# xipengwang/AprilSAM

Measured on AMD Instinct MI355X. Metric: Gauss-Newton iterations/sec + factorise ms on M3500 (chi2 match <=1e-6), higher is better.
Workload: dtype f64; 1 GPU; M3500 batch april_graph_cholesky, 1 replica per GPU (3500 poses, 5454 factors, n=10500); parallelism=single GPU, fronts=680, levels=9, nnz_L=422121

## Files before the change

### aprilsam_amd/csrc/capi.cpp

```cpp
#include <algorithm>
#include <cstdio>
#include <cstdlib>
#include <cstring>
#include <string>
#include <vector>

#include "../../include/aprilsam_amd.h"
#include "plan.h"
#include "errors.h"
#include "refmodel.h"
#include "solver.h"

extern "C" {

void APRILSAM_VERSION(void) {
    printf("================\n");
    printf("| APRILSAM 0.0 |   solver: aprilsam_amd (MI355X / gfx950)\n");
    printf("================\n");
    printf("\n");
}

void april_graph_cholesky_param_init(april_graph_cholesky_param_t *param) {
    asam::drop_context(param);
    asam::unbind_param(param);
// ... 39 lines not shown
int aprilsam_amd_resident_steps(april_graph_t *graph, april_graph_cholesky_param_t *param, int n, int mode) { return asam::resident_steps(graph, param, n, mode); }
int aprilsam_amd_resident_sync(april_graph_t *graph, april_graph_cholesky_param_t *param) { return asam::resident_sync(graph, param); }
double aprilsam_amd_resident_chi2(april_graph_t *graph) { return asam::resident_chi2(graph); }
int aprilsam_amd_resident_end(april_graph_t *graph, april_graph_cholesky_param_t *param) { return asam::resident_end(graph, param); }
int aprilsam_amd_level_profile(const april_graph_cholesky_param_t *param, double *out6, int cap_levels) { return asam::level_profile(param, out6, cap_levels); }
int aprilsam_amd_kernel_profile(const april_graph_cholesky_param_t *param, double *ms, long long *calls, double *flops, double *bytes, const char **names) {
    return asam::kernel_profile(param, ms, calls, flops, bytes, names);
}
int aprilsam_amd_debug_stage(april_graph_t *graph, april_graph_cholesky_param_t *param, int what, double *out) { return asam::debug_stage(graph, param, what, out); }
int aprilsam_amd_debug_front_times(const april_graph_cholesky_param_t *param, long long *out, int n_fronts) { return asam::debug_front_times(param, out, n_fronts); }
int aprilsam_amd_reference_order(int n_nodes, int n_factors, const int *fa, const int *fb, int *out_order, int *out_parent) {
    asam::RefModel m;
    m.batch(n_nodes, n_factors, fa, fb);
    memcpy(out_order, m.ord.data(), sizeof(int) * (size_t)n_nodes);
    if (out_parent) memcpy(out_parent, m.parent.data(), sizeof(int) * (size_t)n_nodes);
    return 0;
}
int aprilsam_amd_shard_begin(april_graph_t *graph, april_graph_cholesky_param_t *param, int rank, int world) { return asam::shard_begin(graph, param, rank, world); }
long long aprilsam_amd_shard_info(const april_graph_cholesky_param_t *param, int what, long long *out, long long cap) { return asam::shard_info(param, what, out, cap); }
int aprilsam_amd_shard_comm_unique_id(char *out128) { return asam::shard_comm_unique_id(out128); }
int aprilsam_amd_shard_comm_init_rccl(april_graph_cholesky_param_t *param, const char *id128) { return asam::shard_comm_init_rccl(param, id128); }
int aprilsam_amd_shard_comm_init_host(april_graph_cholesky_param_t *param, const aprilsam_amd_host_comm_t *cb) { return asam::shard_comm_init_host(param, cb); }
int aprilsam_amd_shard_comm_info(const april_graph_cholesky_param_t *param, long long *out5, char *rccl_path, int cap) { return asam::shard_comm_info(param, out5, rccl_path, cap); }
int aprilsam_amd_shard_iterate(april_graph_t *graph, april_graph_cholesky_param_t *param, int n) { return asam::shard_iterate(graph, param, n); }
int aprilsam_amd_shard_gather_states(april_graph_t *graph, april_graph_cholesky_param_t *param) { return asam::shard_gather_states(graph, param); }
double aprilsam_amd_shard_chi2(april_graph_t *graph, april_graph_cholesky_param_t *param) { return asam::shard_chi2(graph, param); }
void aprilsam_amd_shard_end(april_graph_cholesky_param_t *param) { asam::shard_end(param); }

void *aprilsam_amd_refmodel_create(void) { return new asam::RefModel(); }
void aprilsam_amd_refmodel_destroy(void *m) { delete (asam::RefModel *)m; }
void aprilsam_amd_refmodel_batch(void *m, int n_nodes, int n_factors, const int *fa, const int *fb) { ((asam::RefModel *)m)->batch(n_nodes, n_factors, fa, fb); }
int aprilsam_amd_refmodel_inc_begin(void *m, int n_nodes, int n_factors, const int *fa, const int *fb) {
    asam::RefModel *M = (asam::RefModel *)m;
    M->inc_begin(n_nodes, n_factors, fa, fb);
    return M->naffected;
}
int aprilsam_amd_refmodel_solve_visit(void *m, const double *x, double dxy, double dth, int *visited) {
    asam::RefModel *M = (asam::RefModel *)m;
    for (int i = 0; i < M->N; i++) visited[i] = 0;
    M->solve_visit(x, dxy, dth, [&](int n, bool upd) { visited[n] = upd ? 2 : 1; });
    return M->start_over;
}
void aprilsam_amd_refmodel_get(void *m, int *parent, int *changed, int *relin) {
    asam::RefModel *M = (asam::RefModel *)m;
    for (int i = 0; i < M->N; i++) { if (parent) parent[i] = M->parent[i]; if (changed) changed[i] = M->changed[i]; if (relin) relin[i] = M->relin[i]; }
}
int aprilsam_amd_refmodel_check(void *m) { return ((asam::RefModel *)m)->check_tree(); }
int aprilsam_amd_last_error(char *msg, int cap) { return asam::get_last_error(msg, cap); }
void aprilsam_amd_clear_error(void) { asam::clear_last_error(); }
int aprilsam_amd_selftest(void) { return asam::selftest(); }
const char *aprilsam_amd_version(void) { return "aprilsam_amd 0.1 (gfx950, multifrontal FP64)"; }
void aprilsam_amd_free(void *p) { free(p); }

struct aprilsam_amd_plan { asam::Plan P; };

aprilsam_amd_plan_t *aprilsam_amd_plan_create(int n_nodes, int n_factors, const int *factor_nodes, const double *xy, int leaf_nodes) {
    aprilsam_amd_plan *pl = new aprilsam_amd_plan();
    try {
        asam::build_plan(pl->P, n_nodes, n_factors, factor_nodes, xy, leaf_nodes > 0 ? leaf_nodes : asam::g_opt.leaf_nodes);
    } catch (const asam::SolverError &e) {
        asam::set_last_error(e.code, e.msg);
        fprintf(stderr, "aprilsam_amd: ERROR %d: %s\n", e.code, e.msg.c_str());
        delete pl;
        return nullptr;
    } catch (const std::exception &e) {
        asam::set_last_error(asam::ERR_INTERNAL, e.what());
        fprintf(stderr, "aprilsam_amd: ERROR %d: %s\n", (int)asam::ERR_INTERNAL, e.what());
        delete pl;
        return nullptr;
    }
    return pl;
}
void aprilsam_amd_plan_destroy(aprilsam_amd_plan_t *plan) { delete plan; }

long long aprilsam_amd_shard_plan(const aprilsam_amd_plan_t *plan, int world, int what, long long *out, long long cap) {
    if (!plan || world < 1) return -1;
    std::vector<int> owner; std::vector<char> top; std::vector<long long> xfer, bcast, v;
    asam::shard_map(plan->P, world, owner, top, xfer, bcast);
    if (what == 1) v = xfer; else if (what == 2) v = bcast; else if (what == 3) v.assign(owner.begin(), owner.end());
    else if (what == 4) v = asam::shard_critical_path(plan->P, world, owner, top); else return -1;
    if (out) for (long long i = 0; i < (long long)v.size() && i < cap; i++) out[i] = v[i];
    return (long long)v.size();
}

int aprilsam_amd_xcd_place(int nF, const int *parent, const int *level, const int *nsb, int l0, int cap, int cap_leaf, int which, int *out, int out_cap) {
    if (nF < 0 || !parent || !level || !nsb || which < 0 || which > 3) return -100;
    std::vector<int> up, leaves;
    int top = 0;
    for (int t = 0; t < nF; t++) top = std::max(top, level[t]);
    for (int l = l0; l <= top; l++) for (int t = 0; t < nF; t++) if (level[t] == l) up.push_back(t);
    if (l0 == 1) for (int t = 0; t < nF; t++) if (level[t] == 0) leaves.push_back(t);
    const asam::XcdLists x = asam::xcd_place(up, leaves, parent, nsb, nF, cap, cap_leaf);
    if (which == 3) return asam::xcd_check(x, up, leaves, parent, nF, cap, cap_leaf);
    const std::vector<int> &v = which == 0 ? x.up : which == 1 ? x.dn : x.leaf;
    if (out) for (int i = 0; i < (int)v.size() && i < out_cap; i++) out[i] = v[i];
    return (int)v.size();
}

long long aprilsam_amd_plan_query(const aprilsam_amd_plan_t *plan, const char *what, long long **out) {
    std::string k(what);
    if (k.compare(0, 3, "bd_") == 0 || k.compare(0, 3, "rd_") == 0) asam::build_gather_lists(const_cast<asam::Plan &>(plan->P));
    const asam::Plan &P = plan->P;
    std::vector<long long> v;
    auto from = [&](const auto &a) { v.assign(a.begin(), a.end()); };
    if (k == "perm") from(P.perm);
    else if (k == "pos") from(P.pos);
    else if (k == "front_first") from(P.f_first);
// ... 34 lines not shown
```

### aprilsam_amd/csrc/kernels.hip.h

```cpp
#pragma once
#include <hip/hip_runtime.h>
#include <stdint.h>

#include <type_traits>
namespace asam {

constexpr int PROF_SLOTS = 16;
constexpr int PROF_XCD_UP = 12, PROF_XCD_DN = 13;
constexpr int PROF_X_STORED = 14, PROF_X_DRAINED = 11, PROF_X_FLAG = 15;
__device__ __forceinline__ int xcc_id() { return __builtin_amdgcn_s_getreg(20 | (0 << 6) | ((4 - 1) << 11)) & 7; }
constexpr int TPB = 256;
constexpr int NB = 32;
constexpr int TILE = 64;
constexpr int ASM_CB = 4;
constexpr int OBP = 4;

struct FrontDesc {
    long long off;
    int nsb, nub, first;
    int dest_begin, dest_end;
    int ch_begin, ch_end;
    int rows_begin;
    int parent;
    int dinv0;
// ... 418 lines not shown
        asm volatile("buffer_wbl2 sc1\n\ts_waitcnt vmcnt(0) lgkmcnt(0)" ::: "memory");
        __hip_atomic_store(flag, ev ? ev : 1, __ATOMIC_RELAXED, __HIP_MEMORY_SCOPE_AGENT);
        if (pf) { pf[PROF_X_DRAINED] = t_drained; pf[PROF_X_FLAG] = wall_clock64(); }
    }
}
__device__ __forceinline__ void st_agent(double *p, double v) { __hip_atomic_store(p, v, __ATOMIC_RELAXED, __HIP_MEMORY_SCOPE_AGENT); }
__device__ __forceinline__ void publish_flag_wt(int *flag, int ev, long long *pf = nullptr) {
    asm volatile("s_waitcnt vmcnt(0)" ::: "memory");
    __syncthreads();
    if (threadIdx.x == 0) {
        const long long t_drained = pf ? wall_clock64() : 0;
        __hip_atomic_store(flag, ev, __ATOMIC_RELAXED, __HIP_MEMORY_SCOPE_AGENT);
        if (pf) { pf[PROF_X_DRAINED] = t_drained; pf[PROF_X_FLAG] = wall_clock64(); }
    }
}
__device__ __forceinline__ int x_handover_mode(const DevPlan &P, const int *xflags, int ev, bool in_launch) { return (xflags && ev != 0 && in_launch) ? P.xmode : X_FLUSH; }
constexpr size_t HANDOVER_LDS_MIN = 80 * 1024 + 256;
__device__ __forceinline__ __amdgpu_buffer_rsrc_t xg_rsrc(const DevPlan &P) { return __builtin_amdgcn_make_buffer_rsrc((void *)P.xg, 0, (int)P.xg_bytes, 0x00020000); }
typedef unsigned xg_u4 __attribute__((ext_vector_type(4)));
__device__ __forceinline__ void st_granule(__amdgpu_buffer_rsrc_t r, size_t i, double v, int tag) {
    const xg_u4 g = { (unsigned)__double2loint(v), (unsigned)tag, (unsigned)__double2hiint(v), (unsigned)tag };
    __builtin_amdgcn_raw_buffer_store_b128(g, r, (int)(i * 16), 0, 16);
}
__device__ __forceinline__ void gather_x(const DevPlan &P, const FrontDesc &D_, const int *rows, double *dst, int n, int ev, int *bad, long long *pf) {
    const int tid = threadIdx.x;
    const __amdgpu_buffer_rsrc_t r = xg_rsrc(P);
    auto tagged = [&](const xg_u4 &g) { return ((int)g.y == ev && (int)g.w == ev) || ((int)g.y == XG_CONST && (int)g.w == XG_CONST); };
    auto give_up = [&]() { if (atomicCAS(bad, 0, 9) == 0) { bad[2] = 9; bad[3] = 0; } };
    if (tid == 0) {
        const int g1 = P.fd[D_.parent].parent;
        if (g1 >= 0 && P.fd[g1].nsb > 0) {
            const unsigned gi = 3u * (unsigned)P.fd[g1].first * 16u;
            for (int spins = 0; !tagged(__builtin_amdgcn_raw_buffer_load_b128(r, (int)gi, 0, 16)); ) {
                __builtin_amdgcn_s_sleep(8); asm volatile("" ::: "memory");
                if (++spins > (1 << 21)) { give_up(); break; }
            }
        }
    }
    __syncthreads();
    if (pf && tid == 0) pf[4] = wall_clock64();
    if (tid < n) {
        const int e = tid;
        const unsigned gi = (3u * (unsigned)rows[e / 3] + (unsigned)(e % 3)) * 16u;
        xg_u4 g = __builtin_amdgcn_raw_buffer_load_b128(r, (int)gi, 0, 16);
        for (int spins = 0; !tagged(g); g = __builtin_amdgcn_raw_buffer_load_b128(r, (int)gi, 0, 16)) {
            __builtin_amdgcn_s_sleep(1); asm volatile("" ::: "memory");
            if (++spins > (1 << 23)) { give_up(); break; }
        }
        dst[e] = __hiloint2double((int)g.z, (int)g.x);
    }
}
__device__ __forceinline__ void reset_flag(int *flag, int v) { __hip_atomic_store(flag, v, __ATOMIC_RELAXED, __HIP_MEMORY_SCOPE_AGENT); }

enum { ASM_LDS = 0, ASM_GLOBAL = 1, ASM_SPLIT = 2 };
template <int NT, int MODE, bool ZERO = true>
__device__ __forceinline__ void assemble_front(const DevPlan &P, const FrontDesc &D, const double *__restrict__ pool,
                                               const double *__restrict__ Hc, int bc0, int bc1, bool full,
                                               double *__restrict__ dstL, int ldL, double *__restrict__ dstG, int ldG, int2 *__restrict__ wl,
                                               long long *pf = nullptr, const int *wait_flags = nullptr, int *bad = nullptr, int ev = 0, int skip_child = -1, int skip_child2 = -1) {
    const int tid = threadIdx.x;
    const int nsb = D.nsb, nbc = D.nsb + D.nub;
    const int R = 3 * (nbc + 1);
    const int rhs_row = 3 * nbc;
    const int csplit = MODE == ASM_LDS ? (1 << 30) : (MODE == ASM_GLOBAL ? 0 : 3 * nsb);
    auto put = [&](int col, int row, double v) { if (col < csplit) dstL[(size_t)col * ldL + row] = v; else dstG[(size_t)col * ldG + row] = v; };
    auto add_plain = [&](int col, int row, double v) { if (col < csplit) dstL[(size_t)col * ldL + row] += v; else dstG[(size_t)col * ldG + row] += v; };
    auto add_child = [&](int col, int row, double v) {
        if (col < csplit) front_add<false>(dstL + (size_t)col * ldL + row, v); else front_add<true>(dstG + (size_t)col * ldG + row, v);
    };
    constexpr int NW = NT / 64;
    const int wv = __builtin_amdgcn_readfirstlane(tid >> 6), lane = tid & 63;
    const int nch = D.ch_end - D.ch_begin;
    ChildRec *__restrict__ crs = (ChildRec *)wl;
    if (tid < min(nch, CAPQ)) crs[tid] = P.child[D.ch_begin + tid];
    if constexpr (ZERO) {
        for (int col = 3 * bc0 + wv; col < 3 * bc1; col += NW) {
            const double lam = col < 3 * nsb ? P.lambda[D.first + col / 3] : 0.0;
            for (int row = 3 * (col / 3) + lane; row < R; row += 64) put(col, row, row == col ? lam : 0.0);
        }
    }
    __syncthreads();
    if (pf && tid == 0) pf[4] = wall_clock64();
    {
        int d0 = D.dest_begin, d1 = D.dest_end;
        if (!full) {
            int a = d0, b = d1;
            while (a < b) { int m = (a + b) >> 1; if (P.dest[m].bcol < bc0) a = m + 1; else b = m; }
            d0 = a; b = d1;
            while (a < b) { int m = (a + b) >> 1; if (P.dest[m].bcol < bc1) a = m + 1; else b = m; }
            d1 = a;
        }
        for (int e = tid; e < (d1 - d0) * 9; e += NT) {
            const int d = d0 + e / 9, k = e % 9;
            const int i = k / 3, j = k - 3 * i;
            const DestRec rec = P.dest[d];
            const bool rhs = rec.brow < 0;
            if (rhs ? (i > 0) : (rec.brow == rec.bcol && i < j)) continue;
            double acc = 0;
            if (rec.src_end >= 0) {
                for (int q = rec.src_begin; q < rec.src_end; q += 4) {
                    double a[4];
#pragma unroll
                    for (int j = 0; j < 4; j++) a[j] = Hc[(size_t)min(q + j, rec.src_end - 1) * 9 + k];
#pragma unroll
                    for (int j = 0; j < 4; j++) acc = (q + j < rec.src_end) ? acc + a[j] : acc;
                }
            }
            else { for (int q = rec.src_begin; q < -rec.src_end; q++) acc += Hc[(size_t)P.src_idx[q] * 9 + k]; }
            add_plain(3 * rec.bcol + j, rhs ? rhs_row : 3 * rec.brow + i, acc);
        }
    }
    __syncthreads();
    if (pf && tid == 0) pf[5] = wall_clock64();
    int2 *__restrict__ mywl = wl + CAPQ * 3 + wv * WCAP;
    int g0 = 0;
    auto rec_of = [&](int q) -> ChildRec {
        ChildRec c = crs[q - g0];
        const unsigned lo = __builtin_amdgcn_readfirstlane((unsigned)(c.uoff & 0xffffffffll)), hi = __builtin_amdgcn_readfirstlane((unsigned)(c.uoff >> 32));
        c.uoff = (long long)(((unsigned long long)hi << 32) | lo);
        c.cR = __builtin_amdgcn_readfirstlane(c.cR); c.cnu = __builtin_amdgcn_readfirstlane(c.cnu);
        c.rel_begin = __builtin_amdgcn_readfirstlane(c.rel_begin);
        return c;
    };
    constexpr int TE = 4;
    struct Trip { double v[3 * TE]; int d[TE], rc[TE], col[TE], cc[TE], nrow[TE], r0[TE]; };
    auto load_trip = [&](int i, int n, Trip &T) {
        int2 e[TE]; ChildRec cr[TE];
#pragma unroll
        for (int u = 0; u < TE; u++) e[u] = mywl[i + u < n ? i + u : i];
#pragma unroll
        for (int u = 0; u < TE; u++) cr[u] = crs[(__builtin_amdgcn_readfirstlane(e[u].x) & 0x3fffffff) - g0];
#pragma unroll
        for (int u = 0; u < TE; u++) {
            const bool has = i + u < n;
            const int x = __builtin_amdgcn_readfirstlane(e[u].x), y = __builtin_amdgcn_readfirstlane(e[u].y);
            ChildRec c = cr[u];
            const unsigned lo = __builtin_amdgcn_readfirstlane((unsigned)(c.uoff & 0xffffffffll)), hi = __builtin_amdgcn_readfirstlane((unsigned)(c.uoff >> 32));
            c.uoff = (long long)(((unsigned long long)hi << 32) | lo);
            c.cR = __builtin_amdgcn_readfirstlane(c.cR); c.cnu = __builtin_amdgcn_readfirstlane(c.cnu);
            c.rel_begin = __builtin_amdgcn_readfirstlane(c.rel_begin);
            const int cc = 3 * (y & 0xffff), nrow = has ? 3 * c.cnu + 1 : 0, r = cc + 64 * (x >> 30) + lane;
            T.cc[u] = cc; T.col[u] = 3 * (y >> 16); T.nrow[u] = nrow; T.r0[u] = cc + 64 * (x >> 30);
            const double *__restrict__ sp = pool + c.uoff + (size_t)cc * c.cR;
            const int rc = has ? min(r, nrow - 1) : cc;
#pragma unroll
            for (int c3 = 0; c3 < 3; c3++) T.v[3 * u + c3] = ld_agent(sp + (size_t)c3 * c.cR + rc);
            T.d[u] = P.f_rel[c.rel_begin + min(rc, nrow - 2) / 3];
            T.rc[u] = rc;
        }
    };
    double *dummy = (double *)(wl + CAPQ * 3 + NW * WCAP) + wv * 64 + lane;
    const int dummy_off = MODE == ASM_GLOBAL ? 0 : (int)(dummy - dstL);
    auto apply_trip = [&](const Trip &T) {
#pragma unroll
        for (int u = 0; u < TE; u++) {
            const int r = T.r0[u] + lane;
            const bool inr = r < T.nrow[u];
            const int du = (T.rc[u] < T.nrow[u] - 1) ? 3 * T.d[u] + T.rc[u] % 3 : rhs_row;
            if (T.col[u] < csplit) {
#pragma unroll
                for (int c3 = 0; c3 < 3; c3++) {
                    const int o = (inr && r >= T.cc[u] + c3) ? (T.col[u] + c3) * ldL + du : dummy_off;
                    dstL[o] += T.v[3 * u + c3];
                }
            } else {
#pragma unroll
                for (int c3 = 0; c3 < 3; c3++)
                    if (inr && r >= T.cc[u] + c3) unsafeAtomicAdd(dstG + (size_t)(T.col[u] + c3) * ldG + du, T.v[3 * u + c3]);
            }
        }
    };
    auto rest = [&](int i, int n) {
        for (int u = 0; u < TE && i + u < n; u++) {
            const int2 e = mywl[i + u];
            const int x = __builtin_amdgcn_readfirstlane(e.x), y = __builtin_amdgcn_readfirstlane(e.y);
            if (x >> 30) continue;
            const ChildRec c = rec_of(x & 0x3fffffff);
            const int cc = 3 * (y & 0xffff), col = 3 * (y >> 16), nrow = __builtin_amdgcn_readfirstlane(3 * c.cnu + 1);
            if (cc + 128 >= nrow) continue;
            const double *__restrict__ sp = pool + c.uoff + (size_t)cc * c.cR;
            for (int r0 = cc + 128; r0 < nrow; r0 += 256) {
                double v[12]; int d[4];
#pragma unroll
                for (int k = 0; k < 4; k++) {
                    const int r = r0 + 64 * k + lane;
#pragma unroll
                    for (int c3 = 0; c3 < 3; c3++) v[3 * k + c3] = ld_agent(sp + (size_t)c3 * c.cR + min(r, nrow - 1));
                    d[k] = P.f_rel[c.rel_begin + min(r, nrow - 2) / 3];
                }
#pragma unroll
                for (int k = 0; k < 4; k++) { const int r = r0 + 64 * k + lane; d[k] = (r < nrow - 1) ? 3 * d[k] + r % 3 : rhs_row; }
#pragma unroll
                for (int k = 0; k < 4; k++)
#pragma unroll
                    for (int c3 = 0; c3 < 3; c3++) if (r0 + 64 * k + lane < nrow) add_child(col + c3, d[k], v[3 * k + c3]);
            }
        }
    };
    auto process = [&](int n) {
        for (int i = 0; i < n; i += TE) {
            Trip T;
            load_trip(i, n, T);
            apply_trip(T);
            rest(i, n);
        }
    };
    int qn = 0, c0n = 0;
    auto slice_rel = [&](int q, int c0, int *cnu_out) -> int {
        if (q >= min(nch, g0 + CAPQ)) { *cnu_out = 0; return -1; }
        const ChildRec c = rec_of(q);
        if (q == skip_child || q == skip_child2) { *cnu_out = 0; return -1; }
        *cnu_out = c.cnu;
        const int jb = c0 + lane;
        return (lane < 32 && jb < c.cnu) ? P.f_rel[c.rel_begin + jb] : -1;
    };
// ... 65 lines not shown
#pragma unroll
            for (int b = 0; b < 2; b++) acc[a][b] = (d4_t){ 0, 0, 0, 0 };
        for (int ks = 0; ks < nk; ks++) {
            const int kk = 4 * ks + l4;
            const bool kok = kk < kw;
            const double *col = S + (size_t)(k_lo + (kok ? kk : 0)) * ld;
            double pj[2], pi[2];
#pragma unroll
            for (int q = 0; q < 2; q++) { double x = col[rj[q]], y = col[ri[q]]; pj[q] = kok ? x : 0.0; pi[q] = kok ? y : 0.0; }
#pragma unroll
            for (int a = 0; a < 2; a++)
#pragma unroll
                for (int b = 0; b < 2; b++) acc[a][b] = __builtin_amdgcn_mfma_f64_16x16x4f64(pj[a], pi[b], acc[a][b], 0, 0, 0);
        }
        if (TO_GLOBAL) {
#pragma unroll
            for (int a = 0; a < 2; a++)
#pragma unroll
                for (int b = 0; b < 2; b++)
#pragma unroll
                    for (int reg = 0; reg < 4; reg++) {
                        const int i = i0 + 16 * b + l15, j = j0 + 16 * a + l4 + 4 * reg;
                        if (i < Rv && j < col_hi && i >= j) {
                            if constexpr (TO_GLOBAL == 2) Cg[(size_t)j * ldg + i] = -acc[a][b][reg];
                            else unsafeAtomicAdd(Cg + (size_t)j * ldg + i, -acc[a][b][reg]);
                        }
                    }
        } else {
            double cv[16]; int off[16]; bool ok[16];
#pragma unroll
            for (int a = 0; a < 2; a++)
#pragma unroll
                for (int b = 0; b < 2; b++)
#pragma unroll
                    for (int reg = 0; reg < 4; reg++) {
                        const int i = i0 + 16 * b + l15, j = j0 + 16 * a + l4 + 4 * reg, e = (a * 2 + b) * 4 + reg;
                        ok[e] = i < Rv && j < col_hi && i >= j;
                        off[e] = ok[e] ? j * ld + i : -1;
                    }
#pragma unroll
            for (int e = 0; e < 16; e++) cv[e] = off[e] >= 0 ? S[off[e]] : 0.0;
#pragma unroll
            for (int a = 0; a < 2; a++)
#pragma unroll
                for (int b = 0; b < 2; b++)
#pragma unroll
                    for (int reg = 0; reg < 4; reg++) cv[(a * 2 + b) * 4 + reg] -= acc[a][b][reg];
#pragma unroll
            for (int e = 0; e < 16; e++) if (off[e] >= 0) S[off[e]] = cv[e];
        }
    }
}

template <int NT>
__device__ __forceinline__ void lds_syrk16(double *__restrict__ S, int ld, int k_lo, int k_hi, int col_lo, int col_hi, int Rv,
                                           int w0 = 0, int nw = NT / 64) {
    const int wave = __builtin_amdgcn_readfirstlane((int)(threadIdx.x >> 6)) - w0;
    const int lane = threadIdx.x & 63, l15 = lane & 15, l4 = lane >> 4;
    if (wave < 0 || wave >= nw) return;
    const int ntr = (Rv - col_lo + 15) >> 4, ntc = (col_hi - col_lo + 15) >> 4;
    const int ntiles = ntc * ntr - ntc * (ntc - 1) / 2;
    const int kw = k_hi - k_lo, nk = (kw + 3) >> 2;
    for (int l = wave; l < ntiles; l += nw) {
        int ti = l, tj = 0;
        while (ti >= ntr - tj) { ti -= ntr - tj; tj++; }
        ti += tj;
        const int i0 = col_lo + 16 * ti, j0 = col_lo + 16 * tj;
        const int rj = min(j0 + l15, Rv - 1), ri = min(i0 + l15, Rv - 1);
        const int i = i0 + l15, jb = j0 + l4;
        const int cbase = jb * ld + i;
        bool ok[4];
#pragma unroll
        for (int reg = 0; reg < 4; reg++) { const int j = jb + 4 * reg; ok[reg] = i < Rv && j < col_hi && i >= j; }
        double cv[4], x[4], y[4];
#pragma unroll
        for (int reg = 0; reg < 4; reg++) cv[reg] = S[ok[reg] ? cbase + 4 * reg * ld : 0];
#pragma unroll
        for (int ks = 0; ks < 4; ks++) {
            const int kk = 4 * ks + l4;
            const double *col = S + (k_lo + (kk < kw ? kk : 0)) * ld;
            x[ks] = col[rj]; y[ks] = col[ri];
        }
        d4_t acc = (d4_t){ 0, 0, 0, 0 };
#pragma unroll
        for (int ks = 0; ks < 4; ks++) {
            if (ks < nk) {
                const bool kok = 4 * ks + l4 < kw;
                acc = __builtin_amdgcn_mfma_f64_16x16x4f64(kok ? x[ks] : 0.0, kok ? y[ks] : 0.0, acc, 0, 0, 0);
            }
        }
#pragma unroll
        for (int reg = 0; reg < 4; reg++) if (ok[reg]) S[cbase + 4 * reg * ld] = cv[reg] - acc[reg];
    }
}

constexpr int GB = 4;

constexpr int BW = 16;
template <int NT, int BWT>
__device__ __forceinline__ void chain_block(double *S, int ld, int k0, int wdt, int Rv, int *bad, double (&Dd)[BWT], int nwc) {
    constexpr int BROWS = 64 - BWT;
    constexpr int PER = BWT <= 8 ? 1 : (BWT - 2 + 7) / 8;
    const int wave = __builtin_amdgcn_readfirstlane(threadIdx.x >> 6), lane = threadIdx.x & 63;
    const bool isdiag = lane < BWT;
    const int below0 = k0 + wdt;
    const int nchunk = max(1, (Rv - below0 + BROWS - 1) / BROWS);
    if (wave >= nchunk) return;
    for (int ch = wave + ((nchunk - 1 - wave) / nwc) * nwc; ch >= wave; ch -= nwc) {
        const int row = isdiag ? k0 + lane : below0 + BROWS * ch + (lane - BWT);
        const bool valid = isdiag ? lane < wdt : row < Rv;
        const int rowc = valid ? row : k0;
        double D[BWT];
#pragma unroll
        for (int c = 0; c < BWT; c++) D[c] = S[(size_t)(k0 + (c < wdt ? c : 0)) * ld + rowc];
        int isbad = 0;
        double dn = readlane_d(D[0], 0);
        if (!(dn > 0)) isbad = 1;
        double inv = fast_rsqrt(dn);
#pragma unroll
        for (int j = 0; j < BWT; j++) {
            D[j] *= inv;
            double lc[BWT];
            if (j + 1 < BWT) {
                lc[j + 1] = readlane_d(D[j], j + 1);
                D[j + 1] = fma(-D[j], lc[j + 1], D[j + 1]);
                dn = readlane_d(D[j + 1], j + 1);
                if (j + 1 < wdt && !(dn > 0)) isbad = 1;
            }
#pragma unroll
            for (int c = j + 2; c < BWT; c++) lc[c] = readlane_d(D[j], c);
            __builtin_amdgcn_sched_barrier(0);
            double y = 0, h = 0, e = 0;
#pragma unroll
            for (int st = 0; st < 8; st++) {
                if (j + 1 < BWT) {
                    if (st == 0) { y = __builtin_amdgcn_rsq(dn); h = 0.5 * dn; }
                    else if (st == 1 || st == 4) e = -h * y;
                    else if (st == 2 || st == 5) e = fma(e, y, 0.5);
                    else if (st == 3 || st == 6) y = fma(y, e, y);
                }
#pragma unroll
                for (int q = 0; q < PER; q++) {
                    const int c = j + 2 + PER * st + q;
                    if (c < BWT) D[c] = fma(-D[j], lc[c], D[c]);
                }
                __builtin_amdgcn_sched_barrier(0);
            }
            inv = y;
        }
        if (valid && !isdiag) {
#pragma unroll
            for (int c = BWT - 1; c >= 0; c--) S[(size_t)(k0 + (c < wdt ? c : 0)) * ld + row] = (c < wdt) ? D[c] : D[0];
        }
        if (ch == 0) {
#pragma unroll
            for (int c = 0; c < BWT; c++) Dd[c] = D[c];
            if (isbad && lane == 0) { if (atomicCAS(bad, 0, 1) == 0) { bad[2] = 1; bad[3] = k0 / 3; } }
        }
    }
}
template <int BWT>
__device__ __forceinline__ void chain_store_diag(double *S, int ld, int k0, int wdt, const double (&Dd)[BWT]) {
    const int r = threadIdx.x & 63;
    if (r < wdt) {
#pragma unroll
        for (int c = 0; c < BWT; c++) if (c < wdt) S[(k0 + c) * ld + k0 + r] = (c <= r) ? Dd[c] : 0.0;
    }
}
template <int NT>
__device__ __forceinline__ void factor_dense_blk(double *S, int ld, int ns, int Rv, int hi, int *bad, double * , long long *pf = nullptr) {
    constexpr int NW = NT / 64;
    long long t_chain = 0, t_syrk = 0, t0 = 0;
    const int wave = __builtin_amdgcn_readfirstlane(threadIdx.x >> 6);
    auto chain_sync_store = [&](int k0, int nwc) {
        const int wdt = min(BW, ns - k0);
        if (wdt <= 8) {
            double D8[8];
            chain_block<NT, 8>(S, ld, k0, wdt, Rv, bad, D8, nwc);
            __syncthreads();
            if (wave == 0) chain_store_diag<8>(S, ld, k0, wdt, D8);
        } else {
            double D16[16];
            chain_block<NT, 16>(S, ld, k0, wdt, Rv, bad, D16, nwc);
            __syncthreads();
            if (wave == 0) chain_store_diag<16>(S, ld, k0, wdt, D16);
        }
    };
    auto chain_waves = [&](int k0) {
        const int wdt = min(BW, ns - k0), brows = 64 - (wdt <= 8 ? 8 : 16);
        const int nchunk = max(1, (Rv - (k0 + wdt) + brows - 1) / brows);
        return min(nchunk, NW / 2);
    };
    if (pf) t0 = wall_clock64();
    chain_sync_store(0, NW);
    if (pf) { const long long t1 = wall_clock64(); t_chain += t1 - t0; t0 = t1; }
    for (int k0 = 0; k0 < ns; k0 += BW) {
        const int wdt = min(BW, ns - k0), below0 = k0 + wdt;
        if (below0 < ns) {
            const int next_hi = min(below0 + BW, ns), cw = chain_waves(below0);
            if (NW >= 8) lds_syrk16<NT>(S, ld, k0, below0, below0, next_hi, Rv, 1, NW - 1);
            else lds_syrk16<NT>(S, ld, k0, below0, below0, next_hi, Rv);
            __syncthreads();
            if (pf) { const long long t1 = wall_clock64(); t_syrk += t1 - t0; t0 = t1; }
            if (wave < cw) {
                long long w0_ = 0, c0_ = 0;
                if (pf) { w0_ = wall_clock64(); c0_ = clock64(); }
                chain_sync_store(below0, cw);
                if (pf && threadIdx.x == 0) { pf[10] += clock64() - c0_; pf[15] += wall_clock64() - w0_; }
            } else {
                if (next_hi < hi) lds_syrk16<NT>(S, ld, k0, below0, next_hi, hi, Rv, cw, NW - cw);
                __syncthreads();
            }
            if (pf) { const long long t1 = wall_clock64(); t_chain += t1 - t0; t0 = t1; }
        } else {
            __syncthreads();
            if (below0 < hi) lds_syrk16<NT>(S, ld, k0, below0, below0, hi, Rv);
            __syncthreads();
            if (pf) { const long long t1 = wall_clock64(); t_syrk += t1 - t0; t0 = t1; }
        }
    }
    if (pf && threadIdx.x == 0) { pf[8] = t_chain; pf[9] = t_syrk; }
}
template <int NT>
__device__ __forceinline__ void factor_front_blk(double *S, int ld, int nsb, int nbc, int *bad, double *stage, int nbc_upd = -1, long long *pf = nullptr) {
    if (nbc_upd < 0) nbc_upd = nbc;
    factor_dense_blk<NT>(S, ld, 3 * nsb, 3 * (nbc + 1) - 2, 3 * nbc_upd, bad, stage, pf);
}

__host__ __device__ inline size_t small_front_lds(int R, int C, int nw) { return (size_t)(R | 1) * C * 8 + wl_bytes(nw); }
__host__ __device__ inline size_t panel_front_lds(int R, int ns, int nw) { return (size_t)(R | 1) * ns * 8 + wl_bytes(nw); }

template <int NT>
__device__ __forceinline__ void front_small_body(const DevPlan &P, const int t, double *__restrict__ pool, const double *__restrict__ Hc, int *bad,
                                                 long long full_lds_limit, int *flags, int wait, double *S) {
    const int *wflags = wait ? flags : nullptr;
    const int ev = flags ? flag_value(P) : 0;
    const FrontDesc D = P.fd[t];
    const int nsb = D.nsb, nbc = D.nsb + D.nub;
    const int R = 3 * (nbc + 1), C = 3 * nbc, ld = R | 1;
    double *Fg = pool + D.off;
    if (P.prof && threadIdx.x == 0) P.prof[(size_t)t * PROF_SLOTS + PROF_XCD_UP] = 1 + xcc_id();
    if ((long long)small_front_lds(R, C, NT / 64) <= full_lds_limit) {
        int2 *wl = (int2 *)(S + (size_t)ld * C);
        if (P.prof && threadIdx.x == 0) P.prof[(size_t)t * PROF_SLOTS + 0] = wall_clock64();
        assemble_front<NT, ASM_LDS>(P, D, pool, Hc, 0, nbc, true, S, ld, nullptr, 0, wl, P.prof ? P.prof + (size_t)t * PROF_SLOTS : nullptr, wflags, bad, ev);
        if (P.prof && threadIdx.x == 0) P.prof[(size_t)t * PROF_SLOTS + 1] = wall_clock64();
        factor_front_blk<NT>(S, ld, nsb, nbc, bad, (double *)wl, -1, P.prof ? P.prof + (size_t)t * PROF_SLOTS : nullptr);
        if (P.prof && threadIdx.x == 0) P.prof[(size_t)t * PROF_SLOTS + 2] = wall_clock64();
        for (int c = 3 * nsb + (threadIdx.x >> 6); c < C; c += NT / 64) {
            int r0 = 3 * (c / 3);
            for (int r = r0 + (threadIdx.x & 63); r < R; r += 64) Fg[(size_t)c * R + r] = S[(size_t)c * ld + r];
        }
        if (flags) publish_flag(flags + t, ev);
        for (int c = threadIdx.x >> 6; c < 3 * nsb; c += NT / 64) {
            int r0 = 3 * (c / 3);
            for (int r = r0 + (threadIdx.x & 63); r < R; r += 64) Fg[(size_t)c * R + r] = S[(size_t)c * ld + r];
        }
    } else {
        const int ns = 3 * nsb;
        int2 *wl = (int2 *)(S + (size_t)ld * ns);
        const bool schur_first = P.schur_first_nub > 0 && D.nub >= P.schur_first_nub;
        if (P.prof && threadIdx.x == 0) P.prof[(size_t)t * PROF_SLOTS + 0] = wall_clock64();
        if (schur_first) assemble_front<NT, ASM_SPLIT>(P, D, pool, Hc, 0, nsb, false, S, ld, Fg, R, wl, P.prof ? P.prof + (size_t)t * PROF_SLOTS : nullptr, wflags, bad, ev);
        else assemble_front<NT, ASM_SPLIT>(P, D, pool, Hc, 0, nbc, true, S, ld, Fg, R, wl, P.prof ? P.prof + (size_t)t * PROF_SLOTS : nullptr, wflags, bad, ev);
        if (P.prof && threadIdx.x == 0) P.prof[(size_t)t * PROF_SLOTS + 1] = wall_clock64();
        factor_front_blk<NT>(S, ld, nsb, nbc, bad, (double *)wl, nsb, P.prof ? P.prof + (size_t)t * PROF_SLOTS : nullptr);
        if (P.prof && threadIdx.x == 0) P.prof[(size_t)t * PROF_SLOTS + 2] = wall_clock64();
        if (schur_first) {
            lds_panel_syrk<NT, 2>(S, ld, 0, ns, ns, C, R - 2, Fg, R);
            __syncthreads();
            assemble_front<NT, ASM_GLOBAL, false>(P, D, pool, Hc, nsb, nbc, false, nullptr, 0, Fg, R, wl, nullptr, nullptr, bad);
        }
        else if (nbc > nsb) lds_panel_syrk<NT, 1>(S, ld, 0, ns, ns, C, R - 2, Fg, R);
        if (flags) publish_flag(flags + t, ev);
        for (int c = threadIdx.x >> 6; c < ns; c += NT / 64) {
            int r0 = 3 * (c / 3);
            for (int r = r0 + (threadIdx.x & 63); r < R; r += 64) Fg[(size_t)c * R + r] = S[(size_t)c * ld + r];
        }
    }
    if (P.prof) { __syncthreads(); if (threadIdx.x == 0) P.prof[(size_t)t * PROF_SLOTS + 3] = wall_clock64(); }
}
constexpr int UPD_MAXF = 4;
constexpr int UPD_MAXC = 4;
struct UpdRec {
    long long old_off;
    int mode;
    int old_nub;
    int wout;
    int mask;
    int n_own, own_f[UPD_MAXF], own_la[UPD_MAXF], own_lb[UPD_MAXF], own_slot[UPD_MAXF];
    int n_ch, ch_t[UPD_MAXC], ch_wout[UPD_MAXC], ch_rel[UPD_MAXC], ch_cnu[UPD_MAXC], ch_mask[UPD_MAXC];
    int pad[3];
};
static_assert(sizeof(UpdRec) == 192, "UpdRec layout");
struct UpdCtx {
// ... 226 lines not shown
                    }
#pragma unroll
                    for (int u = 0; u < 4; u++) {
                        r0 = fma(-L[u], kk[7 * u], r0); r1 = fma(-L[u], kk[7 * u + 1], r1); r2 = fma(-L[u], kk[7 * u + 2], r2);
                        L[u] = fma(kk[7 * u + 6], L[u], fma(r0, kk[7 * u + 3], fma(r1, kk[7 * u + 4], r2 * kk[7 * u + 5])));
                    }
#pragma unroll
                    for (int u = 0; u < 4; u++) Li[(size_t)(j + u) * ld] = L[u];
                }
                for (; j < jn; j++) {
                    const double *k8 = K8 + 8 * j;
                    const double L = Li[(size_t)j * ld];
                    r0 = fma(-L, k8[0], r0); r1 = fma(-L, k8[1], r1); r2 = fma(-L, k8[2], r2);
                    Li[(size_t)j * ld] = fma(k8[6], L, fma(r0, k8[3], fma(r1, k8[4], r2 * k8[5])));
                }
                if (i >= ns) {
                    const double w0 = r0 * Cm[0], w1 = (r1 - Cm[1] * w0) * Cm[2], w2 = (r2 - Cm[3] * w0 - Cm[4] * w1) * Cm[5];
                    W0[i] = w0; W0[(size_t)ld + i] = w1; W0[(size_t)2 * ld + i] = w2;
                }
            }
        }
        __syncthreads();
    }
    for (int cu0 = 4 * wave; cu0 < nu; cu0 += 4 * NW) {
        for (int pass = 0; pass * 64 < nu + 1; pass++) {
            double old[4];
#pragma unroll
            for (int u = 0; u < 4; u++) {
                const int cu = min(cu0 + u, nu - 1), ru = pass * 64 + lane;
                const bool has = cu < nu_o && (ru < nu_o || ru == nu);
                old[u] = has ? Fo[(size_t)(ns + cu) * R_o + ns + (ru == nu ? nu_o : ru)] : 0.0;
            }
#pragma unroll
            for (int u = 0; u < 4; u++) {
                const int cu = cu0 + u, ru = pass * 64 + lane;
                if (cu < nu && ru <= nu && ru >= 3 * (cu / 3)) {
                    double acc = old[u];
                    for (int v = 0; v < 3 * nact; v++) acc = fma(Wv[(size_t)v * ld + ns + ru], Wv[(size_t)v * ld + ns + cu], acc);
                    Fg[(size_t)(ns + cu) * R + ns + ru] = acc;
                }
            }
        }
    }
    for (int c = wave; c < ns; c += NW) {
        const int r0 = 3 * (c / 3);
        for (int r = r0 + lane; r < R; r += 64) Fg[(size_t)c * R + r] = Ls[(size_t)c * ld + r];
    }
    if (flags) publish_flag(flags + t, ev);
    if (pf) { __syncthreads(); if (tid == 0) pf[3] = wall_clock64(); }
}

template <int NT>
__global__ void __launch_bounds__(NT) k_front_small(DevPlan P, const int *__restrict__ fronts, double *__restrict__ pool,
                                                    const double *__restrict__ Hc, int *bad, long long full_lds_limit,
                                                    int *flags = nullptr, int wait = 0, UpdCtx uc = UpdCtx{}) {
    extern __shared__ __attribute__((aligned(16))) double S[];
    const int t = fronts[blockIdx.x];
    if (t < 0) return;
    if (uc.recs) {
        const UpdRec *rec = uc.recs + blockIdx.x;
        if (rec->mode) { front_update_body<NT>(P, t, *rec, uc, pool, flags, bad, S); return; }
    }
    front_small_body<NT>(P, t, pool, Hc, bad, full_lds_limit, flags, wait, S);
}

constexpr int ASM_INV_CAP = 4096;
__global__ void __launch_bounds__(TPB) k_assemble_big(DevPlan P, const int *__restrict__ list, const int *__restrict__ pre, int n,
                                                      double *__restrict__ pool, const double *__restrict__ Hc) {
    const int a = find_seg(pre, n, blockIdx.x);
    const int t = list[a], bc0 = (blockIdx.x - pre[a]) * ASM_CB;
    const FrontDesc D = P.fd[t];
    const int nbc = D.nsb + D.nub;
    const int bc1 = min(bc0 + ASM_CB, nbc);
    __shared__ int2 wl[wl_bytes(TPB / 64) / 8];
    __shared__ short inv[2][ASM_INV_CAP];
    const int prim = D.prim1 - 1, sec = D.prim2 - 1;
    if (prim < 0 || nbc + 1 > ASM_INV_CAP) {
        assemble_front<TPB, ASM_GLOBAL>(P, D, pool, Hc, bc0, bc1, false, nullptr, 0, pool + D.off, 3 * (nbc + 1), wl);
        return;
    }
    const int tid = threadIdx.x, wv = __builtin_amdgcn_readfirstlane(tid >> 6), lane = tid & 63;
    const int nst = sec >= 0 ? 2 : 1;
    const ChildRec cr0 = P.child[D.ch_begin + prim], cr1 = P.child[D.ch_begin + max(sec, 0)];
    const int R = 3 * (nbc + 1);
    for (int e = tid; e <= nbc; e += TPB) { inv[0][e] = -1; inv[1][e] = -1; }
    __syncthreads();
    for (int j = tid; j < cr0.cnu; j += TPB) inv[0][P.f_rel[cr0.rel_begin + j]] = (short)j;
    if (nst > 1) for (int j = tid; j < cr1.cnu; j += TPB) inv[1][P.f_rel[cr1.rel_begin + j]] = (short)j;
    if (tid == 0) { inv[0][nbc] = (short)cr0.cnu; if (nst > 1) inv[1][nbc] = (short)cr1.cnu; }
    __syncthreads();
    double *__restrict__ dst = pool + D.off;
    for (int col = 3 * bc0 + wv; col < 3 * bc1; col += TPB / 64) {
        const int bcol = col / 3, c3 = col - 3 * bcol;
        const double lam = col < 3 * D.nsb ? P.lambda[D.first + bcol] : 0.0;
        const int jc0 = __builtin_amdgcn_readfirstlane((int)inv[0][bcol]), jc1 = nst > 1 ? __builtin_amdgcn_readfirstlane((int)inv[1][bcol]) : -1;
        if (jc0 < 0 && jc1 < 0) {
            for (int row = 3 * bcol + lane; row < R; row += 64) dst[(size_t)col * R + row] = row == col ? lam : 0.0;
            continue;
        }
        const int cc0 = 3 * max(jc0, 0) + c3, cc1 = 3 * max(jc1, 0) + c3;
        const double *__restrict__ s0 = pool + cr0.uoff + (size_t)cc0 * cr0.cR, *__restrict__ s1 = pool + cr1.uoff + (size_t)cc1 * cr1.cR;
        for (int r0 = 3 * bcol; r0 < R; r0 += 128) {
            double v0[2], v1[2]; bool ok0[2], ok1[2];
#pragma unroll
            for (int u = 0; u < 2; u++) {
                const int row = r0 + 64 * u + lane, rc = min(row, R - 1), brow = rc / 3, i3 = rc - 3 * brow;
                const int jr0 = inv[0][brow], cr_0 = 3 * jr0 + i3, jr1 = inv[1][brow], cr_1 = 3 * jr1 + i3;
                ok0[u] = row < R && jc0 >= 0 && jr0 >= 0 && (brow < nbc ? cr_0 >= cc0 : i3 == 0);
                ok1[u] = row < R && jc1 >= 0 && jr1 >= 0 && (brow < nbc ? cr_1 >= cc1 : i3 == 0);
                v0[u] = ld_agent(s0 + (ok0[u] ? cr_0 : cc0));
                v1[u] = ld_agent(s1 + (ok1[u] ? cr_1 : cc1));
            }
#pragma unroll
            for (int u = 0; u < 2; u++) {
                const int row = r0 + 64 * u + lane;
                if (row < R) dst[(size_t)col * R + row] = ((row == col ? lam : 0.0) + (ok0[u] ? v0[u] : 0.0)) + (ok1[u] ? v1[u] : 0.0);
// ... 1103 lines not shown
        if (tid < 64) chain_store_diag<W>(M, TAIL_LD, 0, q, Dd);
        __syncthreads();
    };
    if (q <= 8) chain(std::integral_constant<int, 8>{}); else if (q <= 16) chain(std::integral_constant<int, 16>{}); else chain(std::integral_constant<int, TAILQ>{});
    if (ts.solve && tid < 64) {
        const int c = tid, off = 3 * (ts.a_idx - ts.s_idx), qs = off + q;
        const bool on = c < qs, fresh = c >= off;
        const double *Mc = M + (size_t)((on && fresh) ? c - off : 0) * TAIL_LD;
        double l[TAILQ];
#pragma unroll
        for (int i = 1; i < TAILQ; i++) l[i] = fresh ? ((on && i > c && i < qs) ? Mc[i - off] : 0.0) : so[i];
        const double rinv = on ? 1.0 / (fresh ? Mc[c - off] : so[0]) : 0.0;
        double w = on ? (fresh ? Mc[q] : so[TAILQ]) * rinv : 0.0;
#pragma unroll
        for (int i = 1; i < TAILQ; i++) l[i] *= rinv;
#pragma unroll
        for (int i = TAILQ - 1; i > 0; i--) {
            const double xi = readlane_d(w, i);
            w = fma(-l[i], xi, w);
        }
        const int k = c / 3, comp = c - 3 * k;
        const double x0 = __shfl(w, 3 * k, 64), x1 = __shfl(w, 3 * k + 1, 64), x2 = __shfl(w, 3 * k + 2, 64);
        if (on) {
            const int node = ts.first + ts.s_idx + k;
            xg[(size_t)3 * node + comp] = w;
            const size_t o = (size_t)3 * node + comp;
            if (isnan(x0) || isnan(x1) || isnan(x2)) {
                const double qnan = __longlong_as_double(0x7ff8000000000000ll);
                upd.dX[o] = qnan;
                if (upd.dx_out) upd.dx_out[o] = qnan;
            } else {
                double sv = upd.lp[o] + w;
                if (comp == 2) sv = mod2pi_dev(sv);
                upd.dX[o] = w;
                if (upd.st) upd.st[o] = sv;
                if (upd.st_out) { upd.st_out[o] = sv; upd.dx_out[o] = w; }
            }
        }
        if (upd.bad_out && tid == 0 && __hip_atomic_load(a.bad, __ATOMIC_RELAXED, __HIP_MEMORY_SCOPE_AGENT) != 0) {
#pragma unroll
            for (int kk = 0; kk < 4; kk++) upd.bad_out[kk] = __hip_atomic_load(a.bad + kk, __ATOMIC_RELAXED, __HIP_MEMORY_SCOPE_AGENT);
        }
    }
    for (int c = tid >> 6; c < q; c += NT / 64) {
        const int cg = c0 + c;
        for (int r = 3 * (cg / 3) + (tid & 63); r <= m; r += 64)
            Fg[(size_t)cg * R + r] = r < c0 + q ? M[c * TAIL_LD + r - c0] : (r == m ? M[c * TAIL_LD + q] : 0.0);
    }
}

template <int NT>
__global__ void __launch_bounds__(NT) k_inc_one(IncPrologue a, IncFlags fl, InlinePatches, DevPlan P, TailStep ts, const int *__restrict__ up_list, int n_up,
                                                const int *__restrict__ dn_list, int n_dn,
                                                double *__restrict__ pool, long long full_lds_limit, double *__restrict__ x, UpdArgs upd, UpdCtx uc = UpdCtx{}) {
    extern __shared__ __attribute__((aligned(16))) double S[];
    long long *stamps = a.stamps;
    if (stamps && threadIdx.x == 0) stamps[0] = wall_clock64();
    double pre[TAIL_PRE], so[TAILQ + 1];
    if (ts.t >= 0) {
        tail_prefetch<NT>(ts, pool, pre);
        if constexpr (NT < 1024) tail_prefetch_solve(ts, pool, so);
        else { for (int i = 0; i <= TAILQ; i++) so[i] = 0.0; }
    }
    inc_prologue_body(a, fl, ts.t >= 0 ? tail_mirror(S) : nullptr);
    __syncthreads();
    __builtin_amdgcn_s_dcache_inv();
    if (stamps && threadIdx.x == 0) stamps[2] = wall_clock64();
    if (ts.t >= 0) { tail_refactor<NT>(ts, pool, a, S, pre, x, upd, so); __syncthreads(); }
    for (int i = 0; i < n_up; i++) {
        const int t = up_list[i];
        if (uc.recs && uc.recs[i].mode) {
            UpdCtx ul = uc; ul.wflags = nullptr;
            front_update_body<NT>(P, t, uc.recs[i], ul, pool, nullptr, a.bad, S);
            __syncthreads();
            continue;
        }
        if (stamps && i == n_up - 1) {
            DevPlan Pp = P; Pp.prof = stamps + 8 - (size_t)t * PROF_SLOTS; Pp.prof_mode = 1;
            front_small_body<NT>(Pp, t, pool, a.Hc, a.bad, full_lds_limit, nullptr, 0, S);
            if (threadIdx.x == 0) { const FrontDesc D = P.fd[t]; stamps[5] = D.nsb; stamps[6] = D.nub; stamps[7] = D.ch_end - D.ch_begin; }
        } else
            front_small_body<NT>(P, t, pool, a.Hc, a.bad, full_lds_limit, nullptr, 0, S);
        __syncthreads();
    }
    if (stamps && threadIdx.x == 0) stamps[3] = wall_clock64();
    if (threadIdx.x >= TPB) return;
    for (int i = 0; i < n_dn; i++) {
        backsolve_w_body<(NT >= 1024 ? 32 : BSW)>(P, dn_list[i], pool, x, nullptr, a.bad, upd, S);
        __syncthreads();
    }
    if (stamps && threadIdx.x == 0) stamps[4] = wall_clock64();
    if (a.done) {
        __threadfence_system();
        __syncthreads();
        if (threadIdx.x == 0) {
            asm volatile("buffer_wbl2 sc0 sc1\n\ts_waitcnt vmcnt(0) lgkmcnt(0)" ::: "memory");
            __hip_atomic_store(a.done, a.seq, __ATOMIC_RELAXED, __HIP_MEMORY_SCOPE_SYSTEM);
        }
    }
}
__global__ void __launch_bounds__(TPB) k_load_states_lp(int n3, const double *__restrict__ host_st, const double *__restrict__ host_lp,
                                                        double *__restrict__ st, double *__restrict__ lp, int *__restrict__ bad) {
    const int i = blockIdx.x * blockDim.x + threadIdx.x;
    if (bad && i < 4) bad[i] = 0;
    if (i < n3) { st[i] = host_st[i]; lp[i] = host_lp[i]; }
}

__global__ void __launch_bounds__(TPB) k_mask_owned(int n3, const int *__restrict__ nown, int rank, const double *__restrict__ st,
                                                    const double *__restrict__ lp, const double *__restrict__ dx, double *__restrict__ out) {
    const int i = blockIdx.x * blockDim.x + threadIdx.x;
    if (i >= n3) return;
    const bool mine = nown[i / 3] == rank;
    out[i] = mine ? st[i] : 0.0; out[n3 + i] = mine ? lp[i] : 0.0; out[2 * (size_t)n3 + i] = mine ? dx[i] : 0.0;
}

__global__ void __launch_bounds__(TPB) k_load_states(int n3, const double *__restrict__ host_st, double *__restrict__ st, double *__restrict__ lp) {
    const int i = blockIdx.x * blockDim.x + threadIdx.x;
    if (i < n3) { const double v = host_st[i]; st[i] = v; lp[i] = v; }
}

__global__ void __launch_bounds__(TPB) k_update_states(int N, const int *__restrict__ pos, const double *__restrict__ x,
                                                       const double *__restrict__ lp, double *__restrict__ st,
                                                       double *__restrict__ dX, double *__restrict__ st_out = nullptr,
                                                       double *__restrict__ dx_out = nullptr, const int *__restrict__ bad = nullptr,
                                                       int *__restrict__ bad_out = nullptr) {
    int i = blockIdx.x * blockDim.x + threadIdx.x;
    if (bad_out && i < 4) bad_out[i] = bad[i];
    if (i >= N) return;
    const double *d = x + (size_t)3 * pos[i];
    double d0 = d[0], d1 = d[1], d2 = d[2];
    if (isnan(d0) || isnan(d1) || isnan(d2)) {
        const double qnan = __longlong_as_double(0x7ff8000000000000ll);
        dX[3 * i + 0] = qnan; dX[3 * i + 1] = qnan; dX[3 * i + 2] = qnan;
        if (dx_out) { dx_out[3 * i + 0] = qnan; dx_out[3 * i + 1] = qnan; dx_out[3 * i + 2] = qnan; }
        return;
// ... 12 lines not shown
```

### aprilsam_amd/csrc/plan.h

```cpp
#pragma once
#include <cstdint>
#include <functional>
#include <vector>

namespace asam {

struct Plan {
    int N = 0;
    int F = 0;
    int leaf_nodes = 16;

    std::vector<int> perm;
    std::vector<int> pos;

    int nF = 0;
    std::vector<int> f_first;
    std::vector<int> f_nsb;
    std::vector<int> f_nub;
    std::vector<int> f_parent;
    std::vector<int> f_level;
    std::vector<int64_t> f_rows_ptr;
    std::vector<int> f_rows;
    std::vector<int> f_rel;
    std::vector<int> ch_ptr, ch_idx;
    std::vector<int64_t> f_off;
    int64_t pool_doubles = 0;

    inline int rows(int t) const { return 3 * (f_nsb[t] + f_nub[t] + 1); }
    inline int cols(int t) const { return 3 * (f_nsb[t] + f_nub[t]); }

    std::vector<int> fac_front;
    std::vector<int> fac_la, fac_lb;
    std::vector<int> bd_front_ptr;
    std::vector<int> bd_row, bd_col;
    std::vector<int> bd_src_ptr;
    std::vector<int> bd_src;
    std::vector<int> rd_front_ptr;
    std::vector<int> rd_col;
    std::vector<int> rd_src_ptr;
    std::vector<int> rd_src;
    std::vector<uint8_t> fac_swap;
    struct DestRec { int brow, bcol, src_begin, src_end; };
    std::vector<int> dest_front_ptr;
    std::vector<DestRec> dest;
    std::vector<int> slot_blk;
    std::vector<int> slot_rhs;
    int n_slots = 0;

    int nLevels = 0;
    std::vector<int> lev_ptr, lev_fronts;

    int max_rows = 0;
    int64_t nnzL = 0;
    double flops = 0;
};

void build_plan(Plan &P, int N, int F, const int *factor_nodes, const double *xy, int leaf_nodes);
void build_gather_lists(Plan &P);

struct XcdLists { std::vector<int> up, dn, leaf; };
XcdLists xcd_place(const std::vector<int> &up, const std::vector<int> &leaves, const int *parent, const int *nsb, int nF, int cap, int cap_leaf);
int xcd_check(const XcdLists &x, const std::vector<int> &up, const std::vector<int> &leaves, const int *parent, int nF, int cap, int cap_leaf);

struct NDTree {
    struct Node { std::vector<int> verts; std::vector<int> children; };
    std::vector<Node> nodes;
    std::vector<int> roots;
};
void nested_dissection(int N, const std::vector<int> &adj_ptr, const std::vector<int> &adj,
                       const double *xy, int leaf_nodes, NDTree &tree);

struct PlanSession { explicit PlanSession(int n_nodes, int min_nodes = 1024); ~PlanSession(); PlanSession(const PlanSession &) = delete; bool on = false; };
void plan_parallel_for(int n, int grain, const std::function<void(int, int)> &body);

}
```

### aprilsam_amd/csrc/solver.h

```cpp
#pragma once
#include <vector>
#include "../../include/aprilsam_amd.h"

namespace asam {

struct Options {
    int leaf_nodes = 16;
    int deterministic = 0;
    int use_graph = 1;
    int device_timing = 0;
    int trust_factor_cache = 0;
    int small_lds_kb = 156;
    int inc_fast = 1;
    int inc_multi = 1;
    int inc_one = 1;
    int inc_one_up = 3, inc_one_dn = 4, inc_one_threads = 512, inc_one_spin = 1;
    int inc_tail = 1;
    int inc_inline = 1;
    int inc_tail_solve = 1;
    int inc_lazy_states = 1;
    int inc_replan_tall = 1;
    int inc_update = 1;
    int speculate_factors = 1;
    int warm_up = 1;
    int syrk_xcd_order = 512;
    int syrk_small_tiles = 320;
    int syrk_pair_tiles = 2048;
    int syrk_group = 3;
    int schur_first = 40;
    int small_threads = 1024;
    int tp_threads = 512;
    int tp_fronts = 1000;
    int tp_lds_kb = 80;
    int amalg = 0;
    int amalg_max = 64;
    int pin_last = 0;
    int batch_extend = 1;
    int extend_tail_fronts = 3;
    int persist = 1;
    int persist_max_fronts = 240;
    int xcd_place = 1;
    int tail_poses = 28;
    int blk_backsolve = 1;
    int wave_backsolve = 1;
    int tagged_x = 1;
    int linearize_staged_min = 32768;
    int mem_cap_mb = 0;
    int pool_guard = 0;
    int pool_poison = 0;
    int skip_flag_waits = 0;
    int panel_mode = 1;
};
extern Options g_opt;

void batch_step(april_graph_t *g, april_graph_cholesky_param_t *param);
void inc_step(april_graph_t *g, april_graph_cholesky_param_t *param);
void inc_solve_only(april_graph_t *g, april_graph_cholesky_param_t *param);
double graph_chi2(april_graph_t *g);
int batch_resident(april_graph_t *g, april_graph_cholesky_param_t *param, int iters, double *chi2_out, double *ms_out);
int resident_begin(april_graph_t *g, april_graph_cholesky_param_t *param);
int resident_steps(april_graph_t *g, april_graph_cholesky_param_t *param, int n, int mode);
int resident_sync(april_graph_t *g, april_graph_cholesky_param_t *param);
double resident_chi2(april_graph_t *g);
int resident_end(april_graph_t *g, april_graph_cholesky_param_t *param);
int level_profile(const april_graph_cholesky_param_t *param, double *out, int cap_levels);
int kernel_profile(const april_graph_cholesky_param_t *param, double *ms, long long *calls, double *flops, double *bytes, const char **names);
void drop_context(const april_graph_cholesky_param_t *p);
void drop_graph_pack(const april_graph_t *g);
bool get_stats(const april_graph_cholesky_param_t *p, aprilsam_amd_stats_t *out);
int shard_begin(april_graph_t *g, april_graph_cholesky_param_t *param, int rank, int world);
long long shard_info(const april_graph_cholesky_param_t *param, int what, long long *out, long long cap);
int shard_comm_unique_id(char *out128);
int shard_comm_init_rccl(const april_graph_cholesky_param_t *param, const char *id128);
int shard_comm_init_host(const april_graph_cholesky_param_t *param, const aprilsam_amd_host_comm_t *cb);
int shard_comm_info(const april_graph_cholesky_param_t *param, long long *out, char *path, int cap);
int shard_iterate(april_graph_t *g, april_graph_cholesky_param_t *param, int n);
int shard_gather_states(april_graph_t *g, april_graph_cholesky_param_t *param);
double shard_chi2(april_graph_t *g, april_graph_cholesky_param_t *param);
void shard_end(const april_graph_cholesky_param_t *param);
int debug_guard_selftest(const april_graph_cholesky_param_t *param);
int debug_stage(april_graph_t *g, april_graph_cholesky_param_t *param, int what, double *out);
// ... 35 lines not shown
```

### aprilsam_amd/csrc/solver.hip.cpp

```cpp
#include <hip/hip_runtime.h>
#include <rccl/rccl.h>
#include <dlfcn.h>

#include <algorithm>
#include <array>
#include <chrono>
#include <thread>
#include <cmath>
#include <cstdio>
#include <cstdlib>
#include <cstring>
#include <functional>
#include <map>
#include <memory>
#include <atomic>
#include <mutex>
#include <string>
#include <unordered_map>
#include <vector>

#include "../../include/aprilsam_amd.h"
#include "errors.h"
#include "kernels.hip.h"
#include "maxmix.hip.h"
#include "robust.hip.h"
#include "lm.hip.h"
#include "chordal.hip.h"
#include "selinv.hip.h"
#include "pathsolve.hip.h"
#include "plan.h"
#include "refmodel.h"
#include "solver.h"

namespace asam {

#define HIPCHECK(expr)                                                                                 \
    do {                                                                                               \
        hipError_t e_ = (expr);                                                                        \
        if (e_ != hipSuccess) {                                                                        \
            (void)hipGetLastError();                                                                   \
            fail(e_ == hipErrorOutOfMemory ? ERR_OOM : ERR_HIP, "%s failed: %s (%s:%d)", #expr, hipGetErrorString(e_), __FILE__, __LINE__); \
        }                                                                                              \
    } while (0)

static double now_ms() {
    return std::chrono::duration<double, std::milli>(std::chrono::steady_clock::now().time_since_epoch()).count();
}

Options g_opt;
struct OptionDef { const char *name; int Options::*member; int min_value; bool policy; int max_value = 0x7fffffff; };
static const OptionDef OPTION_TABLE[] = {
    { "leaf_nodes", &Options::leaf_nodes, 1, false }, { "deterministic", &Options::deterministic, 0, true }, { "use_graph", &Options::use_graph, 0, true },
    { "device_timing", &Options::device_timing, 0, true }, { "trust_factor_cache", &Options::trust_factor_cache, 0, true },
    { "small_lds_kb", &Options::small_lds_kb, 0, false }, { "syrk_xcd_order", &Options::syrk_xcd_order, 0, false },
    { "schur_first", &Options::schur_first, 0, false }, { "syrk_small_tiles", &Options::syrk_small_tiles, 0, false }, { "syrk_pair_tiles", &Options::syrk_pair_tiles, 0, false }, { "syrk_group", &Options::syrk_group, 2, false, 8 }, { "panel_mode", &Options::panel_mode, 0, false },
    { "small_threads", &Options::small_threads, 64, false }, { "tp_fronts", &Options::tp_fronts, 0, false }, { "tp_lds_kb", &Options::tp_lds_kb, 0, false },
    { "tp_threads", &Options::tp_threads, 64, false }, { "inc_fast", &Options::inc_fast, 0, true }, { "inc_multi", &Options::inc_multi, 0, true },
    { "inc_one", &Options::inc_one, 0, true }, { "inc_one_up", &Options::inc_one_up, 1, true }, { "inc_one_dn", &Options::inc_one_dn, 1, true },
    { "inc_one_threads", &Options::inc_one_threads, 64, true }, { "inc_one_spin", &Options::inc_one_spin, 0, true }, { "inc_tail", &Options::inc_tail, 0, false },
    { "inc_inline", &Options::inc_inline, 0, true }, { "inc_update", &Options::inc_update, 0, true }, { "inc_tail_solve", &Options::inc_tail_solve, 0, true },
    { "inc_lazy_states", &Options::inc_lazy_states, 0, true }, { "inc_replan_tall", &Options::inc_replan_tall, 0, true },
    { "speculate_factors", &Options::speculate_factors, 0, true }, { "warm_up", &Options::warm_up, 0, true }, { "pin_last", &Options::pin_last, 0, false }, { "persist", &Options::persist, 0, false },
    { "persist_max_fronts", &Options::persist_max_fronts, 0, false }, { "xcd_place", &Options::xcd_place, 0, false }, { "linearize_staged_min", &Options::linearize_staged_min, 0, false },
    { "wave_backsolve", &Options::wave_backsolve, 0, false }, { "tagged_x", &Options::tagged_x, 0, false, 2 }, { "blk_backsolve", &Options::blk_backsolve, 0, false }, { "tail_poses", &Options::tail_poses, 8, false },
    { "batch_extend", &Options::batch_extend, 0, true }, { "extend_tail_fronts", &Options::extend_tail_fronts, 0, true }, { "mem_cap_mb", &Options::mem_cap_mb, 0, true },
    { "pool_guard", &Options::pool_guard, 0, false }, { "amalg", &Options::amalg, 0, false }, { "amalg_max", &Options::amalg_max, 1, false }, { "pool_poison", &Options::pool_poison, 0, false }, { "skip_flag_waits", &Options::skip_flag_waits, 0, false },
};
static const OptionDef *find_option(const char *name) {
    for (const OptionDef &d : OPTION_TABLE) if (!strcmp(d.name, name)) return &d;
    return nullptr;
}
static std::once_flag g_opt_once;
static void load_env_options() {
    std::call_once(g_opt_once, [] {
        for (const OptionDef &d : OPTION_TABLE) {
            std::string env = "APRILSAM_AMD_";
            for (const char *q = d.name; *q; q++) env += (char)toupper((unsigned char)*q);
            const char *sv = getenv(env.c_str());
            if (sv && *sv) g_opt.*(d.member) = std::min(d.max_value, std::max(d.min_value, (int)atof(sv)));
        }
    });
}

constexpr int MAX_SLOTS = 64;
static std::atomic<int> g_device{ -1 };
static std::mutex g_slot_mu[MAX_SLOTS];
static thread_local int t_slot = 0;
static int device_count() {
    static std::atomic<int> cached{ 0 };
    int n = cached.load(std::memory_order_relaxed);
    if (n > 0) return n;
    if (hipGetDeviceCount(&n) != hipSuccess) { (void)hipGetLastError(); return 0; }
    if (n > 0) cached.store(n, std::memory_order_relaxed);
    return n;
}
static int physical_device(int slot) { const int n = device_count(); return n > 0 ? slot % n : 0; }
static thread_local int t_device = -1;
template <class V> struct Registry {
    using Map = std::map<const void *, std::unique_ptr<V>>;
    Map m; mutable std::mutex mu;
    typename Map::iterator find(const void *k) { std::lock_guard<std::mutex> lk(mu); return m.find(k); }
    typename Map::iterator end() { return m.end(); }
    std::pair<typename Map::iterator, bool> emplace(const void *k, std::unique_ptr<V> v) { std::lock_guard<std::mutex> lk(mu); return m.emplace(k, std::move(v)); }
    void erase(typename Map::iterator it) { std::lock_guard<std::mutex> lk(mu); m.erase(it); }
    void put(const void *k, std::unique_ptr<V> v) { std::lock_guard<std::mutex> lk(mu); m[k] = std::move(v); }
    template <class F> void for_each(F &&f) { std::lock_guard<std::mutex> lk(mu); for (auto &kv : m) f(*kv.second); }
    template <class F> bool with(const void *k, F &&f) { std::lock_guard<std::mutex> lk(mu); auto it = m.find(k); if (it == m.end()) return false; f(*it->second); return true; }
};
// ... 181 lines not shown
            std::fill(applied.begin(), applied.end(), 0); std::fill(ksum.begin(), ksum.end(), 0);
            for (int o = 0; o * OBP < steps; o++) {
                const int k0 = o * OBP * NB, k1 = std::min(ns, k0 + OBP * NB);
                for (int j = k0; j < k1; j++)
                    for (int i = j; i < Rv; i++)
                        if (applied[(size_t)j * Rv + i] != k0 || ksum[(size_t)j * Rv + i] != (long long)k0 * (k0 - 1) / 2) return -13;
                const int rc = run(o * OBP, (o + 1) * OBP, tile); if (rc) return rc;
            }
            for (int j = ns; j < C; j++)
                for (int i = j; i < Rv; i++)
                    if (applied[(size_t)j * Rv + i] != ns || ksum[(size_t)j * Rv + i] != (long long)ns * (ns - 1) / 2) return -14;
        }
        for (int G : { 2, 3, 4 }) for (int tile : { TILE, TILE / 2 }) {
            std::fill(applied.begin(), applied.end(), 0); std::fill(ksum.begin(), ksum.end(), 0);
            const int nobs = (steps + OBP - 1) / OBP;
            for (int o = 0; o < nobs; o++) {
                const int k0 = o * OBP * NB, k1 = std::min(ns, k0 + OBP * NB);
                for (int j = k0; j < k1; j++)
                    for (int i = j; i < Rv; i++)
                        if (applied[(size_t)j * Rv + i] != k0 || ksum[(size_t)j * Rv + i] != (long long)k0 * (k0 - 1) / 2) return -15;
                int rc;
                const int g0 = (o - o % G) * OBP;
                if (o % G != G - 1) rc = run(g0, (o + 1) * OBP, tile, o + 1 < nobs);
                else rc = run(g0, (o + 1) * OBP, tile);
                if (rc) return rc;
            }
            for (int j = ns; j < C; j++)
                for (int i = j; i < Rv; i++)
                    if (applied[(size_t)j * Rv + i] != ns || ksum[(size_t)j * Rv + i] != (long long)ns * (ns - 1) / 2) return -16;
        }
        long long run_off = 0;
        for (int j = ns; j < C; j++) { if (upd_packed_offset(R, ns, j) != run_off) return -21; run_off += Rv - 3 * (j / 3); }
        if (upd_packed_offset(R, ns, C) != run_off) return -22;
        for (int o = 0; o * OBP < steps; o++)
            for (int rb : { 1, 2 }) {
                const int c1 = std::min(ns, (o + 1) * OBW), below = Rv - c1, nt = block_tiles(R, ns, o, rb);
                if ((long long)nt * BLOCK_ROWS * rb < below || (nt > 0 && (long long)(nt - 1) * BLOCK_ROWS * rb >= below)) return -31;
            }
    }
    for (int ntr = 1; ntr <= 75; ntr += (ntr < 20 ? 1 : 7))
        for (int ntc = 1; ntc <= ntr; ntc += (ntc < 20 ? 1 : 5)) {
            const int nt = ntc * ntr - ntc * (ntc - 1) / 2;
            std::vector<char> seen((size_t)ntr * ntc, 0);
            for (int l = 0; l < nt; l++) {
                int ti = -1, tj = -1;
                trapezoid_tile_xcd(l, nt, ntr, ntc, &ti, &tj);
                if (tj < 0 || tj >= ntc || ti < tj || ti >= ntr || seen[(size_t)tj * ntr + ti]++) return -35;
            }
        }
    for (int nw : { 4, 8, 16 })
        for (int R = 6; R < 400; R += 7)
            for (int nsb = 1; 3 * nsb < R - 3; nsb += 5) {
                const int C = R - 3;
                if (panel_front_lds(R, 3 * nsb, nw) > small_front_lds(R, C, nw)) return -41;
                if (small_front_lds(R, C, nw) != (size_t)(R | 1) * C * 8 + (size_t)wl_bytes(nw)) return -42;
            }
    for (int kind = 0; kind < 3; kind++)
        for (int cap : { 2, 8, 32 }) {
            const int nF = kind == 2 ? 150 : 400;
            std::vector<int> parent(nF, -1), nsb(nF), level(nF, 0);
            unsigned r = 12345u + 77u * kind + (unsigned)cap;
            auto rnd = [&](int m) { r = r * 1103515245u + 12345u; return (int)((r >> 8) % (unsigned)m); };
            for (int t = 0; t < nF - 1; t++) {
                if (kind == 0) parent[t] = t + 1 + rnd(std::min(20, nF - 1 - t));
                else if (kind == 1) parent[t] = t % 3 == 0 ? t + 1 : std::min(nF - 1, t + 3 - t % 3);
                else parent[t] = nF - 1;
                nsb[t] = 1 + rnd(30);
            }
            nsb[nF - 1] = 12;
            for (int t = 0; t < nF - 1; t++) level[parent[t]] = std::max(level[parent[t]], level[t] + 1);
            int top = 0; for (int t = 0; t < nF; t++) top = std::max(top, level[t]);
            for (int l0 : { 0, 1, 2 }) {
                std::vector<int> up, leaves;
                for (int l = l0; l <= top; l++) for (int t = 0; t < nF; t++) if (level[t] == l) up.push_back(t);
                if (l0 == 1) for (int t = 0; t < nF; t++) if (level[t] == 0) leaves.push_back(t);
                const XcdLists x = xcd_place(up, leaves, parent.data(), nsb.data(), nF, cap, cap);
                const int rc = xcd_check(x, up, leaves, parent.data(), nF, cap, cap);
                if (rc) return -50 + rc;
            }
        }
    return 0;
}

int api_device_count() { return device_count(); }
int api_set_device(int d) {
    int n = device_count();
    if (d < 0 || d >= n) return -1;
    g_device = d;
    return 0;
}
int api_param_set_device(const april_graph_cholesky_param_t *param, int slot) {
    if (!param || slot < 0 || slot >= MAX_SLOTS) return -1;
    { SlotLock lk0(param, nullptr); drop_shard_state(param); }
    drop_context(param);
    std::lock_guard<std::mutex> lk(g_param_slot_mu);
    g_param_slot[param] = slot;
    g_param_slot_n.store((int)g_param_slot.size(), std::memory_order_release);
    return 0;
}
int api_param_get_device(const april_graph_cholesky_param_t *param) { return physical_device(slot_for(param, nullptr)); }
void unbind_param(const april_graph_cholesky_param_t *param) {
    if (g_param_slot_n.load(std::memory_order_acquire) == 0) return;
    std::lock_guard<std::mutex> lk(g_param_slot_mu);
    g_param_slot.erase(param);
    g_param_slot_n.store((int)g_param_slot.size(), std::memory_order_release);
}
int api_set_option(const char *name, double v) {
    load_env_options();
    const OptionDef *d = name ? find_option(name) : nullptr;
    if (!d) return -1;
    const int nv = std::min(d->max_value, std::max(d->min_value, (int)v));
    if (g_opt.*(d->member) == nv) return 0;
    g_opt.*(d->member) = nv;
    if (!d->policy) g_opt_epoch++;
    return 0;
}
int api_get_option(const char *name, double *v) {
    load_env_options();
    const OptionDef *d = name ? find_option(name) : nullptr;
    if (!d || !v) return -1;
    *v = (double)(g_opt.*(d->member));
    return 0;
}

}

extern "C" int aprilsam_amd_marginals(april_graph_t *graph, april_graph_cholesky_param_t *param, int n, const int *nodes, double *cov) {
    return asam::marginals(graph, param, n, nodes, nullptr, cov, false);
}
extern "C" int aprilsam_amd_marginals_joint(april_graph_t *graph, april_graph_cholesky_param_t *param, int n, const int *a, const int *b, double *cov) {
    return asam::marginals(graph, param, n, a, b, cov, true);
}
extern "C" int aprilsam_amd_max_selected(april_graph_t *graph, april_graph_cholesky_param_t *param, int n, const int *factors, int *out) {
    return asam::max_selected(graph, param, n, factors, out);
}
extern "C" int aprilsam_amd_robust_weights(april_graph_t *graph, april_graph_cholesky_param_t *param, int n, const int *factors, double *w) {
    return asam::robust_weights(graph, param, n, factors, w);
}
extern "C" long long aprilsam_amd_debug_selinv_runs(const april_graph_cholesky_param_t *param) { return asam::selinv_runs(param); }
extern "C" int aprilsam_amd_marginals_joint_any(april_graph_t *graph, april_graph_cholesky_param_t *param, int n, const int *a, const int *b, double *cov) {
    return asam::marginals_joint_any(graph, param, n, a, b, cov);
}
extern "C" int aprilsam_amd_gate_xyt(april_graph_t *graph, april_graph_cholesky_param_t *param, int n, const int *a, const int *b, const double *z,
                                     const double *W, double *d2, double *S) {
    return asam::gate_xyt(graph, param, n, a, b, z, W, d2, S);
}
extern "C" long long aprilsam_amd_debug_path_solve_bytes(const april_graph_cholesky_param_t *param) { return asam::path_solve_bytes(param); }
extern "C" void aprilsam_amd_lm_opts_init(aprilsam_amd_lm_opts_t *opts) { asam::lm_opts_init(opts); }
extern "C" int aprilsam_amd_optimize_lm(april_graph_t *graph, april_graph_cholesky_param_t *param, const aprilsam_amd_lm_opts_t *opts,
                                        aprilsam_amd_lm_report_t *report, double *trace) {
    return asam::optimize_lm(graph, param, opts, report, trace);
}
extern "C" void aprilsam_amd_chordal_opts_init(aprilsam_amd_chordal_opts_t *opts) { asam::chordal_opts_init(opts); }
extern "C" int aprilsam_amd_initialize_chordal(april_graph_t *graph, april_graph_cholesky_param_t *param, const aprilsam_amd_chordal_opts_t *opts,
                                               aprilsam_amd_chordal_report_t *report, double *rot_out) {
    return asam::initialize_chordal(graph, param, opts, report, rot_out, nullptr);
}
extern "C" int aprilsam_amd_debug_chordal_raw(april_graph_t *graph, april_graph_cholesky_param_t *param, const aprilsam_amd_chordal_opts_t *opts,
                                              aprilsam_amd_chordal_report_t *report, double *raw) {
    return asam::initialize_chordal(graph, param, opts, report, nullptr, raw);
}
```

### aprilsam_amd/csrc/solver_context.inc.h

```cpp
enum { K_LINEARIZE = 0, K_FRONT_SMALL, K_ASSEMBLE_BIG, K_PANEL_BIG, K_SYRK_BIG, K_BACKSOLVE, K_UPDATE, NKERN };
static const char *const KNAMES[NKERN] = { "k_linearize", "k_front_small", "k_assemble_big", "k_panel_big", "k_syrk_big", "k_backsolve", "k_update_states" };
struct Launch { int list_off, pre_off, n, grid; bool single = false; int tile = TILE; };

struct LevelPlan {
    int small_off = 0, n_small = 0; size_t small_lds = 0;
    long long full_limit = 0;
    int small_nt = 512;
    int n_big = 0; size_t asm_lds = 0;
    Launch asm_big{};
    std::vector<Launch> syrka, syrk1;
    bool paired = false;
    std::vector<Launch> bchain, btile, syrkw;
    int all_off = 0, n_all = 0; size_t solve_lds = 0;
    size_t solve_w_lds = 0; int maxns = 0;
    Launch bs_gemv{};
    Launch bs_blk{}; size_t bs_blk_lds = 0;
    int rest_off = 0, n_rest = 0; size_t rest_lds = 0;
};

struct IncState {
    bool ready = false;
    bool pristine = false;
    int Nb = 0, Fb = 0, nF0 = 0, nLev0 = 0;
    int cap_nodes = 0, cap_fact = 0;
    long long i32_used = 0, dest_used = 0, child_used = 0, tab_used = 0, pool_used = 0, pool_cap = 0, o_rows = 0, o_rel = 0;
    int slots_used = 0;
    std::vector<FrontDesc> fd;
    std::vector<int> pos_front;
    std::vector<int> parent;
    std::vector<std::vector<int>> E;
    std::vector<std::vector<int>> xfac;
    std::vector<int> bf_ptr, bf_idx;
    std::vector<int> rel_begin;
    std::vector<int> cur_nub;
    std::vector<long long> cur_cap;
    std::vector<char> dirty;
    std::vector<int> f_level;
    int zpos = 0;
    int tail_ok = -1;
    int recs_stale = -1;
    std::vector<int> t_first, t_cnt;
    std::vector<int> tf_of;
    std::vector<std::vector<int>> kids;
    std::vector<LevelPlan> base_levels;
    std::vector<int> st_i32, st_tab, st_sb, st_sr, st_ids; std::vector<DestRec> st_dest; std::vector<ChildRec> st_child;
    std::vector<unsigned char> st_sw; std::vector<double> st_zeros; std::vector<char> need;
    std::vector<char> stale;
    bool upd_ok = true;
    bool base_has_big = false;
    std::vector<char> st_mid, st_mode; std::vector<int> st_owner, st_mask, st_wout, st_slot; std::vector<UpdRec> st_upd, st_rec;
};

struct SelLevel { int gat_off = 0, n_gat = 0, diag_off = 0, n_diag = 0, tri_off = 0, n_tri = 0, x_off = 0, n_x = 0, sus_off = 0, n_sus = 0, sss_off = 0, n_sss = 0; };

struct PathState {
    long long serial = -1;
    int N = 0;
    std::vector<SelFront> fr; std::vector<int> depth, i32, rec, node_j;
    DBuf<PsFront> d_fr; DBuf<int4> d_ent; DBuf<int> d_cmap; DBuf<long long> d_at; DBuf<PsPath> d_path; DBuf<PsPair> d_pair;
// ... 1 lines not shown
    long long peak_doubles = 0;
    void release() {
        d_fr.release(); d_ent.release(); d_cmap.release(); d_at.release(); d_path.release(); d_pair.release(); d_buf.release(); d_cov.release(); d_in.release(); h_out.release();
        fr.clear(); depth.clear(); i32.clear(); rec.clear(); node_j.clear(); serial = -1;
    }
};

struct Context {
    Plan plan;
    bool have_plan = false;
    std::vector<int> pat;
    int patN = 0;
    DBuf<int> d_i32; DBuf<FrontDesc> d_fd; DBuf<DestRec> d_dest; DBuf<ChildRec> d_child; DBuf<double> d_lambda;
    DevPlan dp{};
    DBuf<int> d_tab;
    std::vector<LevelPlan> levels;
    DBuf<unsigned char> d_swap;
    DBuf<int> d_pos;
    DBuf<long long> d_prof;
    DBuf<double> d_pool, d_H, d_x, d_diag;
    DBuf<int> d_bad;
    HBuf<int> h_bad;
    IncPrologue pro{}; InlinePatches inl{};
    bool no_speculation = false;
    HBuf<long long> h_kstamp; HBuf<int> h_done; int done_seq = 0, one_wait = 0;
    std::vector<double> h_lambda;
    aprilsam_amd_stats_t st{};
    hipEvent_t ev[8] = {};
    bool have_events = false;
    double k_ms[NKERN] = {}; long long k_calls[NKERN] = {};
    std::vector<hipEvent_t> k_ev; std::vector<int> k_ids, k_lev;
    std::vector<double> lev_up_ms, lev_dn_ms;
    bool have_fact = false;
    int plan_pin = 0;
    long long plan_persist = 0;
    int same_topo_batches = 0;
    bool used_inc = false;
    bool want_inc = false;
    int batch_nodes = 0;
    IncState inc;
    int inc_F = 0, inc_N = 0;
    std::vector<RefModel::Visit> visits; std::vector<int> involved;
    std::vector<int> base_tab;
    std::vector<int> inc_slot_blk, inc_slot_rhs;
    long long pat_serial = -1, pat_topo = -1;
    RefModel model;
    PatchList patches;
    int batch_factors = 0;
    std::vector<unsigned char> wt; bool wt_any = false, wt_dirty = false;
    long long wt_serial = -1, wt_topo = -1, wt_content = -1;
    DBuf<long long> d_guard; DBuf<int> d_guard_cnt; int n_guard = 0, guard_len = 0;
    std::vector<unsigned char> swap_host;
    int persist_l0 = -1;
    int p_up_off = 0, p_up_n = 0, p_dn_off = 0, p_dn_n = 0, p_nt = 1024; size_t p_up_lds = 0, p_dn_lds = 0; long long p_up_full = 0; int p_dn_maxns = 0, p_dn_maxnu = 0;
    int x_up_off = 0, x_up_n = 0, x_dn_off = 0, x_dn_n = 0;
    int x_leaf_off = 0, x_leaf_n = 0;
    DBuf<int> d_flags, d_flevel, d_perm, d_epoch, d_marks;
    DBuf<uint4> d_xg;
    int flag_stride = 0;
    long long epoch_steps = 0;
    DBuf<double> d_dinv, d_bsb_far; DBuf<int> d_bsb_flags;
    DBuf<int> d_solve_tab; std::vector<int> solve_tab;
    DBuf<UpdRec> d_upd; DBuf<double> d_wbuf;
    hipGraphExec_t gexec = nullptr;
    const void *gexec_key = nullptr;
    long long gexec_serial = 0;
    long long gexec_mx = -1;
    long long gexec_rb = -1;
    hipGraphExec_t gexec_api = nullptr;
    const void *api_key[9] = {};
    hipGraphExec_t gexec_lm = nullptr;
    const void *lm_key[9] = {};
    DBuf<double> d_lm_trial, d_lm_hacc, d_lm_terms, d_lm_trace; DBuf<LmScalars> d_lm; HBuf<LmScalars> h_lm;
    DBuf<double> d_ch; HBuf<double> h_ch; DBuf<int> d_ch_sel;
    int api_key_runs = 0;
    struct Retired { hipGraphExec_t g; hipEvent_t done; };
    std::vector<Retired> retired;
    hipStream_t graph_stream = nullptr;
    void reap_retired(bool wait = false) {
        size_t keep = 0;
        for (Retired &r : retired) {
            if (r.done) {
                if (wait) (void)hipEventSynchronize(r.done);
                else if (hipEventQuery(r.done) != hipSuccess) { retired[keep++] = r; continue; }
                (void)hipEventDestroy(r.done);
            }
            (void)hipGraphExecDestroy(r.g);
        }
        retired.resize(keep);
    }
    void retire(hipGraphExec_t &g) {
        if (!g) return;
        if (retired.size() >= 8) reap_retired();
        if (retired.size() >= 32) reap_retired(true);
        Retired r{ g, nullptr };
        if (graph_stream && hipEventCreateWithFlags(&r.done, hipEventDisableTiming) == hipSuccess) {
            if (hipEventRecord(r.done, graph_stream) != hipSuccess) { (void)hipEventDestroy(r.done); r.done = nullptr; }
        } else r.done = nullptr;
        retired.push_back(r); g = nullptr;
    }
    double lambda_val = -1; int lambda_N = -1;
    int fact_kind = 0; long long fact_epoch = -1; bool fact_asym = false;
    DBuf<double> d_sigma, d_sel_scr; DBuf<SelFront> d_sel_fd; DBuf<int> d_sel_i32, d_sel_q; DBuf<int4> d_sel_ent; HBuf<double> h_cov;
    long long fact_serial = 0;
    std::vector<SelLevel> sel_levels; int sel_tab_kind = 0, sel_N = 0;
    long long sel_serial = -1, sel_tab_serial = -1, sel_runs = 0, sel_pool = 1; double sel_flops = 0;
    PathState ps;
// ... 58 lines not shown
                    hipGraph_t gr = nullptr;
                    (void)hipStreamEndCapture(s, &gr);
                    if (gr) (void)hipGraphDestroy(gr);
                }
                (void)hipStreamSynchronize(s);
                (void)hipGetLastError();
            }
            it->second->release(); g_packs.erase(it);
        }
    }
    if (param) {
        drop_shard_state(param);
        auto it = g_ctx.find(param);
        aprilsam_amd_stats_t st{};
        if (it != g_ctx.end()) { st = it->second->st; it->second->release(); }
        auto fresh = std::make_unique<Context>();
        fresh->st = st; fresh->st.error_code = code; fresh->st.not_spd = 0;
        g_ctx.put(param, std::move(fresh));
    }
}
template <class Fn> static void guarded(const april_graph_cholesky_param_t *param, const april_graph_t *g, Fn &&fn) {
    try { fn(); }
    catch (const SolverError &e) { on_failure(param, g, e.code, e.msg); }
    catch (const std::bad_alloc &) { on_failure(param, g, ERR_OOM, "host memory exhausted (std::bad_alloc)"); }
    catch (const std::exception &e) { on_failure(param, g, ERR_INTERNAL, e.what()); }
}
template <class Fn> static int guarded_rc(const april_graph_cholesky_param_t *param, const april_graph_t *g, Fn &&fn) {
    try { return fn(); }
    catch (const SolverError &e) { on_failure(param, g, e.code, e.msg); return e.code; }
    catch (const std::bad_alloc &) { on_failure(param, g, ERR_OOM, "host memory exhausted (std::bad_alloc)"); return ERR_OOM; }
    catch (const std::exception &e) { on_failure(param, g, ERR_INTERNAL, e.what()); return ERR_INTERNAL; }
}

static const int FIRST_EPOCH = 1 << 20;
struct Context;
static void rewind_epoch(Context &c, hipStream_t s, long long phases);
static void set_const_granules(Context &c, hipStream_t s);
enum { FACT_NONE = 0, FACT_PLAN = 1, FACT_EXTENDED = 2 };
static void record_factor(Context &c, int kind, const GraphPack &gp);
constexpr int INC_NODES = 4096, INC_FACT = 16384, INC_I32 = 4 << 20, INC_DEST = 1 << 20, INC_CHILD = 1 << 18, INC_TAB = 1 << 20;
#define TAIL_POSES (g_opt.tail_poses)
constexpr int MAX_TAIL_FRONTS = INC_NODES / 8 + 8;
constexpr long long INC_POOL_MIN = 8ll << 20;

static int waves_of(int nt) { return nt >= 1024 ? 16 : (nt >= 512 ? 8 : 4); }
static long long g_incfail[32] = { 0 };
static bool inc_fail(int why) { g_incfail[why & 31]++; return false; }
static long long g_updstat[6] = { 0 };
static double g_incsub[8] = { 0 }; static long long g_incsub_n = 0;
static const bool g_incprof_stamps = [] { const char *e = getenv("APRILSAM_AMD_INC_PROFILE"); return e && *e == '2'; }();
static int small_threads_for(size_t n_fronts) { return (int)n_fronts >= g_opt.tp_fronts ? std::min(g_opt.small_threads, g_opt.tp_threads) : g_opt.small_threads; }

static size_t diag_doubles(int n_big) { return (size_t)std::max(n_big, 1) * OBP * NB * NB; }
constexpr int BSB_MAX_WGS = 64;
template <class Dims, class KeepInv>
static void build_level(LevelPlan &L, std::vector<int> &fronts, std::vector<int> &tab, Dims dims, KeepInv keep_inv) {
    const size_t small_max = (size_t)g_opt.small_lds_kb * 1024;
    L = LevelPlan();
    std::vector<int> small, big;
    size_t maxm = 0;
    auto rows = [&](int t) { int a, b; dims(t, &a, &b); return 3 * (a + b + 1); };
    auto cols = [&](int t) { int a, b; dims(t, &a, &b); return 3 * (a + b); };
    auto nsb_of = [&](int t) { int a, b; dims(t, &a, &b); return a; };
    size_t full_max = small_max;
    if ((int)fronts.size() >= g_opt.tp_fronts && g_opt.tp_lds_kb > 0) full_max = std::min(small_max, (size_t)g_opt.tp_lds_kb * 1024);
    L.full_limit = (long long)full_max;
    L.small_nt = small_threads_for(fronts.size());
    const int nw = waves_of(L.small_nt);
    for (int t : fronts) {
        const int R = rows(t), C = cols(t);
        maxm = std::max<size_t>(maxm, C);
        L.solve_w_lds = std::max(L.solve_w_lds, backsolve_lds(C, 3 * nsb_of(t), true)); L.maxns = std::max(L.maxns, 3 * nsb_of(t));
        const size_t lds_s = small_front_lds(R, C, nw), lds_p = panel_front_lds(R, 3 * nsb_of(t), nw);
        if (lds_s <= full_max) { small.push_back(t); L.small_lds = std::max(L.small_lds, lds_s); }
        else if (g_opt.panel_mode && lds_p <= small_max) { small.push_back(t); L.small_lds = std::max(L.small_lds, lds_p); }
        else if (lds_s <= small_max) { small.push_back(t); L.small_lds = std::max(L.small_lds, lds_s); L.full_limit = std::max(L.full_limit, (long long)lds_s); }
        else big.push_back(t);
    }
    std::sort(small.begin(), small.end(), [&](int a, int b) { int ra = rows(a), rb = rows(b); return ra != rb ? ra > rb : a < b; });
    L.all_off = (int)tab.size(); L.n_all = (int)fronts.size();
    tab.insert(tab.end(), fronts.begin(), fronts.end());
    {
        std::vector<int> sp;
        for (int t : fronts) { int a, b; dims(t, &a, &b); if (bs_split_front(a, b)) sp.push_back(t); }
        L.bs_gemv = Launch{ (int)tab.size(), 0, (int)sp.size(), 0, false };
        tab.insert(tab.end(), sp.begin(), sp.end());
        L.bs_gemv.pre_off = (int)tab.size();
        int acc = 0; tab.push_back(0);
        for (int t : sp) { acc += (3 * nsb_of(t) + NB - 1) / NB; tab.push_back(acc); }
        L.bs_gemv.grid = acc;
    }
    L.solve_lds = (maxm + NB + 8 + NB * (NB + 1)) * 8;
    L.small_off = (int)tab.size(); L.n_small = (int)small.size();
    tab.insert(tab.end(), small.begin(), small.end());
    L.n_big = (int)big.size();
    if (big.empty()) return;
    std::sort(big.begin(), big.end(), [&](int a, int b) { return nsb_of(a) != nsb_of(b) ? nsb_of(a) > nsb_of(b) : a < b; });
    int list_off = (int)tab.size();
    tab.insert(tab.end(), big.begin(), big.end());
    auto make = [&](int nact, auto count) {
        Launch La; La.list_off = list_off; La.n = nact; La.pre_off = (int)tab.size();
        int acc = 0; tab.push_back(0);
        for (int i = 0; i < nact; i++) { acc += count(big[i]); tab.push_back(acc); }
        La.grid = acc; La.single = acc == nact;
        return La;
    };
    L.asm_big = make((int)big.size(), [&](int t) { return asm_chunks(cols(t) / 3); });
    {
        std::vector<int> wide, rest, bigs(big);
        std::sort(bigs.begin(), bigs.end());
        int wgs = 0;
        for (int t : fronts) {
            int a, b; dims(t, &a, &b);
            const bool isbig = std::binary_search(bigs.begin(), bigs.end(), t);
            if (isbig && 3 * a <= BSB_FAR && (b == 0 || bs_split_front(a, b)) && keep_inv(t)) { wide.push_back(t); wgs += 1 + bsb_helpers(3 * a); }
            else rest.push_back(t);
        }
        if (!wide.empty() && wgs <= BSB_MAX_WGS && g_opt.blk_backsolve) {
            const int lo = (int)tab.size();
            tab.insert(tab.end(), wide.begin(), wide.end());
            L.bs_blk = Launch{ lo, (int)tab.size(), (int)wide.size(), 0, false };
            int acc = 0; tab.push_back(0);
            for (int t : wide) { acc += 1 + bsb_helpers(3 * nsb_of(t)); tab.push_back(acc); L.bs_blk_lds = std::max(L.bs_blk_lds, bsb_lds(3 * nsb_of(t))); }
            L.bs_blk.grid = acc;
            L.rest_off = (int)tab.size(); L.n_rest = (int)rest.size();
            tab.insert(tab.end(), rest.begin(), rest.end());
            size_t mm = 0; for (int t : rest) mm = std::max<size_t>(mm, cols(t));
            L.rest_lds = (mm + NB + 8 + NB * (NB + 1)) * 8;
        }
    }
    const int steps = (3 * nsb_of(big[0]) + NB - 1) / NB;
// ... 117 lines not shown
    static_assert(sizeof(DestRec) == sizeof(Plan::DestRec), "DestRec layout");
    if (!P.dest.empty()) HIPCHECK(hipMemcpyAsync(c.d_dest.p, P.dest.data(), P.dest.size() * sizeof(DestRec), hipMemcpyHostToDevice, s));
    c.d_lambda.need((size_t)P.N + INC_NODES_);
    DevPlan &d = c.dp;
    d.nF = P.nF;
    d.fd = c.d_fd.p; d.dest = c.d_dest.p; d.child = c.d_child.p;
    d.f_rows = c.d_i32.p; d.f_rel = c.d_i32.p; d.slot_blk = c.d_i32.p + o_sb; d.slot_rhs = c.d_i32.p + o_sr; d.src_idx = c.d_i32.p;
    c.inc.o_rows = (long long)o_rows; c.inc.o_rel = (long long)o_rel;
    d.lambda = c.d_lambda.p;
    d.prof = nullptr; d.prof_mode = 0;
    d.schur_first_nub = std::max(0, g_opt.schur_first);
    d.epoch = nullptr; d.flevel = nullptr; d.l0 = 0; d.marks = nullptr;
    if (getenv("APRILSAM_AMD_KPROF")) { c.d_prof.need((size_t)PROF_SLOTS * P.nF); HIPCHECK(hipMemsetAsync(c.d_prof.p, 0, (size_t)8 * PROF_SLOTS * P.nF, s)); d.prof = c.d_prof.p; d.prof_mode = atoi(getenv("APRILSAM_AMD_KPROF")) >= 2 ? atoi(getenv("APRILSAM_AMD_KPROF")) : 1; }
    c.d_swap.need((size_t)P.F + INC_FACT_); c.d_pos.need((size_t)P.N + INC_NODES_);
    fill_swap_host(c);
    HIPCHECK(hipMemcpyAsync(c.d_swap.p, c.swap_host.data(), P.F, hipMemcpyHostToDevice, s));
    c.wt_dirty = false;
    HIPCHECK(hipMemcpyAsync(c.d_pos.p, P.pos.data(), (size_t)P.N * 4, hipMemcpyHostToDevice, s));
    c.d_perm.need((size_t)P.N + INC_NODES_);
    HIPCHECK(hipMemcpyAsync(c.d_perm.p, P.perm.data(), (size_t)P.N * 4, hipMemcpyHostToDevice, s));

    const double u2 = uprof ? now_ms() : 0;
    std::vector<int> tab;
    c.levels.assign(P.nLevels, LevelPlan());
    for (int l = 0; l < P.nLevels; l++) {
        std::vector<int> fr(P.lev_fronts.begin() + P.lev_ptr[l], P.lev_fronts.begin() + P.lev_ptr[l + 1]);
        build_level(c.levels[l], fr, tab, [&](int t, int *nsb, int *nub) { *nsb = P.f_nsb[t]; *nub = P.f_nub[t]; }, [](int) { return true; });
    }
    {
        long long slots = 0;
        for (int t = 0; t < P.nF; t++) fd[t].dinv0 = -1;
        for (int l = 0; l < P.nLevels; l++) {
            const LevelPlan &L = c.levels[l];
            for (int k = 0; k < L.asm_big.n; k++) { const int t = tab[L.asm_big.list_off + k]; fd[t].dinv0 = (int)slots; slots += (long long)OBP * bsb_blocks(3 * P.f_nsb[t]); }
        }
        c.d_dinv.need((size_t)std::max<long long>(slots, 1) * NB * NB);
        HIPCHECK(hipMemcpyAsync(c.d_fd.p, fd.data(), fd.size() * sizeof(FrontDesc), hipMemcpyHostToDevice, s));
        if (!c.d_bsb_flags.p) { c.d_bsb_flags.need((size_t)BSB_MAX_WGS * 2 * BSB_MAXB); HIPCHECK(hipMemsetAsync(c.d_bsb_flags.p, 0, c.d_bsb_flags.cap * 4, s)); c.d_bsb_far.need((size_t)BSB_MAX_WGS * BSB_FAR); }
    }
    for (int l = 0; l < P.nLevels; l++)
        if (c.levels[l].solve_lds > 160 * 1024)
            fail(ERR_UNSUPPORTED, "a frontal matrix has more rows than the back-substitution kernel can hold in LDS (an unsplittable dense region "
                 "of more than ~6000 poses); this build does not tile the solve of such a front");
    c.persist_l0 = -1;
    if (g_opt.persist && !lay && P.nLevels >= 3) {
        int l0 = P.nLevels, cnt = 0;
        const int nt_top = c.levels[P.nLevels - 1].small_nt;
        for (int l = P.nLevels - 1; l >= 0; l--) {
            const LevelPlan &L = c.levels[l];
            if (L.n_big > 0 || L.bs_gemv.grid > 0 || L.small_nt != nt_top || L.n_small != L.n_all || cnt + L.n_small > g_opt.persist_max_fronts) break;
            cnt += L.n_small; l0 = l;
        }
        if (P.nLevels - l0 >= 2) {
            c.persist_l0 = l0; c.p_nt = nt_top; c.p_up_lds = 0; c.p_dn_lds = 0; c.p_up_full = 0; c.p_dn_maxns = 0; c.p_dn_maxnu = 0;
            c.p_up_off = (int)tab.size(); c.p_up_n = cnt;
            for (int l = l0; l < P.nLevels; l++) {
                const LevelPlan &L = c.levels[l];
                for (int k = 0; k < L.n_small; k++) tab.push_back(tab[L.small_off + k]);
                c.p_up_lds = std::max(c.p_up_lds, L.small_lds); c.p_up_full = std::max(c.p_up_full, L.full_limit);
                for (int k = 0; k < L.n_all; k++) { const int t = tab[L.all_off + k]; c.p_dn_lds = std::max(c.p_dn_lds, backsolve_lds(P.cols(t), 3 * P.f_nsb[t], true)); c.p_dn_maxns = std::max(c.p_dn_maxns, 3 * P.f_nsb[t]); c.p_dn_maxnu = std::max(c.p_dn_maxnu, P.cols(t) - 3 * P.f_nsb[t]); }
            }
            c.p_dn_off = (int)tab.size(); c.p_dn_n = cnt;
            for (int l = P.nLevels - 1; l >= l0; l--) { const LevelPlan &L = c.levels[l]; for (int k = 0; k < L.n_all; k++) tab.push_back(tab[L.all_off + k]); }
        }
    }
    c.x_up_n = c.x_dn_n = c.x_leaf_n = 0;
    if (c.persist_l0 >= 0 && g_opt.xcd_place) {
        int cus = 0;
        HIPCHECK(hipDeviceGetAttribute(&cus, hipDeviceAttributeMultiprocessorCount, physical_device(t_slot)));
        const int per_xcd = std::max(1, cus / 8);
        auto per_cu = [](size_t lds, int nt) { return std::max(1, std::min(2048 / std::max(nt, 64), (int)((160 * 1024) / std::max<size_t>(lds, 1)))); };
        const std::vector<int> up(tab.begin() + c.p_up_off, tab.begin() + c.p_up_off + c.p_up_n);
        const LevelPlan &L0 = c.levels[0];
        const bool leaf = c.persist_l0 == 1 && L0.n_big == 0 && L0.bs_gemv.grid == 0 && L0.bs_blk.grid == 0 && L0.n_small == L0.n_all;
        const std::vector<int> leaves = leaf ? std::vector<int>(tab.begin() + L0.small_off, tab.begin() + L0.small_off + L0.n_small) : std::vector<int>();
        const int cap = per_xcd * per_cu(c.p_up_lds, c.p_nt), cap_leaf = per_xcd * (((int)leaves.size() + 8 * per_xcd - 1) / (8 * per_xcd));
        const XcdLists x = xcd_place(up, leaves, P.f_parent.data(), P.f_nsb.data(), P.nF, cap, cap_leaf);
        c.x_up_off = (int)tab.size(); c.x_up_n = (int)x.up.size(); tab.insert(tab.end(), x.up.begin(), x.up.end());
        c.x_dn_off = (int)tab.size(); c.x_dn_n = (int)x.dn.size(); tab.insert(tab.end(), x.dn.begin(), x.dn.end());
        c.x_leaf_off = (int)tab.size(); c.x_leaf_n = (int)x.leaf.size(); tab.insert(tab.end(), x.leaf.begin(), x.leaf.end());
    }
    {
        const size_t stride = (size_t)P.nF + MAX_TAIL_FRONTS;
        const bool fresh = c.d_flags.need(3 * stride);
        c.d_flevel.need(stride);
        if (fresh || (size_t)c.flag_stride != stride) HIPCHECK(hipMemsetAsync(c.d_flags.p, 0, c.d_flags.cap * 4, s));
        c.flag_stride = (int)stride;
        if (c.d_marks.need(stride)) HIPCHECK(hipMemsetAsync(c.d_marks.p, 0, c.d_marks.cap * 4, s));
        if (c.d_epoch.need(1)) { HIPCHECK(hipMemcpyAsync(c.d_epoch.p, &FIRST_EPOCH, 4, hipMemcpyHostToDevice, s)); c.epoch_steps = 0; }
        d.epoch = c.d_epoch.p;
    }
    if (inc) { c.d_upd.need((size_t)g_opt.persist_max_fronts + 64); c.d_wbuf.need((size_t)1 << 19); }
    HIPCHECK(hipMemcpyAsync(c.d_flevel.p, P.f_level.data(), (size_t)P.nF * 4, hipMemcpyHostToDevice, s));
    if (tab.empty()) tab.push_back(0);
    c.d_tab.need(tab.size() + INC_TAB_);
    c.inc.tab_used = (long long)tab.size();
    c.base_tab = tab;
    const double u3 = uprof ? now_ms() : 0;
    HIPCHECK(hipMemcpyAsync(c.d_tab.p, tab.data(), tab.size() * 4, hipMemcpyHostToDevice, s));
    HIPCHECK(hipStreamSynchronize(s));
    const double u4 = uprof ? now_ms() : 0;

    const long long pool_slack = inc ? std::max<long long>(INC_POOL_MIN, P.pool_doubles / 4) : 0;
    const long long pool_doubles = lay ? lay->pool_doubles : P.pool_doubles;
    c.d_pool.need((size_t)std::max<long long>(pool_doubles, 1) + (size_t)pool_slack);
    c.inc.pool_used = pool_doubles; c.inc.pool_cap = (long long)c.d_pool.cap;
    c.n_guard = 0;
    if (g_opt.pool_guard > 0 && !lay) {
        const long long G = ((long long)g_opt.pool_guard + 31) & ~31ll;
        std::vector<long long> go((size_t)P.nF);
        for (int t = 0; t < P.nF; t++) go[t] = P.f_off[t] + ((((long long)P.rows(t) * P.cols(t)) + 31) & ~31ll);
        c.d_guard.need((size_t)P.nF); c.d_guard_cnt.need(2);
        HIPCHECK(hipMemcpyAsync(c.d_guard.p, go.data(), go.size() * 8, hipMemcpyHostToDevice, s));
        HIPCHECK(hipMemsetAsync(c.d_guard_cnt.p, 0, 8, s));
// ... 125 lines not shown
```

### aprilsam_amd/csrc/solver_inc.inc.h

```cpp

static void inc_prepare(Context &c) {
    IncState &I = c.inc; const Plan &P = c.plan;
    I.Nb = P.N; I.Fb = P.F; I.nF0 = P.nF; I.nLev0 = P.nLevels;
    I.pos_front.assign(P.N, 0);
    for (int t = 0; t < P.nF; t++) for (int k = 0; k < P.f_nsb[t]; k++) I.pos_front[P.f_first[t] + k] = t;
    I.parent.assign(P.f_parent.begin(), P.f_parent.end());
    I.E.assign(P.nF, {}); I.xfac.assign(P.nF, {});
    I.bf_ptr.assign(P.nF + 1, 0);
    for (int f = 0; f < P.F; f++) if (P.fac_front[f] >= 0) I.bf_ptr[P.fac_front[f] + 1]++;
    for (int t = 0; t < P.nF; t++) I.bf_ptr[t + 1] += I.bf_ptr[t];
    I.bf_idx.resize(P.F);
    { std::vector<int> fill(I.bf_ptr.begin(), I.bf_ptr.end() - 1); for (int f = 0; f < P.F; f++) if (P.fac_front[f] >= 0) I.bf_idx[fill[P.fac_front[f]]++] = f; }
    I.rel_begin.assign(P.nF, 0); I.cur_nub.assign(P.nF, 0); I.cur_cap.assign(P.nF, 0);
    for (int t = 0; t < P.nF; t++) { I.rel_begin[t] = (int)(I.o_rel + P.f_rows_ptr[t]); I.cur_nub[t] = P.f_nub[t]; I.cur_cap[t] = (long long)P.rows(t) * P.cols(t); }
    I.dirty.assign(P.nF, 0);
    I.f_level.assign(P.f_level.begin(), P.f_level.end());
    I.fd.resize(P.nF);
    I.t_first.clear(); I.t_cnt.clear(); I.tf_of.clear(); I.kids.assign(P.nF, {}); I.tail_ok = -1; I.recs_stale = -1;
    I.stale.assign(P.nF, 0); I.upd_ok = true;
    I.base_has_big = false;
    for (const LevelPlan &L : c.levels) I.base_has_big = I.base_has_big || L.n_big > 0;
    I.base_levels = c.levels;
    c.inc_slot_blk.clear(); c.inc_slot_rhs.clear();
    I.ready = true; I.pristine = true;
// ... 74 lines not shown
            D.nsb = n_new; D.nub = nph; I.cur_nub[T] = nph;
            I.recs_stale = T; I.tail_ok = T;
            c.st.reserved0 = 1; c.st.inc_fronts_updated = 0;
            PatchList &PL = c.patches;
            PL.reset();
            const int f0 = gp.F_on_device;
            if (F > f0) {
                PL.add(gp.d_fa.p + f0, gp.h_fa.p + f0, (size_t)(F - f0) * 4); PL.add(gp.d_fb.p + f0, gp.h_fb.p + f0, (size_t)(F - f0) * 4);
                PL.add(gp.d_z.p + (size_t)3 * f0, gp.h_z.p + (size_t)3 * f0, (size_t)(F - f0) * 24);
                PL.add(gp.d_W.p + (size_t)9 * f0, gp.h_W.p + (size_t)9 * f0, (size_t)(F - f0) * 72);
                gp.F_on_device = F;
            }
            if (!solve_here) PL.add(c.d_tab.p + I.tab_used, lst.data(), lst.size() * 4);
            PL.add(c.d_fd.p + T, &D, sizeof(FrontDesc));
            PL.add((int *)c.dp.slot_blk + (size_t)3 * Fold, new_slot_blk.data(), new_slot_blk.size() * 4);
            PL.add((int *)c.dp.slot_rhs + (size_t)2 * Fold, new_slot_rhs.data(), new_slot_rhs.size() * 4);
            PL.add(c.d_swap.p + Fold, new_swap.data(), new_swap.size());
            if (N > Nold) {
                int ids[TAILK + 1]; double zeros[TAILK + 1];
                const int nn = N - Nold;
                for (int i = 0; i < nn; i++) { ids[i] = Nold + i; zeros[i] = 0.0; }
                PL.add(c.d_pos.p + Nold, ids, (size_t)nn * 4);
                PL.add(c.d_perm.p + Nold, ids, (size_t)nn * 4);
                PL.add(c.d_lambda.p + Nold, zeros, (size_t)nn * 8);
                c.lambda_N = -1;
                P.perm.resize(N); P.pos.resize(N);
                for (int i = Nold; i < N; i++) { P.perm[i] = i; P.pos[i] = i; }
            }
            for (int i : gp.changed) {
                PL.add(gp.d_state.p + (size_t)3 * i, gp.h_state.p + (size_t)3 * i, 24);
                PL.add(gp.d_lp.p + (size_t)3 * i, gp.h_lp.p + (size_t)3 * i, 24);
            }
            set_small_attr();
            const Patch *hdr = PL.finish();
            IncPrologue &pro = c.pro;
            pro.patches = hdr; pro.payload = (const char *)PL.buf.p; pro.n_patch = (int)PL.hdr.size(); pro.f_begin = Fold; pro.f_end = F;
            pro.fa = gp.d_fa.p; pro.fb = gp.d_fb.p; pro.Z = gp.d_z.p; pro.Wm = gp.d_W.p; pro.lp = gp.d_lp.p; pro.st = gp.d_state.p; pro.swp = c.d_swap.p;
            pro.slot_blk = c.dp.slot_blk; pro.slot_rhs = c.dp.slot_rhs; pro.Hc = c.d_H.p; pro.bad = c.d_bad.p; pro.stamps = nullptr; pro.done = nullptr; pro.seq = 0;
            pro.inl = g_opt.inc_inline && PL.hdr.size() <= (size_t)INL_PATCHES && PL.used <= (size_t)INL_BYTES;
            if (pro.inl) { memcpy(c.inl.hdr, PL.hdr.data(), PL.hdr.size() * sizeof(Patch)); memcpy(c.inl.pay, PL.buf.p, PL.used); }
            c.one_wait = 0;
            if (g_incprof_stamps) { c.h_kstamp.need(8 + PROF_SLOTS); memset(c.h_kstamp.p, 0, 8 * (8 + PROF_SLOTS)); pro.stamps = c.h_kstamp.p; }
            if (g_opt.inc_one_spin) {
                if (!c.h_done.p) { c.h_done.need(16); c.h_done.p[0] = 0; }
                c.done_seq = c.done_seq >= 0x7ffffff0 ? 1 : c.done_seq + 1;
                pro.done = c.h_done.p; pro.seq = c.done_seq; c.one_wait = c.done_seq;
            }
            gp.h_out.need((size_t)3 * N);
            const UpdArgs upd1{ c.d_perm.p, gp.d_lp.p, nullptr, gp.d_dx.p, gp.h_out.p, gp.h_dx.p, c.h_bad.p };
            const IncFlags nofl{ c.d_epoch.p, nullptr, nullptr, 0 };
            rewind_epoch(c, s, 1);
            const int *dn = c.d_tab.p + I.tab_used; const int n_dn = solve_here ? 0 : (int)lst.size();
            const int one_nt = g_opt.inc_one_threads >= 1024 ? 1024 : g_opt.inc_one_threads >= 512 ? 512 : 256;
            launch_inc_one_nt(one_nt, lds, s, pro, nofl, c.inl, c.dp, tstep, (const int *)nullptr, 0, dn, n_dn, c.d_pool.p, 0ll, c.d_x.p, upd1);
            gp.mirror_sync = true;
            gp.new_states = gp.h_out.p;
            HIPCHECK(hipGetLastError());
            c.pat.resize((size_t)2 * F);
            for (int f = Fold; f < F; f++) { c.pat[2 * f] = fa[f]; c.pat[2 * f + 1] = fb[f]; }
            c.patN = N;
            c.st.n_fronts = nFr0; c.st.n_levels = I.nLev0 + nT0;
            return true;
        }
        tstep.solve = 0; tstep.s_idx = 0;
    }
    if (!tail_fast && I.recs_stale >= 0) I.dirty[I.recs_stale] = 1;
    auto n_tail = [&]() { return (int)I.t_first.size(); };
    int grown_lo = 1 << 30;
    for (int k = std::max(Nold, Nb); k < N; k++) {
        if (I.t_first.empty() || I.t_cnt.back() >= TAIL_POSES) {
            if (n_tail() >= MAX_TAIL_FRONTS - 1) return inc_fail(4);
            I.t_first.push_back(k); I.t_cnt.push_back(0);
            const int t = nF0 + n_tail() - 1;
            I.parent.push_back(-1); I.E.emplace_back(); I.xfac.emplace_back(); I.rel_begin.push_back(0); I.cur_nub.push_back(0); I.cur_cap.push_back(0);
            I.dirty.push_back(0); I.f_level.push_back(I.nLev0 + n_tail() - 1); I.kids.emplace_back(); I.stale.push_back(0);
            I.fd.emplace_back(); memset(&I.fd[t], 0, sizeof(FrontDesc));
            I.fd[t].first = k; I.fd[t].parent = -1; I.fd[t].dinv0 = -1;
        }
        I.t_cnt.back()++;
        I.tf_of.push_back(nF0 + n_tail() - 1);
        I.dirty[nF0 + n_tail() - 1] = 1;
        grown_lo = std::min(grown_lo, nF0 + n_tail() - 1);
    }
    const int nT = n_tail(), nFr = nF0 + nT;
    auto is_tail = [&](int t) { return t >= nF0; };
    auto owns = [&](int t, int node) {
        return is_tail(t) && node >= I.t_first[t - nF0] && node < I.t_first[t - nF0] + I.t_cnt[t - nF0];
    };
    auto set_parent = [&](int t, int par) {
        if (I.parent[t] == par) return;
        if (I.parent[t] >= nF0) { auto &kd = I.kids[I.parent[t]]; kd.erase(std::find(kd.begin(), kd.end(), t)); }
        I.parent[t] = par;
        if (par >= nF0) { auto &kd = I.kids[par]; kd.insert(std::lower_bound(kd.begin(), kd.end(), t), t); }
    };
    bool unfit = false;
    std::vector<char> &mid = I.st_mid; mid.assign(nFr, 0);
    auto add_struct = [&](int t, int k) {
        while (t >= 0 && !owns(t, k)) {
            auto &E = I.E[t];
            auto it = std::lower_bound(E.begin(), E.end(), k);
            if (it == E.end() || *it != k) { if (it != E.end()) mid[t] = 1; E.insert(it, k); I.dirty[t] = 1; }
            if (is_tail(t) || P.f_parent[t] < 0) {
                const int par = I.tf_of[E.front() - Nb];
                if (I.parent[t] >= 0 && I.parent[t] != par) { unfit = true; return; }
                set_parent(t, par);
            }
            t = I.parent[t];
// ... 230 lines not shown
    if (I.i32_used + (long long)st_i32.size() > (long long)c.d_i32.cap || I.dest_used + (long long)st_dest.size() > (long long)c.d_dest.cap ||
        I.child_used + (long long)st_child.size() > (long long)c.d_child.cap || (size_t)9 * I.slots_used > c.d_H.cap || (size_t)nFr > c.d_fd.cap ||
        (size_t)N > c.d_perm.cap) return inc_fail(9);
    const double tsub2 = now_ms();
    std::vector<int> &tab = I.st_tab; tab.clear(); std::vector<LevelPlan> dl(nLev);
    auto dims = [&](int t, int *nsb, int *nub) { *nsb = nsb_of(t); *nub = I.cur_nub[t]; };
    if (batch) {
        for (int l = 0; l < nLev; l++) {
            if (l < I.nLev0) lev_dirty[l].assign(P.lev_fronts.begin() + P.lev_ptr[l], P.lev_fronts.begin() + P.lev_ptr[l + 1]);
            else lev_dirty[l].assign(1, nF0 + l - I.nLev0);
        }
    }
    for (int l = 0; l < nLev; l++) if (!lev_dirty[l].empty()) build_level(dl[l], lev_dirty[l], tab, dims, [&](int t) { return I.fd[t].dinv0 >= 0; });
    I.need.assign(nFr, needed ? 0 : 1);
    if (needed && !batch) {
        for (const RefModel::Visit &v : *needed) {
            int t = v.node >= Nb ? I.tf_of[v.node - Nb] : I.pos_front[P.pos[v.node]];
            while (t >= 0 && !I.need[t]) { I.need[t] = 1; t = I.parent[t]; }
        }
    }
    std::vector<int> bs_off(nLev, -1), bs_n(nLev, 0), bs_maxns(nLev, 0);
    std::vector<size_t> bs_wlds(nLev, 0);
    auto bs_note = [&](int l, int t) { bs_wlds[l] = std::max(bs_wlds[l], backsolve_lds(3 * (nsb_of(t) + I.cur_nub[t]), 3 * nsb_of(t), true)); bs_maxns[l] = std::max(bs_maxns[l], 3 * nsb_of(t)); };
    for (int l = nLev - 1; l >= 0; l--) {
        bs_off[l] = (int)(I.tab_used + (long long)tab.size());
        if (batch) continue;
        if (l >= I.nLev0) { const int t = nF0 + (l - I.nLev0); if (I.need[t]) { tab.push_back(t); bs_n[l] = 1; bs_note(l, t); } }
        else if (needed) {
            for (int k = I.base_levels[l].all_off; k < I.base_levels[l].all_off + I.base_levels[l].n_all; k++) {
                const int t = c.base_tab[k];
                if (I.need[t]) { tab.push_back(t); bs_n[l]++; bs_note(l, t); }
            }
        }
    }
    if (I.tab_used + (long long)tab.size() > (long long)c.d_tab.cap) return inc_fail(10);
    for (int l = 0; l < nLev; l++) {
        if (lev_dirty[l].empty()) continue;
        LevelPlan &L = dl[l];
        const int sh = (int)I.tab_used;
        L.all_off += sh; L.small_off += sh; L.asm_big.list_off += sh; L.asm_big.pre_off += sh;
        for (auto &x : L.syrkw) { x.list_off += sh; x.pre_off += sh; }
        for (auto &x : L.syrka) { x.list_off += sh; x.pre_off += sh; }
        for (auto &x : L.syrk1) { x.list_off += sh; x.pre_off += sh; }
        for (auto &x : L.bchain) { x.list_off += sh; x.pre_off += sh; }
        for (auto &x : L.btile) { x.list_off += sh; x.pre_off += sh; }
        L.bs_blk.list_off += sh; L.bs_blk.pre_off += sh; L.rest_off += sh;
        L.bs_gemv.list_off += sh; L.bs_gemv.pre_off += sh;
        if (l < I.nLev0) for (int t : lev_dirty[l]) {
            I.base_levels[l].solve_lds = std::max(I.base_levels[l].solve_lds, (size_t)(3 * (P.f_nsb[t] + I.cur_nub[t]) + NB + 8 + NB * (NB + 1)) * 8);
            I.base_levels[l].solve_w_lds = std::max(I.base_levels[l].solve_w_lds, backsolve_lds(3 * (P.f_nsb[t] + I.cur_nub[t]), 3 * P.f_nsb[t], true));
        }
    }
    for (int l = 0; l < nLev; l++) if (diag_doubles(dl[l].n_big) > c.d_diag.cap) return inc_fail(11);
    int mp_up_off = 0, mp_dn_off = 0, mp_n = 0, mp_nt = 0; size_t mp_up_lds = 0, mp_dn_lds = 0; long long mp_full = 0; int mp_dn_maxns = 0;
    bool mp = batch && g_opt.persist && nLev >= 3;
    if (mp) {
        mp_nt = dl[nLev - 1].small_nt;
        for (int l = 1; l < nLev && mp; l++) {
            const LevelPlan &L = dl[l];
            mp = L.n_big == 0 && L.bs_gemv.grid == 0 && L.small_nt == mp_nt && L.n_small == L.n_all;
            mp_n += L.n_all;
        }
        mp = mp && mp_n <= g_opt.persist_max_fronts && nFr <= c.flag_stride;
    }
    if (mp) {
        const int sh = (int)I.tab_used;
        const size_t tab_size0 = tab.size();
        mp_up_off = sh + (int)tab.size();
        for (int l = 1; l < nLev; l++) {
            const LevelPlan &L = dl[l];
            for (int k = 0; k < L.n_small; k++) tab.push_back(tab[L.small_off - sh + k]);
            mp_up_lds = std::max(mp_up_lds, L.small_lds); mp_full = std::max(mp_full, L.full_limit);
            for (int k = 0; k < L.n_all; k++) { const int t = tab[L.all_off - sh + k]; mp_dn_lds = std::max(mp_dn_lds, backsolve_lds(3 * (nsb_of(t) + I.cur_nub[t]), 3 * nsb_of(t), true)); mp_dn_maxns = std::max(mp_dn_maxns, 3 * nsb_of(t)); }
        }
        mp_dn_off = sh + (int)tab.size();
        for (int l = nLev - 1; l >= 1; l--) { const LevelPlan &L = dl[l]; for (int k = 0; k < L.n_all; k++) tab.push_back(tab[L.all_off - sh + k]); }
        if (I.tab_used + (long long)tab.size() > (long long)c.d_tab.cap || mp_dn_lds > 160 * 1024) { mp = false; tab.resize(tab_size0); }
    }
    auto solve_lds_of = [&](int t) { return (size_t)(3 * (nsb_of(t) + I.cur_nub[t]) + NB + 8 + NB * (NB + 1)) * 8; };
    for (int t = 0; t < nFr; t++) if (I.need[t] && solve_lds_of(t) > 160 * 1024) return inc_fail(12);
    int iu_off = 0, iu_n = 0, iu_nt = 0; size_t iu_lds = 0; long long iu_full = 0;
    int id_off = 0, id_n = 0, id_maxns = 0, id_rest = -1; size_t id_lds = 0;
    bool iu = !batch && g_opt.persist && g_opt.inc_multi, id = iu;
    if (iu) {
        const int sh = (int)I.tab_used;
        for (int l = 0; l < nLev && iu; l++) {
            if (lev_dirty[l].empty()) continue;
            const LevelPlan &L = dl[l];
            if (iu_nt == 0) iu_nt = L.small_nt;
            iu = L.n_big == 0 && L.n_small == L.n_all && L.small_nt == iu_nt;
            iu_n += L.n_all; iu_lds = std::max(iu_lds, L.small_lds); iu_full = std::max(iu_full, L.full_limit);
        }
        iu = iu && (iu_n >= 1 || tail_fast) && iu_n <= g_opt.persist_max_fronts;
        if (iu) {
            iu_off = sh + (int)tab.size();
            for (int l = 0; l < nLev; l++) if (!lev_dirty[l].empty()) for (int k = 0; k < dl[l].n_small; k++) tab.push_back(tab[dl[l].small_off - sh + k]);
        }
    }
    if (any_upd) {
        if (!iu || (size_t)iu_n > c.d_upd.cap || nFr > c.flag_stride) return inc_fail(13);
        I.st_upd.resize(iu_n);
        const int sh = (int)I.tab_used;
        for (int i = 0; i < iu_n; i++) {
            const int t = tab[iu_off - sh + i];
            if (mode[t]) {
                I.st_upd[i] = rec_of[t];
                iu_lds = std::max(iu_lds, update_front_lds(3 * (nsb_of(t) + I.cur_nub[t] + 1), 3 * nsb_of(t), __builtin_popcount(fmask[t])));
            } else memset(&I.st_upd[i], 0, sizeof(UpdRec));
        }
    }
    if (id) {
        if (needed) {
            id_off = bs_off[nLev - 1];
            for (int l = nLev - 1; l >= 0; l--) { id_n += bs_n[l]; id_lds = std::max(id_lds, bs_wlds[l]); id_maxns = std::max(id_maxns, bs_maxns[l]); }
            id = id_n >= 1 && id_n <= g_opt.persist_max_fronts && id_lds <= 160 * 1024;
        } else {
            id_off = (int)(I.tab_used + (long long)tab.size());
            id_rest = nLev - 1;
            for (int l = nLev - 1; l >= 0; l--) {
                size_t lds = 0; int mx = 0, n = 0;
                if (l >= I.nLev0) { const int t = nF0 + (l - I.nLev0); lds = backsolve_lds(3 * (nsb_of(t) + I.cur_nub[t]), 3 * nsb_of(t), true); mx = 3 * nsb_of(t); n = 1; }
                else { const LevelPlan &L = I.base_levels[l]; lds = L.solve_w_lds; mx = L.maxns; n = L.n_all; }
                if (id_n + n > g_opt.persist_max_fronts || std::max(id_lds, lds) > 160 * 1024) break;
                if (l >= I.nLev0) tab.push_back(nF0 + (l - I.nLev0));
                else for (int k = 0; k < n; k++) tab.push_back(c.base_tab[I.base_levels[l].all_off + k]);
                id_n += n; id_lds = std::max(id_lds, lds); id_maxns = std::max(id_maxns, mx); id_rest = l - 1;
            }
            id = id_n >= 2;
            if (!id) id_rest = -1;
        }
    }
    bool one = iu && id && needed && g_opt.inc_one && iu_n <= g_opt.inc_one_up && id_n <= g_opt.inc_one_dn && id_maxns <= BSW_MAX_NS && g_opt.wave_backsolve;
    const int one_nt = g_opt.inc_one_threads >= 1024 ? 1024 : g_opt.inc_one_threads >= 512 ? 512 : 256;
    size_t one_lds = std::max(id_lds, tail_fast ? tail_refactor_lds() : (size_t)0);
    if (one) {
        for (int l = 0; l < nLev; l++) for (int t : lev_dirty[l]) {
            const int R = 3 * (nsb_of(t) + I.cur_nub[t] + 1), C = R - 3;
            if (any_upd && mode[t]) { one_lds = std::max(one_lds, update_front_lds(R, 3 * nsb_of(t), __builtin_popcount(fmask[t]))); continue; }
            const size_t full = small_front_lds(R, C, one_nt / 64);
            one_lds = std::max(one_lds, (long long)full <= iu_full ? full : panel_front_lds(R, 3 * nsb_of(t), one_nt / 64));
        }
        one = one_lds <= 160 * 1024;
    }
    if (!one) { iu = iu && (iu_n >= 2 || any_upd); id = id && id_n >= 2; }
    if (tail_fast && !one && tail_refactor_lds() > 64 * 1024) return inc_fail(14);
    if (I.tab_used + (long long)tab.size() > (long long)c.d_tab.cap) return inc_fail(15);
    c.st.reserved0 = (int)fd_dirty.size();
    c.st.dn_launch_fronts = one ? 0 : id ? id_n : mp ? mp_n : 0;
    if (!batch) {
        int nu_ = 0; for (int t : fd_dirty) nu_ += (any_upd && mode[t]) ? 1 : 0;
        c.st.inc_fronts_updated = nu_;
        if (any_upd) { g_updstat[0]++; g_updstat[2] += nu_; g_updstat[3] += (long long)fd_dirty.size() - nu_; } else { g_updstat[1]++; g_updstat[4] += (long long)fd_dirty.size(); }
        if (one) g_updstat[5]++;
    }
    const double tsub3 = now_ms();
    PatchList &PL = c.patches;
    PL.reset();
    {
        if (F > gp.F_cap) return inc_fail(16);
        const int f0 = gp.F_on_device;
        if (F > f0) {
            PL.add(gp.d_fa.p + f0, gp.h_fa.p + f0, (size_t)(F - f0) * 4); PL.add(gp.d_fb.p + f0, gp.h_fb.p + f0, (size_t)(F - f0) * 4);
            PL.add(gp.d_z.p + (size_t)3 * f0, gp.h_z.p + (size_t)3 * f0, (size_t)(F - f0) * 24);
            PL.add(gp.d_W.p + (size_t)9 * f0, gp.h_W.p + (size_t)9 * f0, (size_t)(F - f0) * 72);
            gp.F_on_device = F;
        }
    }
    PL.add(c.d_i32.p + I.i32_used, st_i32.data(), st_i32.size() * 4);
    PL.add(c.d_dest.p + I.dest_used, st_dest.data(), st_dest.size() * sizeof(DestRec));
    PL.add(c.d_child.p + I.child_used, st_child.data(), st_child.size() * sizeof(ChildRec));
    PL.add(c.d_tab.p + I.tab_used, tab.data(), tab.size() * 4);
    I.i32_used += (long long)st_i32.size(); I.dest_used += (long long)st_dest.size(); I.child_used += (long long)st_child.size();
    for (int t : fd_dirty) PL.add(c.d_fd.p + t, &I.fd[t], sizeof(FrontDesc));
    if (any_upd) PL.add(c.d_upd.p, I.st_upd.data(), I.st_upd.size() * sizeof(UpdRec));
    if (F > Fold) {
        PL.add((int *)c.dp.slot_blk + (size_t)3 * Fold, new_slot_blk.data(), new_slot_blk.size() * 4);
        PL.add((int *)c.dp.slot_rhs + (size_t)2 * Fold, new_slot_rhs.data(), new_slot_rhs.size() * 4);
        PL.add(c.d_swap.p + Fold, new_swap.data(), new_swap.size());
    }
    if (N > Nold) {
        std::vector<int> &ids = I.st_ids; std::vector<double> &zeros = I.st_zeros;
        ids.resize(N - Nold); zeros.assign(N - Nold, 0.0);
        for (int i = Nold; i < N; i++) ids[i - Nold] = i;
        PL.add(c.d_pos.p + Nold, ids.data(), ids.size() * 4);
        PL.add(c.d_perm.p + Nold, ids.data(), ids.size() * 4);
        if (!batch) PL.add(c.d_lambda.p + Nold, zeros.data(), zeros.size() * 8);
        c.lambda_N = -1;
        P.perm.resize(N); P.pos.resize(N);
        for (int i = Nold; i < N; i++) { P.perm[i] = i; P.pos[i] = i; }
    }
    if (batch) {
        c.h_lambda.assign(N, batch_lambda);
        PL.add(c.d_lambda.p, c.h_lambda.data(), (size_t)N * 8);
        c.lambda_N = -1;
    }
    if (mp) {
        I.st_ids.resize(nT);
        for (int i = 0; i < nT; i++) I.st_ids[i] = I.nLev0 + i;
        PL.add(c.d_flevel.p + nF0, I.st_ids.data(), (size_t)nT * 4);
    }
    const double tsub4 = now_ms();
    set_small_attr();
    if (iu && nFr > c.flag_stride) return inc_fail(13);
    rewind_epoch(c, s, 1);
    DevPlan dpi = c.dp; dpi.marks = c.d_marks.p;
    DevPlan dpm = c.dp; dpm.flevel = c.d_flevel.p; dpm.l0 = 1;
    int *const xfl = c.d_flags.p + c.flag_stride;
    const DevPlan dpx = launch_plan(c, c.dp, I.cur_nub.empty() ? 0 : 3 * *std::max_element(I.cur_nub.begin(), I.cur_nub.end()));
    const UpdCtx uctx = any_upd ? UpdCtx{ c.d_upd.p, c.d_wbuf.p, c.d_flags.p + (size_t)2 * c.flag_stride, gp.d_fa.p, gp.d_fb.p, gp.d_z.p, gp.d_W.p, gp.d_lp.p, gp.d_state.p } : UpdCtx{};
    if (batch) {
        PL.launch(s);
        enqueue_poison(c, s, nullptr, nFr);
        hipLaunchKernelGGL(k_load_states, dim3((3 * N + TPB - 1) / TPB), dim3(TPB), 0, s, 3 * N, gp.h_state.p, gp.d_state.p, gp.d_lp.p);
        enqueue_select(gp, s);
        enqueue_robust(gp, s, nullptr);
        hipLaunchKernelGGL((k_linearize_t<false>), dim3((F + TPB - 1) / TPB), dim3(TPB), 0, s, 0, F, (const int *)nullptr, gp.d_fa.p, gp.d_fb.p, gp.d_z.p, gp.d_W.p,
                           gp.d_lp.p, gp.d_state.p, c.d_swap.p, c.dp.slot_blk, c.dp.slot_rhs, c.d_H.p, c.d_bad.p, (const double *)nullptr, c.d_epoch.p);
    } else {
        if (patch_states) {
            for (int i : gp.changed) {
                PL.add(gp.d_state.p + (size_t)3 * i, gp.h_state.p + (size_t)3 * i, 24);
                PL.add(gp.d_lp.p + (size_t)3 * i, gp.h_lp.p + (size_t)3 * i, 24);
            }
        } else {
            hipLaunchKernelGGL(k_load_states_lp, dim3((3 * N + TPB - 1) / TPB), dim3(TPB), 0, s, 3 * N, gp.h_state.p, gp.h_lp.p, gp.d_state.p, gp.d_lp.p, c.d_bad.p);
        }
        const Patch *hdr = PL.finish();
        IncPrologue &pro = c.pro;
        pro.patches = hdr; pro.payload = (const char *)PL.buf.p; pro.n_patch = (int)PL.hdr.size(); pro.f_begin = Fold; pro.f_end = F;
        pro.fa = gp.d_fa.p; pro.fb = gp.d_fb.p; pro.Z = gp.d_z.p; pro.Wm = gp.d_W.p; pro.lp = gp.d_lp.p; pro.st = gp.d_state.p; pro.swp = c.d_swap.p;
        pro.slot_blk = c.dp.slot_blk; pro.slot_rhs = c.dp.slot_rhs; pro.Hc = c.d_H.p; pro.bad = c.d_bad.p; pro.stamps = nullptr; pro.done = nullptr; pro.seq = 0;
        pro.inl = g_opt.inc_inline && PL.hdr.size() <= (size_t)INL_PATCHES && PL.used <= (size_t)INL_BYTES;
        if (pro.inl) { memcpy(c.inl.hdr, PL.hdr.data(), PL.hdr.size() * sizeof(Patch)); memcpy(c.inl.pay, PL.buf.p, PL.used); }
        c.one_wait = 0;
        const IncFlags fl = (!one && iu) ? IncFlags{ c.d_epoch.p, c.d_marks.p, c.d_tab.p + iu_off, iu_n } : IncFlags{ c.d_epoch.p, nullptr, nullptr, 0 };
        if (tail_fast && !one) {
            launch_inc_one_nt(1024, tail_refactor_lds(), s, pro, fl, c.inl, c.dp, tstep, (const int *)nullptr, 0, (const int *)nullptr, 0, c.d_pool.p, iu_full, c.d_x.p, UpdArgs{});
        } else if (one) {
            if (g_incprof_stamps) { c.h_kstamp.need(8 + PROF_SLOTS); memset(c.h_kstamp.p, 0, 8 * (8 + PROF_SLOTS)); pro.stamps = c.h_kstamp.p; }
            if (g_opt.inc_one_spin) {
                if (!c.h_done.p) { c.h_done.need(16); c.h_done.p[0] = 0; }
                c.done_seq = c.done_seq >= 0x7ffffff0 ? 1 : c.done_seq + 1;
                pro.done = c.h_done.p; pro.seq = c.done_seq; c.one_wait = c.done_seq;
            }
            gp.h_out.need((size_t)3 * N);
            const UpdArgs upd1{ c.d_perm.p, gp.d_lp.p, nullptr, gp.d_dx.p, gp.h_out.p, gp.h_dx.p, c.h_bad.p };
            launch_inc_one_nt(one_nt, one_lds, s, pro, fl, c.inl, c.dp, tstep, c.d_tab.p + iu_off, iu_n, c.d_tab.p + id_off, id_n, c.d_pool.p, iu_full, c.d_x.p, upd1, uctx);
        } else
            hipLaunchKernelGGL(k_inc_prologue, dim3(1), dim3(1024), 0, s, pro, fl, c.inl);
    }
    if (g_opt.pool_poison > 0 && !batch && !one) {
        if (iu) { enqueue_poison(c, s, c.d_tab.p + iu_off, iu_n, 1, any_upd ? c.d_upd.p : nullptr); if (any_upd) HIPCHECK(hipMemsetAsync(c.d_wbuf.p, 0xff, c.d_wbuf.cap * 8, s)); }
        if (id) enqueue_poison(c, s, c.d_tab.p + id_off, id_n, 2);
    }
    if (iu && !one) launch_front_small_nt(iu_nt, iu_n, iu_lds, s, dpi, c.d_tab.p + iu_off, c.d_pool.p, c.d_H.p, c.d_bad.p, iu_full, c.d_flags.p, 1, uctx);
    for (int l = 0; l < nLev; l++) {
        if (lev_dirty[l].empty() || iu || one) continue;
        if (mp && l >= 1) {
            if (l > 1) continue;
            launch_front_small_nt(mp_nt, mp_n, mp_up_lds, s, dpm, c.d_tab.p + mp_up_off, c.d_pool.p, c.d_H.p, c.d_bad.p, mp_full, c.d_flags.p, 1);
            continue;
        }
        enqueue_factor_level(c, dl[l], s, no_timer);
    }
    if (mp) launch_backsolve_multi(c, s, dpx, c.d_tab.p + mp_dn_off, mp_n, mp_dn_lds, mp_dn_maxns, xfl, UpdArgs{});
    gp.h_out.need((size_t)3 * N);
    const UpdArgs upd = batch ? UpdArgs{} : UpdArgs{ c.d_perm.p, gp.d_lp.p, nullptr, gp.d_dx.p, gp.h_out.p, gp.h_dx.p, c.h_bad.p };
    bool rode = one;
    if (id && !one) {
        launch_backsolve_multi(c, s, dpx, c.d_tab.p + id_off, id_n, id_lds, id_maxns, xfl, upd);
        rode = true;
    }
    for (int l = (one ? -1 : id ? (needed ? -1 : id_rest) : nLev - 1); l >= 0; l--) {
        if (mp && l >= 1) continue;
        if (batch) { launch_backsolve(c, dl[l], s, no_timer); continue; }
        if (l >= I.nLev0 || needed) {
            if (bs_n[l] > 0) {
                const size_t lds = l >= I.nLev0 ? solve_lds_of(nF0 + l - I.nLev0) : I.base_levels[l].solve_lds;
                const bool wave = g_opt.wave_backsolve && bs_maxns[l] <= BSW_MAX_NS && bs_wlds[l] <= 160 * 1024;
                launch_backsolve_list(c, s, wave ? BS_WAVE : BS_THREAD, c.d_tab.p + bs_off[l], bs_n[l], wave ? bs_wlds[l] : lds, 0, c.d_bad.p, upd);
                rode = true;
            }
        } else {
            const LevelPlan &L = I.base_levels[l];
            launch_backsolve_list(c, s, BS_THREAD, c.d_tab.p + L.all_off, L.n_all, L.solve_lds, 0, c.d_bad.p, upd);
            rode = true;
        }
    }
    if (batch || !rode) {
        hipLaunchKernelGGL(k_update_states, dim3((N + TPB - 1) / TPB), dim3(TPB), 0, s, N, c.d_pos.p, c.d_x.p, gp.d_lp.p, gp.d_state.p, gp.d_dx.p,
                           batch ? gp.h_lp.p : gp.h_out.p, gp.h_dx.p, c.d_bad.p, c.h_bad.p);
        gp.mirror_sync = false;
    } else {
        gp.mirror_sync = true;
    }
    gp.new_states = gp.h_out.p;
    HIPCHECK(hipGetLastError());
    if (!batch) { const double te = now_ms(); g_incsub[0] += tsub1 - tsub0; g_incsub[1] += tsub2 - tsub1; g_incsub[2] += tsub3 - tsub2; g_incsub[3] += tsub4 - tsub3; g_incsub[4] += te - tsub4; g_incsub[5] += (double)fd_dirty.size(); g_incsub_n++; }
    if (nT > 0 && I.dirty[nFr - 1]) I.tail_ok = g_opt.inc_tail ? nFr - 1 : -1;
    for (int t : fd_dirty) I.dirty[t] = 0;
    c.pat.resize((size_t)2 * F);
    for (int f = Fold; f < F; f++) { c.pat[2 * f] = fa[f]; c.pat[2 * f + 1] = fb[f]; }
    c.patN = N;
    c.st.n_fronts = nFr; c.st.n_levels = nLev;
    return true;
}

static void check_guard(Context &c, hipStream_t s) {
    if (c.n_guard <= 0 || !c.d_pool.p) return;
    int cnt[2] = { 0, 0 };
    hipLaunchKernelGGL(k_guard, dim3(c.n_guard), dim3(TPB), 0, s, 1, c.d_guard.p, c.n_guard, c.guard_len, c.d_pool.p, c.d_guard_cnt.p);
    HIPCHECK(hipMemcpyAsync(cnt, c.d_guard_cnt.p, 8, hipMemcpyDeviceToHost, s));
    HIPCHECK(hipStreamSynchronize(s));
// ... 18 lines not shown
```

### aprilsam_amd/csrc/solver_launch.inc.h

```cpp

template <class K> static void allow_full_lds(K kern) { HIPCHECK(hipFuncSetAttribute((const void *)kern, hipFuncAttributeMaxDynamicSharedMemorySize, 160 * 1024)); }
static void set_small_attr() {
    static std::once_flag once[MAX_SLOTS];
    std::call_once(once[physical_device(t_slot) % MAX_SLOTS], [] {
        allow_full_lds(k_front_small<256>); allow_full_lds(k_front_small<512>); allow_full_lds(k_front_small<1024>);
        allow_full_lds(k_backsolve_t<false>); allow_full_lds(k_backsolve_t<true>); allow_full_lds(k_backsolve_w); allow_full_lds(k_backsolve_t<false, true>);
        allow_full_lds(k_block_chain); allow_full_lds(k_backsolve_blk); allow_full_lds(k_block_solve<1>); allow_full_lds(k_block_solve<2>);
        allow_full_lds(k_inc_one<256>); allow_full_lds(k_inc_one<512>); allow_full_lds(k_inc_one<1024>);
    });
}
template <class... Args> static void launch_front_small_nt(int nt, int grid, size_t lds, hipStream_t s, const Args &...a) {
    if (nt >= 1024) hipLaunchKernelGGL(k_front_small<1024>, dim3(grid), dim3(1024), lds, s, a...);
    else if (nt >= 512) hipLaunchKernelGGL(k_front_small<512>, dim3(grid), dim3(512), lds, s, a...);
    else hipLaunchKernelGGL(k_front_small<256>, dim3(grid), dim3(256), lds, s, a...);
}
template <class... Args> static void launch_inc_one_nt(int nt, size_t lds, hipStream_t s, const Args &...a) {
    if (nt >= 1024) hipLaunchKernelGGL(k_inc_one<1024>, dim3(1), dim3(1024), lds, s, a...);
    else if (nt >= 512) hipLaunchKernelGGL(k_inc_one<512>, dim3(1), dim3(512), lds, s, a...);
    else hipLaunchKernelGGL(k_inc_one<256>, dim3(1), dim3(256), lds, s, a...);
}

struct KTimer {
    Context *c = nullptr; hipStream_t s = nullptr; size_t nev = 0;
    int level = -1;
// ... 13 lines not shown
    else if (form == BS_THREAD_TALL) hipLaunchKernelGGL((k_backsolve_t<false, true>), dim3(n), dim3(TPB), lds, s, c.dp, list, c.d_pool.p, c.d_x.p, split, (int *)nullptr, 0, bad, upd);
    else hipLaunchKernelGGL((k_backsolve_t<false>), dim3(n), dim3(TPB), lds, s, c.dp, list, c.d_pool.p, c.d_x.p, split, (int *)nullptr, 0, bad, upd);
}

static void launch_backsolve(Context &c, const LevelPlan &L, hipStream_t s, KTimer &kt, const int *tab = nullptr, UpdArgs upd = UpdArgs{}, int list_off = -1, int list_n = 0) {
    if (!tab) tab = c.d_tab.p;
    if (!L.n_all) return;
    kt.tic(K_BACKSOLVE);
    if (L.bs_gemv.grid > 0)
        hipLaunchKernelGGL(k_backsolve_gemv, dim3(L.bs_gemv.grid), dim3(TPB), 0, s, c.dp, tab + L.bs_gemv.list_off, tab + L.bs_gemv.pre_off,
                           L.bs_gemv.n, c.d_pool.p, c.d_x.p);
    int n_all = list_off >= 0 ? list_n : L.n_all, all_off = list_off >= 0 ? list_off : L.all_off; size_t solve_lds = L.solve_lds;
    if (L.bs_blk.grid > 0) {
        hipLaunchKernelGGL(k_backsolve_blk, dim3(L.bs_blk.grid), dim3(TPB), L.bs_blk_lds, s, c.dp, tab + L.bs_blk.list_off, tab + L.bs_blk.pre_off, L.bs_blk.n,
                           c.d_pool.p, c.d_x.p, c.d_dinv.p, c.d_bsb_flags.p, c.d_bsb_far.p, L.bs_gemv.grid > 0 ? 1 : 0, c.d_bad.p, upd);
        n_all = L.n_rest; all_off = L.rest_off; solve_lds = L.rest_lds;
        if (!n_all) { kt.toc(); return; }
    }
    const bool wave = g_opt.wave_backsolve && L.bs_gemv.grid == 0 && L.n_all < g_opt.tp_fronts && L.maxns <= BSW_MAX_NS && L.solve_w_lds <= 80 * 1024;
    const BsForm form = wave ? BS_WAVE : solve_lds >= (size_t)(BS_TALL_ROWS + NB + 8 + NB * (NB + 1)) * 8 ? BS_THREAD_TALL : BS_THREAD;
    launch_backsolve_list(c, s, form, tab + all_off, n_all, wave ? L.solve_w_lds : solve_lds, L.bs_gemv.grid > 0 ? 1 : 0, c.d_bad.p, upd);
    kt.toc();
}

static int launch_xmode(const Context &c, int max_upd_rows) { return c.dp.xmode == X_TAGGED && max_upd_rows > TPB ? (int)X_FLUSH : c.dp.xmode; }
static int device_cus() {
    int cus = 0;
    HIPCHECK(hipDeviceGetAttribute(&cus, hipDeviceAttributeMultiprocessorCount, physical_device(t_slot)));
    return cus;
}
static size_t handover_lds(int xmode, size_t lds, int grid) {
    if (xmode == X_WT || (xmode == X_TAGGED && grid <= device_cus())) return std::max(lds, HANDOVER_LDS_MIN);
    return lds;
}
static DevPlan launch_plan(const Context &c, DevPlan d, int max_upd_rows) { d.xmode = launch_xmode(c, max_upd_rows); return d; }
static DevPlan persist_plan(const Context &c) { DevPlan d = c.dp; d.flevel = c.d_flevel.p; d.l0 = c.persist_l0; d.xmode = launch_xmode(c, c.p_dn_maxnu); return d; }
static void launch_backsolve_multi(Context &c, hipStream_t s, const DevPlan &dp, const int *list, int n, size_t lds, int maxns, int *xflags, const UpdArgs &upd) {
    lds = handover_lds(dp.xmode, lds, n);
    if (g_opt.wave_backsolve && maxns <= BSW_MAX_NS) hipLaunchKernelGGL(k_backsolve_w, dim3(n), dim3(TPB), lds, s, dp, list, c.d_pool.p, c.d_x.p, xflags, c.d_bad.p, upd);
    else hipLaunchKernelGGL((k_backsolve_t<true>), dim3(n), dim3(TPB), lds, s, dp, list, c.d_pool.p, c.d_x.p, 0, xflags, 1, c.d_bad.p, upd);
}

static void enqueue_poison(Context &c, hipStream_t s, const int *list, int n, int what = 3, const UpdRec *recs = nullptr) {
    if (g_opt.pool_poison <= 0 || n <= 0) return;
    static_assert(offsetof(UpdRec, mode) % 4 == 0 && sizeof(UpdRec) % 4 == 0, "UpdRec::mode as a strided int");
    hipLaunchKernelGGL(k_poison, dim3(n), dim3(TPB), 0, s, c.dp, list, n, recs ? (const int *)((const char *)recs + offsetof(UpdRec, mode)) : (const int *)nullptr,
                       (int)(sizeof(UpdRec) / 4), what, c.d_pool.p, c.d_x.p);
}
static void launch_front_persist(Context &c, hipStream_t s) {
    const bool xp = c.x_up_n > 0;
    const int *list = c.d_tab.p + (xp ? c.x_up_off : c.p_up_off), n = xp ? c.x_up_n : c.p_up_n;
    DevPlan dpe = persist_plan(c);
    if (g_opt.skip_flag_waits > 0) dpe.l0 = 1 << 30;
    launch_front_small_nt(c.p_nt, n, c.p_up_lds, s, dpe, list, c.d_pool.p, c.d_H.p, c.d_bad.p, c.p_up_full, c.d_flags.p, 1);
}

static void launch_front_small(Context &c, const LevelPlan &L, hipStream_t s, const int *tab = nullptr, int list_off = -1, int list_n = 0) {
    if (!tab) tab = c.d_tab.p;
    const int off = list_off >= 0 ? list_off : L.small_off, n = list_off >= 0 ? list_n : L.n_small;
    launch_front_small_nt(L.small_nt, n, L.small_lds, s, c.dp, tab + off, c.d_pool.p, c.d_H.p, c.d_bad.p, L.full_limit, (int *)nullptr, 0);
}

static void enqueue_big_steps(Context &c, const LevelPlan &L, hipStream_t s, KTimer &kt, const int *tab = nullptr) {
    if (!tab) tab = c.d_tab.p;
    const int xcd = std::max(0, g_opt.syrk_xcd_order) << SYRK_MODE_XCD_SHIFT;
    for (size_t o = 0; o < L.bchain.size(); o++) {
        const Launch &bc = L.bchain[o], &bt = L.btile[o], &sw = L.syrkw[o];
        kt.tic(K_PANEL_BIG);
        hipLaunchKernelGGL(k_block_chain, dim3(bc.n), dim3(BCH_THREADS), block_chain_lds(), s, c.dp, tab + bc.list_off, (int)o, c.d_pool.p, c.d_diag.p, c.d_dinv.p, c.d_bad.p);
        if (bt.grid > 0) {
            if (bt.tile == 2) hipLaunchKernelGGL(k_block_solve<2>, dim3(bt.grid), dim3(TPB), block_solve_lds(), s, c.dp, tab + bt.list_off, tab + bt.pre_off, bt.n, (int)o, c.d_pool.p, c.d_diag.p, c.d_dinv.p);
            else hipLaunchKernelGGL(k_block_solve<1>, dim3(bt.grid), dim3(TPB), block_solve_lds(), s, c.dp, tab + bt.list_off, tab + bt.pre_off, bt.n, (int)o, c.d_pool.p, c.d_diag.p, c.d_dinv.p);
        }
        kt.toc();
        auto wide = [&](const Launch &w, int s_lo, int s_hi, int mode) {
            if (w.grid <= 0) return;
            kt.tic(K_SYRK_BIG);
            if (w.tile == TILE / 2) hipLaunchKernelGGL(k_syrk_big32, dim3(w.grid), dim3(TPB), 0, s, c.dp, tab + w.list_off, tab + w.pre_off, w.n, s_lo, s_hi, mode | xcd, c.d_pool.p);
            else hipLaunchKernelGGL(k_syrk_big, dim3(w.grid), dim3(TPB), 0, s, c.dp, tab + w.list_off, tab + w.pre_off, w.n, s_lo, s_hi, mode | xcd, c.d_pool.p);
            kt.toc();
        };
        const int G = std::max(2, g_opt.syrk_group), g0 = (int)(o - o % G) * OBP;
        if (!L.paired) wide(sw, (int)o * OBP, (int)(o + 1) * OBP, 1);
        else if ((int)(o % G) != G - 1) { wide(L.syrka[o], g0, (int)(o + 1) * OBP, 2); wide(L.syrk1[o], g0, (int)(o + 1) * OBP, 1); }
        else wide(sw, g0, (int)(o + 1) * OBP, 1);
    }
}

static void enqueue_factor_level(Context &c, const LevelPlan &L, hipStream_t s, KTimer &kt, const int *tab = nullptr) {
    if (!tab) tab = c.d_tab.p;
    if (L.n_small) {
        kt.tic(K_FRONT_SMALL);
        launch_front_small(c, L, s, tab);
        kt.toc();
    }
    if (L.n_big) {
        kt.tic(K_ASSEMBLE_BIG);
        hipLaunchKernelGGL(k_assemble_big, dim3(L.asm_big.grid), dim3(TPB), L.asm_lds, s, c.dp, tab + L.asm_big.list_off,
                           tab + L.asm_big.pre_off, L.asm_big.n, c.d_pool.p, c.d_H.p);
        kt.toc();
        enqueue_big_steps(c, L, s, kt, tab);
    }
}

static void enqueue_linearise(Context &c, GraphPack &gp, hipStream_t s, bool unary_at_lp) {
    const int F = c.plan.F;
    enqueue_select(gp, s);
    enqueue_robust(gp, s, unary_at_lp ? gp.d_upt.p : (const double *)nullptr);
    auto launch = [&](auto kern) {
        hipLaunchKernelGGL(kern, dim3((F + TPB - 1) / TPB), dim3(TPB), 0, s, 0, F, (const int *)nullptr, gp.d_fa.p, gp.d_fb.p, gp.d_z.p, gp.d_W.p,
                           gp.d_lp.p, gp.d_state.p, c.d_swap.p, c.dp.slot_blk, c.dp.slot_rhs, c.d_H.p, c.d_bad.p, unary_at_lp ? gp.d_upt.p : (const double *)nullptr, c.d_epoch.p);
    };
    if (F >= g_opt.linearize_staged_min) launch(k_linearize_t<true>); else launch(k_linearize_t<false>);
// ... 113 lines not shown
```

### aprilsam_amd/host.py

```python
import ctypes as C
import os
import os

import numpy as np

from . import abi

_PKG_DIR = os.path.dirname(os.path.abspath(__file__))
PRODUCT_LIB = os.environ.get("APRILSAM_AMD_LIB") or os.path.join(_PKG_DIR, "lib", "libaprilsam_amd.so")

_dp = C.POINTER(C.c_double)
_ip = C.POINTER(C.c_int)


def _np_d(a):
    return a.ctypes.data_as(_dp)


def _np_i(a):
    return a.ctypes.data_as(_ip)


class MarginalsError(RuntimeError):

# ... 27 lines not shown
        self.dll = C.CDLL(self.path, mode=os.RTLD_LOCAL if hasattr(os, "RTLD_LOCAL") else 0)
        d = self.dll
        self.is_product = hasattr(d, "aprilsam_amd_version")
        d.april_graph_create.restype = C.POINTER(abi.Graph)
        d.april_graph_destroy.argtypes = [C.POINTER(abi.Graph)]
        d.april_graph_node_xyt_create.restype = C.POINTER(abi.Node)
        d.april_graph_node_xyt_create.argtypes = [_dp, _dp, _dp]
        d.april_graph_factor_xyt_create.restype = C.POINTER(abi.Factor)
        d.april_graph_factor_xyt_create.argtypes = [C.c_int, C.c_int, _dp, _dp, C.POINTER(abi.Matd3x3)]
        d.april_graph_factor_xytpos_create.restype = C.POINTER(abi.Factor)
        d.april_graph_factor_xytpos_create.argtypes = [C.c_int, _dp, _dp, C.POINTER(abi.Matd3x3)]
        d.april_graph_chi2.restype = C.c_double
        d.april_graph_chi2.argtypes = [C.POINTER(abi.Graph)]
        for name in ("april_graph_cholesky", "april_graph_cholesky_inc"):
            getattr(d, name).argtypes = [C.POINTER(abi.Graph), C.POINTER(abi.CholeskyParam)]
            getattr(d, name).restype = None
        d.april_graph_cholesky_inc_solver.argtypes = [C.POINTER(abi.Graph), C.POINTER(abi.CholeskyParam), _ip]
        d.april_graph_cholesky_inc_solver.restype = None
        d.april_graph_cholesky_param_init.argtypes = [C.POINTER(abi.CholeskyParam)]
        d.april_graph_cholesky_param_destory.argtypes = [C.POINTER(abi.CholeskyParam)]
        if self.is_product:
            self._add_node = d.aprilsam_amd_graph_add_node
            self._add_factor = d.aprilsam_amd_graph_add_factor
            d.aprilsam_amd_version.restype = C.c_char_p
            d.aprilsam_amd_get_stats.argtypes = [C.POINTER(abi.CholeskyParam), C.POINTER(abi.Stats)]
            d.aprilsam_amd_set_option.argtypes = [C.c_char_p, C.c_double]
            if hasattr(d, "aprilsam_amd_get_option"):
                d.aprilsam_amd_get_option.argtypes = [C.c_char_p, _dp]
                d.aprilsam_amd_debug_guard_selftest.argtypes = [C.POINTER(abi.CholeskyParam)]
            d.aprilsam_amd_last_error.argtypes = [C.c_char_p, C.c_int]
            d.aprilsam_amd_batch_resident.argtypes = [C.POINTER(abi.Graph), C.POINTER(abi.CholeskyParam),
                                                      C.c_int, _dp, _dp]
            for nm in ("begin", "sync", "end"):
                getattr(d, f"aprilsam_amd_resident_{nm}").argtypes = [C.POINTER(abi.Graph), C.POINTER(abi.CholeskyParam)]
            d.aprilsam_amd_resident_steps.argtypes = [C.POINTER(abi.Graph), C.POINTER(abi.CholeskyParam), C.c_int, C.c_int]
            d.aprilsam_amd_resident_chi2.argtypes = [C.POINTER(abi.Graph)]
            d.aprilsam_amd_resident_chi2.restype = C.c_double
            d.aprilsam_amd_set_device.argtypes = [C.c_int]
            if hasattr(d, "aprilsam_amd_param_set_device"):
                d.aprilsam_amd_param_set_device.argtypes = [C.POINTER(abi.CholeskyParam), C.c_int]
                d.aprilsam_amd_param_get_device.argtypes = [C.POINTER(abi.CholeskyParam)]
            d.aprilsam_amd_make_lattice.argtypes = [C.POINTER(abi.Graph), C.c_int]
            d.aprilsam_amd_lattice_arrays.argtypes = [C.c_int, _dp, _ip, _ip, _dp, _dp]
            d.aprilsam_amd_graph_from_arrays.argtypes = [C.POINTER(abi.Graph), C.c_int, _dp, C.c_int, _ip, _ip, _dp, _dp]
            if hasattr(d, "aprilsam_amd_graph_node_arrays"):
                d.aprilsam_amd_graph_node_arrays.argtypes = [C.POINTER(abi.Graph), _dp, _dp, _dp]
                d.aprilsam_amd_graph_node_arrays.restype = None
            d.aprilsam_amd_plan_create.restype = C.c_void_p
            d.aprilsam_amd_plan_create.argtypes = [C.c_int, C.c_int, _ip, _dp, C.c_int]
            d.aprilsam_amd_plan_destroy.argtypes = [C.c_void_p]
            d.aprilsam_amd_plan_query.restype = C.c_longlong
            d.aprilsam_amd_plan_query.argtypes = [C.c_void_p, C.c_char_p, C.POINTER(C.POINTER(C.c_longlong))]
            d.aprilsam_amd_free.argtypes = [C.c_void_p]
            if hasattr(d, "aprilsam_amd_marginals"):
                d.aprilsam_amd_marginals.argtypes = [C.POINTER(abi.Graph), C.POINTER(abi.CholeskyParam), C.c_int, _ip, _dp]
                d.aprilsam_amd_marginals_joint.argtypes = [C.POINTER(abi.Graph), C.POINTER(abi.CholeskyParam), C.c_int, _ip, _ip, _dp]
                d.aprilsam_amd_debug_selinv_runs.argtypes = [C.POINTER(abi.CholeskyParam)]
                d.aprilsam_amd_debug_selinv_runs.restype = C.c_longlong
            if hasattr(d, "aprilsam_amd_marginals_joint_any"):
                d.aprilsam_amd_marginals_joint_any.argtypes = [C.POINTER(abi.Graph), C.POINTER(abi.CholeskyParam), C.c_int, _ip, _ip, _dp]
                d.aprilsam_amd_gate_xyt.argtypes = [C.POINTER(abi.Graph), C.POINTER(abi.CholeskyParam), C.c_int, _ip, _ip, _dp, _dp, _dp, _dp]
                d.aprilsam_amd_debug_path_solve_bytes.argtypes = [C.POINTER(abi.CholeskyParam)]
                d.aprilsam_amd_debug_path_solve_bytes.restype = C.c_longlong
            if hasattr(d, "aprilsam_amd_optimize_lm"):
                d.aprilsam_amd_lm_opts_init.argtypes = [C.POINTER(abi.LmOpts)]
                d.aprilsam_amd_lm_opts_init.restype = None
                d.aprilsam_amd_optimize_lm.argtypes = [C.POINTER(abi.Graph), C.POINTER(abi.CholeskyParam), C.POINTER(abi.LmOpts),
                                                       C.POINTER(abi.LmReport), _dp]
            if hasattr(d, "aprilsam_amd_initialize_chordal"):
                d.aprilsam_amd_chordal_opts_init.argtypes = [C.POINTER(abi.ChordalOpts)]
                d.aprilsam_amd_chordal_opts_init.restype = None
                for nm in ("aprilsam_amd_initialize_chordal", "aprilsam_amd_debug_chordal_raw"):
                    getattr(d, nm).argtypes = [C.POINTER(abi.Graph), C.POINTER(abi.CholeskyParam), C.POINTER(abi.ChordalOpts),
                                               C.POINTER(abi.ChordalReport), _dp]
            if hasattr(d, "aprilsam_amd_factor_max_create"):
                d.aprilsam_amd_factor_max_create.restype = C.POINTER(abi.Factor)
                d.aprilsam_amd_factor_max_create.argtypes = [C.POINTER(C.POINTER(abi.Factor)), _dp, C.c_int]
            if hasattr(d, "aprilsam_amd_max_selected"):
                d.aprilsam_amd_max_selected.argtypes = [C.POINTER(abi.Graph), C.POINTER(abi.CholeskyParam), C.c_int, _ip, _ip]
            if hasattr(d, "aprilsam_amd_factor_set_robust"):
                d.aprilsam_amd_factor_set_robust.argtypes = [C.POINTER(abi.Factor), C.c_int, C.c_double]
                d.aprilsam_amd_factor_get_robust.argtypes = [C.POINTER(abi.Factor), C.POINTER(C.c_int), C.POINTER(C.c_double)]
            if hasattr(d, "aprilsam_amd_robust_weights"):
                d.aprilsam_amd_robust_weights.argtypes = [C.POINTER(abi.Graph), C.POINTER(abi.CholeskyParam), C.c_int, _ip, _dp]
            d.aprilsam_amd_graph_save_ex.argtypes = [C.POINTER(abi.Graph), C.c_char_p, C.c_ulonglong]
            d.aprilsam_amd_graph_load.restype = C.POINTER(abi.Graph)
            d.aprilsam_amd_graph_load.argtypes = [C.c_char_p]
            d.aprilsam_amd_attr_put_string.argtypes = [C.POINTER(C.c_void_p), C.c_char_p, C.c_char_p]
            d.aprilsam_amd_attr_get_string.restype = C.c_char_p
            d.aprilsam_amd_attr_get_string.argtypes = [C.c_void_p, C.c_char_p]
        else:
            self._add_node = d.rs_graph_add_node
            self._add_factor = d.rs_graph_add_factor
        d.april_graph_save.argtypes = [C.POINTER(abi.Graph), C.c_char_p]
        d.april_graph_create_from_file.restype = C.POINTER(abi.Graph)
        d.april_graph_create_from_file.argtypes = [C.c_char_p]
        self._add_node.argtypes = [C.POINTER(abi.Graph), C.POINTER(abi.Node)]
        self._add_factor.argtypes = [C.POINTER(abi.Graph), C.POINTER(abi.Factor)]
        self._libc = C.CDLL(None)
        self._libc.calloc.restype = C.c_void_p
        self._libc.calloc.argtypes = [C.c_size_t, C.c_size_t]

    def version(self):
        return self.dll.aprilsam_amd_version().decode()

    def device_count(self):
# ... 389 lines not shown
```

### include/aprilsam_amd.h

```cpp
#ifndef APRILSAM_AMD_H
#define APRILSAM_AMD_H

#include <stddef.h>
#include <stdint.h>

#ifdef __cplusplus
extern "C" {
#endif


typedef struct zarray {
    size_t el_sz;
    int    size;
    int    alloc;
    char  *data;
} zarray_t;

typedef struct matd {
    unsigned int nrows, ncols;
    double       data[];
} matd_t;

typedef struct april_graph {
    zarray_t   *factors;
// ... 186 lines not shown

int aprilsam_amd_optimize_lm(april_graph_t *graph, april_graph_cholesky_param_t *param, const aprilsam_amd_lm_opts_t *opts,
                             aprilsam_amd_lm_report_t *report, double *trace);

typedef struct {
    int    stages;
} aprilsam_amd_chordal_opts_t;
void aprilsam_amd_chordal_opts_init(aprilsam_amd_chordal_opts_t *opts);
typedef struct {
    int    status;
    int    n_degenerate;
    int    not_spd_stage;
    double min_norm;
    double F_initial, F_final;
} aprilsam_amd_chordal_report_t;
int aprilsam_amd_initialize_chordal(april_graph_t *graph, april_graph_cholesky_param_t *param, const aprilsam_amd_chordal_opts_t *opts,
                                    aprilsam_amd_chordal_report_t *report, double *rot_out);
int aprilsam_amd_debug_chordal_raw(april_graph_t *graph, april_graph_cholesky_param_t *param, const aprilsam_amd_chordal_opts_t *opts,
                                   aprilsam_amd_chordal_report_t *report, double *raw);

#define APRILSAM_AMD_FACTOR_MAX_TYPE 3
april_graph_factor_t *aprilsam_amd_factor_max_create(april_graph_factor_t **components, const double *logw, int n);
int aprilsam_amd_max_selected(april_graph_t *graph, april_graph_cholesky_param_t *param, int n, const int *factors, int *out);

enum { APRILSAM_AMD_ROBUST_NONE = 0, APRILSAM_AMD_ROBUST_HUBER = 1, APRILSAM_AMD_ROBUST_CAUCHY = 2, APRILSAM_AMD_ROBUST_DCS = 3 };
int aprilsam_amd_factor_set_robust(april_graph_factor_t *factor, int kind, double c);
int aprilsam_amd_factor_get_robust(const april_graph_factor_t *factor, int *kind, double *c);
int aprilsam_amd_robust_weights(april_graph_t *graph, april_graph_cholesky_param_t *param, int n, const int *factors, double *w);

typedef struct aprilsam_amd_host_comm {
    void *user;
    int (*send)(void *user, const double *buf, long long count, int dst);
    int (*recv)(void *user, double *buf, long long count, int src);
    int (*bcast)(void *user, double *buf, long long count, int root);
    int (*allreduce_sum)(void *user, double *buf, long long count);
} aprilsam_amd_host_comm_t;
int       aprilsam_amd_shard_begin(april_graph_t *graph, april_graph_cholesky_param_t *param, int rank, int world);
long long aprilsam_amd_shard_info(const april_graph_cholesky_param_t *param, int what, long long *out, long long cap);
int       aprilsam_amd_shard_comm_unique_id(char *out128);
int       aprilsam_amd_shard_comm_init_rccl(april_graph_cholesky_param_t *param, const char *id128);
int       aprilsam_amd_shard_comm_init_host(april_graph_cholesky_param_t *param, const aprilsam_amd_host_comm_t *callbacks);
int       aprilsam_amd_shard_comm_info(const april_graph_cholesky_param_t *param, long long *out5, char *rccl_path, int cap);
int       aprilsam_amd_shard_iterate(april_graph_t *graph, april_graph_cholesky_param_t *param, int n);
int       aprilsam_amd_shard_gather_states(april_graph_t *graph, april_graph_cholesky_param_t *param);
double    aprilsam_amd_shard_chi2(april_graph_t *graph, april_graph_cholesky_param_t *param);
void      aprilsam_amd_shard_end(april_graph_cholesky_param_t *param);

typedef struct aprilsam_amd_plan aprilsam_amd_plan_t;
aprilsam_amd_plan_t *aprilsam_amd_plan_create(int n_nodes, int n_factors, const int *factor_nodes ,
                                              const double *xy , int leaf_nodes);
void aprilsam_amd_plan_destroy(aprilsam_amd_plan_t *plan);
long long aprilsam_amd_plan_query(const aprilsam_amd_plan_t *plan, const char *what, long long **out);
long long aprilsam_amd_shard_plan(const aprilsam_amd_plan_t *plan, int world, int what, long long *out, long long cap);
int aprilsam_amd_xcd_place(int nF, const int *parent, const int *level, const int *nsb, int l0, int cap, int cap_leaf, int which, int *out, int out_cap);
void aprilsam_amd_free(void *p);

int aprilsam_amd_reference_order(int n_nodes, int n_factors, const int *fa, const int *fb, int *out_order, int *out_parent);

void *aprilsam_amd_refmodel_create(void);
void  aprilsam_amd_refmodel_destroy(void *m);
void  aprilsam_amd_refmodel_batch(void *m, int n_nodes, int n_factors, const int *fa, const int *fb);
int   aprilsam_amd_refmodel_inc_begin(void *m, int n_nodes, int n_factors, const int *fa, const int *fb);
int   aprilsam_amd_refmodel_solve_visit(void *m, const double *x, double dxy, double dth, int *visited);
void  aprilsam_amd_refmodel_get(void *m, int *parent, int *changed, int *relin);
int   aprilsam_amd_refmodel_check(void *m);

int aprilsam_amd_make_lattice(april_graph_t *graph, int K);
int aprilsam_amd_lattice_arrays(int K, double *states, int *fa, int *fb, double *z, double *W);
void aprilsam_amd_graph_from_arrays(april_graph_t *graph, int N, const double *states, int F, const int *fa,
                                    const int *fb, const double *z, const double *W);

void aprilsam_amd_graph_node_arrays(const april_graph_t *graph, double *state, double *l_point, double *delta_X);

int aprilsam_amd_debug_stage(april_graph_t *graph, april_graph_cholesky_param_t *param, int what, double *out);

int aprilsam_amd_debug_front_times(const april_graph_cholesky_param_t *param, long long *out, int n_fronts);

const char *aprilsam_amd_version(void);

#ifdef __cplusplus
}
#endif
#endif
```

Measured before the change: 4954 GN iterations/s.

## Add split LDS front layout with trimmed update-block stride for mid-size fronts

Adds a FORM_SPLIT layout for small fronts that do not fit fully in LDS. The supernode columns keep the full row stride, while the update columns use a shorter stride (R-ns). This lets more fronts factor entirely in LDS instead of dropping to the panel or global path. Assembly, syrk and factor routines are templated to handle the two-region addressing, and the update block is published to the pool before the flag. The cost is extra index arithmetic per access and more template variants, which may raise register pressure.

```diff
diff --git a/aprilsam_amd/csrc/capi.cpp b/aprilsam_amd/csrc/capi.cpp
--- a/aprilsam_amd/csrc/capi.cpp
+++ b/aprilsam_amd/csrc/capi.cpp
@@ -115,7 +115,6 @@
 const char *aprilsam_amd_version(void) { return "aprilsam_amd 0.1 (gfx950, multifrontal FP64)"; }
 void aprilsam_amd_free(void *p) { free(p); }
 
-struct aprilsam_amd_plan { asam::Plan P; };
 
 aprilsam_amd_plan_t *aprilsam_amd_plan_create(int n_nodes, int n_factors, const int *factor_nodes, const double *xy, int leaf_nodes) {
     aprilsam_amd_plan *pl = new aprilsam_amd_plan();
diff --git a/aprilsam_amd/csrc/kernels.hip.h b/aprilsam_amd/csrc/kernels.hip.h
--- a/aprilsam_amd/csrc/kernels.hip.h
+++ b/aprilsam_amd/csrc/kernels.hip.h
@@ -494,7 +494,7 @@
 }
 __device__ __forceinline__ void reset_flag(int *flag, int v) { __hip_atomic_store(flag, v, __ATOMIC_RELAXED, __HIP_MEMORY_SCOPE_AGENT); }
 
-enum { ASM_LDS = 0, ASM_GLOBAL = 1, ASM_SPLIT = 2 };
+enum { ASM_LDS = 0, ASM_GLOBAL = 1, ASM_SPLIT = 2, ASM_LDS2 = 3 };
 template <int NT, int MODE, bool ZERO = true>
 __device__ __forceinline__ void assemble_front(const DevPlan &P, const FrontDesc &D, const double *__restrict__ pool,
                                                const double *__restrict__ Hc, int bc0, int bc1, bool full,
@@ -505,10 +505,19 @@
     const int R = 3 * (nbc + 1);
     const int rhs_row = 3 * nbc;
     const int csplit = MODE == ASM_LDS ? (1 << 30) : (MODE == ASM_GLOBAL ? 0 : 3 * nsb);
-    auto put = [&](int col, int row, double v) { if (col < csplit) dstL[(size_t)col * ldL + row] = v; else dstG[(size_t)col * ldG + row] = v; };
-    auto add_plain = [&](int col, int row, double v) { if (col < csplit) dstL[(size_t)col * ldL + row] += v; else dstG[(size_t)col * ldG + row] += v; };
+    const int uoff = MODE == ASM_LDS2 ? (int)(dstG - dstL) : 0;
+    auto lidx = [&](int col, int row) { return (MODE == ASM_LDS2 && col >= csplit) ? uoff + col * ldG + row : col * ldL + row; };
+    auto put = [&](int col, int row, double v) {
+        if constexpr (MODE == ASM_LDS2) dstL[lidx(col, row)] = v;
+        else { if (col < csplit) dstL[(size_t)col * ldL + row] = v; else dstG[(size_t)col * ldG + row] = v; }
+    };
+    auto add_plain = [&](int col, int row, double v) {
+        if constexpr (MODE == ASM_LDS2) dstL[lidx(col, row)] += v;
+        else { if (col < csplit) dstL[(size_t)col * ldL + row] += v; else dstG[(size_t)col * ldG + row] += v; }
+    };
     auto add_child = [&](int col, int row, double v) {
-        if (col < csplit) front_add<false>(dstL + (size_t)col * ldL + row, v); else front_add<true>(dstG + (size_t)col * ldG + row, v);
+        if constexpr (MODE == ASM_LDS2) dstL[lidx(col, row)] += v;
+        else { if (col < csplit) front_add<false>(dstL + (size_t)col * ldL + row, v); else front_add<true>(dstG + (size_t)col * ldG + row, v); }
     };
     constexpr int NW = NT / 64;
     const int wv = __builtin_amdgcn_readfirstlane(tid >> 6), lane = tid & 63;
@@ -599,10 +608,12 @@
             const int r = T.r0[u] + lane;
             const bool inr = r < T.nrow[u];
             const int du = (T.rc[u] < T.nrow[u] - 1) ? 3 * T.d[u] + T.rc[u] % 3 : rhs_row;
-            if (T.col[u] < csplit) {
+            const bool own = T.col[u] < csplit;
+            if (MODE == ASM_LDS2 || own) {
+                const int cb = (MODE == ASM_LDS2 && !own) ? uoff : 0, cl = (MODE == ASM_LDS2 && !own) ? ldG : ldL;
 #pragma unroll
                 for (int c3 = 0; c3 < 3; c3++) {
-                    const int o = (inr && r >= T.cc[u] + c3) ? (T.col[u] + c3) * ldL + du : dummy_off;
+                    const int o = (inr && r >= T.cc[u] + c3) ? cb + (T.col[u] + c3) * cl + du : dummy_off;
                     dstL[o] += T.v[3 * u + c3];
                 }
             } else {
@@ -774,9 +785,10 @@
     }
 }
 
-template <int NT>
+template <int NT, bool SPLIT = false>
 __device__ __forceinline__ void lds_syrk16(double *__restrict__ S, int ld, int k_lo, int k_hi, int col_lo, int col_hi, int Rv,
-                                           int w0 = 0, int nw = NT / 64) {
+                                           int w0 = 0, int nw = NT / 64,
+                                           int csp = 1 << 30, int ldu = 0, int uoff = 0) {
     const int wave = __builtin_amdgcn_readfirstlane((int)(threadIdx.x >> 6)) - w0;
     const int lane = threadIdx.x & 63, l15 = lane & 15, l4 = lane >> 4;
     if (wave < 0 || wave >= nw) return;
@@ -790,13 +802,16 @@
         const int i0 = col_lo + 16 * ti, j0 = col_lo + 16 * tj;
         const int rj = min(j0 + l15, Rv - 1), ri = min(i0 + l15, Rv - 1);
         const int i = i0 + l15, jb = j0 + l4;
-        const int cbase = jb * ld + i;
-        bool ok[4];
-#pragma unroll
-        for (int reg = 0; reg < 4; reg++) { const int j = jb + 4 * reg; ok[reg] = i < Rv && j < col_hi && i >= j; }
+        bool ok[4]; int co[4];
+#pragma unroll
+        for (int reg = 0; reg < 4; reg++) {
+            const int j = jb + 4 * reg;
+            ok[reg] = i < Rv && j < col_hi && i >= j;
+            co[reg] = ((!SPLIT || j < csp) ? j * ld : uoff + j * ldu) + i;
+        }
         double cv[4], x[4], y[4];
 #pragma unroll
-        for (int reg = 0; reg < 4; reg++) cv[reg] = S[ok[reg] ? cbase + 4 * reg * ld : 0];
+        for (int reg = 0; reg < 4; reg++) cv[reg] = S[ok[reg] ? co[reg] : 0];
 #pragma unroll
         for (int ks = 0; ks < 4; ks++) {
             const int kk = 4 * ks + l4;
@@ -812,7 +827,7 @@
             }
         }
 #pragma unroll
-        for (int reg = 0; reg < 4; reg++) if (ok[reg]) S[cbase + 4 * reg * ld] = cv[reg] - acc[reg];
+        for (int reg = 0; reg < 4; reg++) if (ok[reg]) S[co[reg]] = cv[reg] - acc[reg];
     }
 }
 
@@ -889,8 +904,9 @@
         for (int c = 0; c < BWT; c++) if (c < wdt) S[(k0 + c) * ld + k0 + r] = (c <= r) ? Dd[c] : 0.0;
     }
 }
-template <int NT>
-__device__ __forceinline__ void factor_dense_blk(double *S, int ld, int ns, int Rv, int hi, int *bad, double * , long long *pf = nullptr) {
+template <int NT, bool SPLIT = false>
+__device__ __forceinline__ void factor_dense_blk(double *S, int ld, int ns, int Rv, int hi, int *bad, double * , long long *pf = nullptr,
+                                                 int csp = 1 << 30, int ldu = 0, int uoff = 0) {
     constexpr int NW = NT / 64;
     long long t_chain = 0, t_syrk = 0, t0 = 0;
     const int wave = __builtin_amdgcn_readfirstlane(threadIdx.x >> 6);
@@ -920,8 +936,8 @@
         const int wdt = min(BW, ns - k0), below0 = k0 + wdt;
         if (below0 < ns) {
             const int next_hi = min(below0 + BW, ns), cw = chain_waves(below0);
-            if (NW >= 8) lds_syrk16<NT>(S, ld, k0, below0, below0, next_hi, Rv, 1, NW - 1);
-            else lds_syrk16<NT>(S, ld, k0, below0, below0, next_hi, Rv);
+            if (NW >= 8) lds_syrk16<NT, SPLIT>(S, ld, k0, below0, below0, next_hi, Rv, 1, NW - 1, csp, ldu, uoff);
+            else lds_syrk16<NT, SPLIT>(S, ld, k0, below0, below0, next_hi, Rv, 0, NW, csp, ldu, uoff);
             __syncthreads();
             if (pf) { const long long t1 = wall_clock64(); t_syrk += t1 - t0; t0 = t1; }
             if (wave < cw) {
@@ -930,31 +946,48 @@
                 chain_sync_store(below0, cw);
                 if (pf && threadIdx.x == 0) { pf[10] += clock64() - c0_; pf[15] += wall_clock64() - w0_; }
             } else {
-                if (next_hi < hi) lds_syrk16<NT>(S, ld, k0, below0, next_hi, hi, Rv, cw, NW - cw);
+                if (next_hi < hi) lds_syrk16<NT, SPLIT>(S, ld, k0, below0, next_hi, hi, Rv, cw, NW - cw, csp, ldu, uoff);
                 __syncthreads();
             }
             if (pf) { const long long t1 = wall_clock64(); t_chain += t1 - t0; t0 = t1; }
         } else {
             __syncthreads();
-            if (below0 < hi) lds_syrk16<NT>(S, ld, k0, below0, below0, hi, Rv);
+            if (below0 < hi) lds_syrk16<NT, SPLIT>(S, ld, k0, below0, below0, hi, Rv, 0, NW, csp, ldu, uoff);
             __syncthreads();
             if (pf) { const long long t1 = wall_clock64(); t_syrk += t1 - t0; t0 = t1; }
         }
     }
     if (pf && threadIdx.x == 0) { pf[8] = t_chain; pf[9] = t_syrk; }
 }
-template <int NT>
-__device__ __forceinline__ void factor_front_blk(double *S, int ld, int nsb, int nbc, int *bad, double *stage, int nbc_upd = -1, long long *pf = nullptr) {
+template <int NT, bool SPLIT = false>
+__device__ __forceinline__ void factor_front_blk(double *S, int ld, int nsb, int nbc, int *bad, double *stage, int nbc_upd = -1, long long *pf = nullptr,
+                                                 int csp = 1 << 30, int ldu = 0, int uoff = 0) {
     if (nbc_upd < 0) nbc_upd = nbc;
-    factor_dense_blk<NT>(S, ld, 3 * nsb, 3 * (nbc + 1) - 2, 3 * nbc_upd, bad, stage, pf);
+    factor_dense_blk<NT, SPLIT>(S, ld, 3 * nsb, 3 * (nbc + 1) - 2, 3 * nbc_upd, bad, stage, pf, csp, ldu, uoff);
 }
 
 __host__ __device__ inline size_t small_front_lds(int R, int C, int nw) { return (size_t)(R | 1) * C * 8 + wl_bytes(nw); }
 __host__ __device__ inline size_t panel_front_lds(int R, int ns, int nw) { return (size_t)(R | 1) * ns * 8 + wl_bytes(nw); }
+__host__ __device__ inline int split_front_ldu(int R, int ns) { return (R - ns) | 1; }
+__host__ __device__ inline size_t split_front_lds(int R, int C, int ns, int nw) {
+    return ((size_t)(R | 1) * ns + (size_t)split_front_ldu(R, ns) * (C - ns)) * 8 + wl_bytes(nw);
+}
+enum { FORM_FULL = 0, FORM_SPLIT = 1, FORM_PANEL = 2, FORM_BIG = 3 };
+__host__ __device__ inline int small_front_form(int R, int C, int ns, int nw, long long limit, int split_ok, size_t *lds = nullptr) {
+    size_t b = small_front_lds(R, C, nw);
+    int form = FORM_FULL;
+    if ((long long)b > limit) {
+        b = split_front_lds(R, C, ns, nw);
+        form = FORM_SPLIT;
+        if (!split_ok || C <= ns || (long long)b > limit) { b = panel_front_lds(R, ns, nw); form = FORM_PANEL; }
+    }
+    if (lds) *lds = b;
+    return form;
+}
 
 template <int NT>
 __device__ __forceinline__ void front_small_body(const DevPlan &P, const int t, double *__restrict__ pool, const double *__restrict__ Hc, int *bad,
-                                                 long long full_lds_limit, int *flags, int wait, double *S) {
+                                                 long long full_lds_limit, int split_ok, int *flags, int wait, double *S) {
     const int *wflags = wait ? flags : nullptr;
     const int ev = flags ? flag_value(P) : 0;
     const FrontDesc D = P.fd[t];
@@ -962,7 +995,26 @@
     const int R = 3 * (nbc + 1), C = 3 * nbc, ld = R | 1;
     double *Fg = pool + D.off;
     if (P.prof && threadIdx.x == 0) P.prof[(size_t)t * PROF_SLOTS + PROF_XCD_UP] = 1 + xcc_id();
-    if ((long long)small_front_lds(R, C, NT / 64) <= full_lds_limit) {
+    const int form = small_front_form(R, C, 3 * nsb, NT / 64, full_lds_limit, split_ok);
+    if (form == FORM_SPLIT) {
+        const int ns = 3 * nsb, ldu = split_front_ldu(R, ns);
+        const int uoff = ld * ns - ns * ldu - ns;
+        int2 *wl = (int2 *)(S + (size_t)ld * ns + (size_t)ldu * (C - ns));
+        if (P.prof && threadIdx.x == 0) P.prof[(size_t)t * PROF_SLOTS + 0] = wall_clock64();
+        assemble_front<NT, ASM_LDS2>(P, D, pool, Hc, 0, nbc, true, S, ld, S + uoff, ldu, wl, P.prof ? P.prof + (size_t)t * PROF_SLOTS : nullptr, wflags, bad, ev);
+        if (P.prof && threadIdx.x == 0) P.prof[(size_t)t * PROF_SLOTS + 1] = wall_clock64();
+        factor_front_blk<NT, true>(S, ld, nsb, nbc, bad, (double *)wl, -1, P.prof ? P.prof + (size_t)t * PROF_SLOTS : nullptr, ns, ldu, uoff);
+        if (P.prof && threadIdx.x == 0) P.prof[(size_t)t * PROF_SLOTS + 2] = wall_clock64();
+        for (int c = ns + (threadIdx.x >> 6); c < C; c += NT / 64) {
+            int r0 = 3 * (c / 3);
+            for (int r = r0 + (threadIdx.x & 63); r < R; r += 64) Fg[(size_t)c * R + r] = S[uoff + c * ldu + r];
+        }
+        if (flags) publish_flag(flags + t, ev);
+        for (int c = threadIdx.x >> 6; c < ns; c += NT / 64) {
+            int r0 = 3 * (c / 3);
+            for (int r = r0 + (threadIdx.x & 63); r < R; r += 64) Fg[(size_t)c * R + r] = S[(size_t)c * ld + r];
+        }
+    } else if (form == FORM_FULL) {
         int2 *wl = (int2 *)(S + (size_t)ld * C);
         if (P.prof && threadIdx.x == 0) P.prof[(size_t)t * PROF_SLOTS + 0] = wall_clock64();
         assemble_front<NT, ASM_LDS>(P, D, pool, Hc, 0, nbc, true, S, ld, nullptr, 0, wl, P.prof ? P.prof + (size_t)t * PROF_SLOTS : nullptr, wflags, bad, ev);
@@ -1295,7 +1347,7 @@
 
 template <int NT>
 __global__ void __launch_bounds__(NT) k_front_small(DevPlan P, const int *__restrict__ fronts, double *__restrict__ pool,
-                                                    const double *__restrict__ Hc, int *bad, long long full_lds_limit,
+                                                    const double *__restrict__ Hc, int *bad, long long full_lds_limit, int split_ok,
                                                     int *flags = nullptr, int wait = 0, UpdCtx uc = UpdCtx{}) {
     extern __shared__ __attribute__((aligned(16))) double S[];
     const int t = fronts[blockIdx.x];
@@ -1304,7 +1356,7 @@
         const UpdRec *rec = uc.recs + blockIdx.x;
         if (rec->mode) { front_update_body<NT>(P, t, *rec, uc, pool, flags, bad, S); return; }
     }
-    front_small_body<NT>(P, t, pool, Hc, bad, full_lds_limit, flags, wait, S);
+    front_small_body<NT>(P, t, pool, Hc, bad, full_lds_limit, split_ok, flags, wait, S);
 }
 
 constexpr int ASM_INV_CAP = 4096;
@@ -2514,7 +2566,7 @@
 template <int NT>
 __global__ void __launch_bounds__(NT) k_inc_one(IncPrologue a, IncFlags fl, InlinePatches, DevPlan P, TailStep ts, const int *__restrict__ up_list, int n_up,
                                                 const int *__restrict__ dn_list, int n_dn,
-                                                double *__restrict__ pool, long long full_lds_limit, double *__restrict__ x, UpdArgs upd, UpdCtx uc = UpdCtx{}) {
+                                                double *__restrict__ pool, long long full_lds_limit, int split_ok, double *__restrict__ x, UpdArgs upd, UpdCtx uc = UpdCtx{}) {
     extern __shared__ __attribute__((aligned(16))) double S[];
     long long *stamps = a.stamps;
     if (stamps && threadIdx.x == 0) stamps[0] = wall_clock64();
@@ -2539,10 +2591,10 @@
         }
         if (stamps && i == n_up - 1) {
             DevPlan Pp = P; Pp.prof = stamps + 8 - (size_t)t * PROF_SLOTS; Pp.prof_mode = 1;
-            front_small_body<NT>(Pp, t, pool, a.Hc, a.bad, full_lds_limit, nullptr, 0, S);
+            front_small_body<NT>(Pp, t, pool, a.Hc, a.bad, full_lds_limit, split_ok, nullptr, 0, S);
             if (threadIdx.x == 0) { const FrontDesc D = P.fd[t]; stamps[5] = D.nsb; stamps[6] = D.nub; stamps[7] = D.ch_end - D.ch_begin; }
         } else
-            front_small_body<NT>(P, t, pool, a.Hc, a.bad, full_lds_limit, nullptr, 0, S);
+            front_small_body<NT>(P, t, pool, a.Hc, a.bad, full_lds_limit, split_ok, nullptr, 0, S);
         __syncthreads();
     }
     if (stamps && threadIdx.x == 0) stamps[3] = wall_clock64();
diff --git a/aprilsam_amd/csrc/plan.h b/aprilsam_amd/csrc/plan.h
--- a/aprilsam_amd/csrc/plan.h
+++ b/aprilsam_amd/csrc/plan.h
@@ -74,3 +74,5 @@
 void plan_parallel_for(int n, int grain, const std::function<void(int, int)> &body);
 
 }
+
+struct aprilsam_amd_plan { asam::Plan P; };
diff --git a/aprilsam_amd/csrc/solver.h b/aprilsam_amd/csrc/solver.h
--- a/aprilsam_amd/csrc/solver.h
+++ b/aprilsam_amd/csrc/solver.h
@@ -27,6 +27,7 @@
     int syrk_small_tiles = 320;
     int syrk_pair_tiles = 2048;
     int syrk_group = 3;
+    int split_front = 1;
     int schur_first = 40;
     int small_threads = 1024;
     int tp_threads = 512;
diff --git a/aprilsam_amd/csrc/solver.hip.cpp b/aprilsam_amd/csrc/solver.hip.cpp
--- a/aprilsam_amd/csrc/solver.hip.cpp
+++ b/aprilsam_amd/csrc/solver.hip.cpp
@@ -53,7 +53,7 @@
     { "leaf_nodes", &Options::leaf_nodes, 1, false }, { "deterministic", &Options::deterministic, 0, true }, { "use_graph", &Options::use_graph, 0, true },
     { "device_timing", &Options::device_timing, 0, true }, { "trust_factor_cache", &Options::trust_factor_cache, 0, true },
     { "small_lds_kb", &Options::small_lds_kb, 0, false }, { "syrk_xcd_order", &Options::syrk_xcd_order, 0, false },
-    { "schur_first", &Options::schur_first, 0, false }, { "syrk_small_tiles", &Options::syrk_small_tiles, 0, false }, { "syrk_pair_tiles", &Options::syrk_pair_tiles, 0, false }, { "syrk_group", &Options::syrk_group, 2, false, 8 }, { "panel_mode", &Options::panel_mode, 0, false },
+    { "schur_first", &Options::schur_first, 0, false }, { "split_front", &Options::split_front, 0, false, 2 }, { "syrk_small_tiles", &Options::syrk_small_tiles, 0, false }, { "syrk_pair_tiles", &Options::syrk_pair_tiles, 0, false }, { "syrk_group", &Options::syrk_group, 2, false, 8 }, { "panel_mode", &Options::panel_mode, 0, false },
     { "small_threads", &Options::small_threads, 64, false }, { "tp_fronts", &Options::tp_fronts, 0, false }, { "tp_lds_kb", &Options::tp_lds_kb, 0, false },
     { "tp_threads", &Options::tp_threads, 64, false }, { "inc_fast", &Options::inc_fast, 0, true }, { "inc_multi", &Options::inc_multi, 0, true },
     { "inc_one", &Options::inc_one, 0, true }, { "inc_one_up", &Options::inc_one_up, 1, true }, { "inc_one_dn", &Options::inc_one_dn, 1, true },
@@ -341,7 +341,15 @@
         for (int R = 6; R < 400; R += 7)
             for (int nsb = 1; 3 * nsb < R - 3; nsb += 5) {
                 const int C = R - 3;
-                if (panel_front_lds(R, 3 * nsb, nw) > small_front_lds(R, C, nw)) return -41;
+                if (panel_front_lds(R, 3 * nsb, nw) > split_front_lds(R, C, 3 * nsb, nw) || split_front_lds(R, C, 3 * nsb, nw) > small_front_lds(R, C, nw)) return -41;
+                for (long long limit : { 16ll << 10, 64ll << 10, 156ll << 10 })
+                    for (int ok = 0; ok < 2; ok++) {
+                        size_t b = 0;
+                        const int form = small_front_form(R, C, 3 * nsb, nw, limit, ok, &b);
+                        const size_t f = small_front_lds(R, C, nw), sp = split_front_lds(R, C, 3 * nsb, nw), pn = panel_front_lds(R, 3 * nsb, nw);
+                        const int want = (long long)f <= limit ? FORM_FULL : (ok && (long long)sp <= limit) ? FORM_SPLIT : FORM_PANEL;
+                        if (form != want || b != (want == FORM_FULL ? f : want == FORM_SPLIT ? sp : pn)) return -43;
+                    }
                 if (small_front_lds(R, C, nw) != (size_t)(R | 1) * C * 8 + (size_t)wl_bytes(nw)) return -42;
             }
     for (int kind = 0; kind < 3; kind++)
@@ -426,6 +434,8 @@
 extern "C" int aprilsam_amd_robust_weights(april_graph_t *graph, april_graph_cholesky_param_t *param, int n, const int *factors, double *w) {
     return asam::robust_weights(graph, param, n, factors, w);
 }
+extern "C" int aprilsam_amd_front_modes(const aprilsam_amd_plan_t *plan, int *out, int cap) { return plan ? asam::front_modes(plan->P, out, cap) : -1; }
+extern "C" long long aprilsam_amd_debug_inc_split_fronts(void) { return asam::g_inc_split.load(std::memory_order_relaxed); }
 extern "C" long long aprilsam_amd_debug_selinv_runs(const april_graph_cholesky_param_t *param) { return asam::selinv_runs(param); }
 extern "C" int aprilsam_amd_marginals_joint_any(april_graph_t *graph, april_graph_cholesky_param_t *param, int n, const int *a, const int *b, double *cov) {
     return asam::marginals_joint_any(graph, param, n, a, b, cov);
diff --git a/aprilsam_amd/csrc/solver_context.inc.h b/aprilsam_amd/csrc/solver_context.inc.h
--- a/aprilsam_amd/csrc/solver_context.inc.h
+++ b/aprilsam_amd/csrc/solver_context.inc.h
@@ -5,6 +5,7 @@
 struct LevelPlan {
     int small_off = 0, n_small = 0; size_t small_lds = 0;
     long long full_limit = 0;
+    int split_ok = 0;
     int small_nt = 512;
     int n_big = 0; size_t asm_lds = 0;
     Launch asm_big{};
@@ -112,7 +113,7 @@
     DBuf<long long> d_guard; DBuf<int> d_guard_cnt; int n_guard = 0, guard_len = 0;
     std::vector<unsigned char> swap_host;
     int persist_l0 = -1;
-    int p_up_off = 0, p_up_n = 0, p_dn_off = 0, p_dn_n = 0, p_nt = 1024; size_t p_up_lds = 0, p_dn_lds = 0; long long p_up_full = 0; int p_dn_maxns = 0, p_dn_maxnu = 0;
+    int p_up_off = 0, p_up_n = 0, p_dn_off = 0, p_dn_n = 0, p_nt = 1024; size_t p_up_lds = 0, p_dn_lds = 0; long long p_up_full = 0; int p_up_split = 0; int p_dn_maxns = 0, p_dn_maxnu = 0;
     int x_up_off = 0, x_up_n = 0, x_dn_off = 0, x_dn_n = 0;
     int x_leaf_off = 0, x_leaf_n = 0;
     DBuf<int> d_flags, d_flevel, d_perm, d_epoch, d_marks;
@@ -277,31 +278,82 @@
 static int small_threads_for(size_t n_fronts) { return (int)n_fronts >= g_opt.tp_fronts ? std::min(g_opt.small_threads, g_opt.tp_threads) : g_opt.small_threads; }
 
 static size_t diag_doubles(int n_big) { return (size_t)std::max(n_big, 1) * OBP * NB * NB; }
+static int split_cus() {
+    if (device_count() < 1) return 256;
+    static std::atomic<int> cached[MAX_SLOTS];
+    std::atomic<int> &c = cached[physical_device(t_slot) % MAX_SLOTS];
+    int n = c.load(std::memory_order_relaxed);
+    if (n <= 0) { HIPCHECK(hipDeviceGetAttribute(&n, hipDeviceAttributeMultiprocessorCount, physical_device(t_slot))); c.store(n, std::memory_order_relaxed); }
+    return n;
+}
+struct SmallLaunch { int nt; size_t full_max; int split_ok; };
+static SmallLaunch small_launch_of(size_t n_fronts) {
+    const size_t small_max = (size_t)g_opt.small_lds_kb * 1024;
+    SmallLaunch a{ small_threads_for(n_fronts), small_max, 0 };
+    if ((int)n_fronts >= g_opt.tp_fronts && g_opt.tp_lds_kb > 0) a.full_max = std::min(small_max, (size_t)g_opt.tp_lds_kb * 1024);
+    a.split_ok = g_opt.split_front >= 2 || (g_opt.split_front == 1 && (long long)n_fronts <= split_cus());
+    return a;
+}
+static bool small_class(int R, int C, int ns, int nw, size_t full_max, long long *full_limit) {
+    const size_t small_max = (size_t)g_opt.small_lds_kb * 1024;
+    const size_t lds_s = small_front_lds(R, C, nw), lds_p = panel_front_lds(R, ns, nw);
+    if (lds_s <= full_max) return true;
+    if (g_opt.panel_mode && lds_p <= small_max) return true;
+    if (lds_s <= small_max) { *full_limit = std::max(*full_limit, (long long)lds_s); return true; }
+    return false;
+}
+template <class Fronts, class Dims> static size_t small_launch_lds(const Fronts &fronts, Dims dims, int nw, long long full_limit, int split_ok, int *n_split = nullptr) {
+    size_t lds = 0;
+    for (int t : fronts) {
+        int a, b; dims(t, &a, &b);
+        size_t one = 0;
+        const int form = small_front_form(3 * (a + b + 1), 3 * (a + b), 3 * a, nw, full_limit, split_ok, &one);
+        if (n_split && form == FORM_SPLIT) ++*n_split;
+        lds = std::max(lds, one);
+    }
+    return lds;
+}
+static std::atomic<long long> g_inc_split{ 0 };
+static int front_modes(const Plan &P, int *out, int cap) {
+    load_env_options();
+    for (int l = 0; l < P.nLevels; l++) {
+        const size_t n = (size_t)(P.lev_ptr[l + 1] - P.lev_ptr[l]);
+        const SmallLaunch sl = small_launch_of(n);
+        const int nw = waves_of(sl.nt);
+        long long limit = (long long)sl.full_max;
+        auto dims = [&](int t, int *R, int *C, int *ns) { *C = 3 * (P.f_nsb[t] + P.f_nub[t]); *R = *C + 3; *ns = 3 * P.f_nsb[t]; };
+        std::vector<char> small(n);
+        for (size_t k = 0; k < n; k++) { int R, C, ns; dims(P.lev_fronts[P.lev_ptr[l] + k], &R, &C, &ns); small[k] = small_class(R, C, ns, nw, sl.full_max, &limit); }
+        for (size_t k = 0; k < n; k++) {
+            const int t = P.lev_fronts[P.lev_ptr[l] + k];
+            int R, C, ns; dims(t, &R, &C, &ns);
+            if (out && t < cap) out[t] = small[k] ? small_front_form(R, C, ns, nw, limit, sl.split_ok) : (int)FORM_BIG;
+        }
+    }
+    return P.nF;
+}
+
 constexpr int BSB_MAX_WGS = 64;
 template <class Dims, class KeepInv>
 static void build_level(LevelPlan &L, std::vector<int> &fronts, std::vector<int> &tab, Dims dims, KeepInv keep_inv) {
-    const size_t small_max = (size_t)g_opt.small_lds_kb * 1024;
     L = LevelPlan();
     std::vector<int> small, big;
     size_t maxm = 0;
     auto rows = [&](int t) { int a, b; dims(t, &a, &b); return 3 * (a + b + 1); };
     auto cols = [&](int t) { int a, b; dims(t, &a, &b); return 3 * (a + b); };
     auto nsb_of = [&](int t) { int a, b; dims(t, &a, &b); return a; };
-    size_t full_max = small_max;
-    if ((int)fronts.size() >= g_opt.tp_fronts && g_opt.tp_lds_kb > 0) full_max = std::min(small_max, (size_t)g_opt.tp_lds_kb * 1024);
-    L.full_limit = (long long)full_max;
-    L.small_nt = small_threads_for(fronts.size());
+    const SmallLaunch sl = small_launch_of(fronts.size());
+    L.full_limit = (long long)sl.full_max;
+    L.split_ok = sl.split_ok;
+    L.small_nt = sl.nt;
     const int nw = waves_of(L.small_nt);
     for (int t : fronts) {
         const int R = rows(t), C = cols(t);
         maxm = std::max<size_t>(maxm, C);
         L.solve_w_lds = std::max(L.solve_w_lds, backsolve_lds(C, 3 * nsb_of(t), true)); L.maxns = std::max(L.maxns, 3 * nsb_of(t));
-        const size_t lds_s = small_front_lds(R, C, nw), lds_p = panel_front_lds(R, 3 * nsb_of(t), nw);
-        if (lds_s <= full_max) { small.push_back(t); L.small_lds = std::max(L.small_lds, lds_s); }
-        else if (g_opt.panel_mode && lds_p <= small_max) { small.push_back(t); L.small_lds = std::max(L.small_lds, lds_p); }
-        else if (lds_s <= small_max) { small.push_back(t); L.small_lds = std::max(L.small_lds, lds_s); L.full_limit = std::max(L.full_limit, (long long)lds_s); }
-        else big.push_back(t);
-    }
+        if (small_class(R, C, 3 * nsb_of(t), nw, sl.full_max, &L.full_limit)) small.push_back(t); else big.push_back(t);
+    }
+    L.small_lds = small_launch_lds(small, dims, nw, L.full_limit, L.split_ok);
     std::sort(small.begin(), small.end(), [&](int a, int b) { int ra = rows(a), rb = rows(b); return ra != rb ? ra > rb : a < b; });
     L.all_off = (int)tab.size(); L.n_all = (int)fronts.size();
     tab.insert(tab.end(), fronts.begin(), fronts.end());
@@ -525,14 +577,15 @@
             cnt += L.n_small; l0 = l;
         }
         if (P.nLevels - l0 >= 2) {
-            c.persist_l0 = l0; c.p_nt = nt_top; c.p_up_lds = 0; c.p_dn_lds = 0; c.p_up_full = 0; c.p_dn_maxns = 0; c.p_dn_maxnu = 0;
+            c.persist_l0 = l0; c.p_nt = nt_top; c.p_up_lds = 0; c.p_dn_lds = 0; c.p_up_full = 0; c.p_up_split = 1; c.p_dn_maxns = 0; c.p_dn_maxnu = 0;
             c.p_up_off = (int)tab.size(); c.p_up_n = cnt;
             for (int l = l0; l < P.nLevels; l++) {
                 const LevelPlan &L = c.levels[l];
                 for (int k = 0; k < L.n_small; k++) tab.push_back(tab[L.small_off + k]);
-                c.p_up_lds = std::max(c.p_up_lds, L.small_lds); c.p_up_full = std::max(c.p_up_full, L.full_limit);
+                c.p_up_full = std::max(c.p_up_full, L.full_limit); c.p_up_split = std::min(c.p_up_split, L.split_ok);
                 for (int k = 0; k < L.n_all; k++) { const int t = tab[L.all_off + k]; c.p_dn_lds = std::max(c.p_dn_lds, backsolve_lds(P.cols(t), 3 * P.f_nsb[t], true)); c.p_dn_maxns = std::max(c.p_dn_maxns, 3 * P.f_nsb[t]); c.p_dn_maxnu = std::max(c.p_dn_maxnu, P.cols(t) - 3 * P.f_nsb[t]); }
             }
+            c.p_up_lds = small_launch_lds(std::vector<int>(tab.begin() + c.p_up_off, tab.end()), [&](int t, int *nsb, int *nub) { *nsb = P.f_nsb[t]; *nub = P.f_nub[t]; }, waves_of(c.p_nt), c.p_up_full, c.p_up_split);
             c.p_dn_off = (int)tab.size(); c.p_dn_n = cnt;
             for (int l = P.nLevels - 1; l >= l0; l--) { const LevelPlan &L = c.levels[l]; for (int k = 0; k < L.n_all; k++) tab.push_back(tab[L.all_off + k]); }
         }
diff --git a/aprilsam_amd/csrc/solver_inc.inc.h b/aprilsam_amd/csrc/solver_inc.inc.h
--- a/aprilsam_amd/csrc/solver_inc.inc.h
+++ b/aprilsam_amd/csrc/solver_inc.inc.h
@@ -150,7 +150,7 @@
             rewind_epoch(c, s, 1);
             const int *dn = c.d_tab.p + I.tab_used; const int n_dn = solve_here ? 0 : (int)lst.size();
             const int one_nt = g_opt.inc_one_threads >= 1024 ? 1024 : g_opt.inc_one_threads >= 512 ? 512 : 256;
-            launch_inc_one_nt(one_nt, lds, s, pro, nofl, c.inl, c.dp, tstep, (const int *)nullptr, 0, dn, n_dn, c.d_pool.p, 0ll, c.d_x.p, upd1);
+            launch_inc_one_nt(one_nt, lds, s, pro, nofl, c.inl, c.dp, tstep, (const int *)nullptr, 0, dn, n_dn, c.d_pool.p, 0ll, 0, c.d_x.p, upd1);
             gp.mirror_sync = true;
             gp.new_states = gp.h_out.p;
             HIPCHECK(hipGetLastError());
@@ -487,7 +487,7 @@
         }
     }
     for (int l = 0; l < nLev; l++) if (diag_doubles(dl[l].n_big) > c.d_diag.cap) return inc_fail(11);
-    int mp_up_off = 0, mp_dn_off = 0, mp_n = 0, mp_nt = 0; size_t mp_up_lds = 0, mp_dn_lds = 0; long long mp_full = 0; int mp_dn_maxns = 0;
+    int mp_up_off = 0, mp_dn_off = 0, mp_n = 0, mp_nt = 0; size_t mp_up_lds = 0, mp_dn_lds = 0; long long mp_full = 0; int mp_split = 1, mp_dn_maxns = 0;
     bool mp = batch && g_opt.persist && nLev >= 3;
     if (mp) {
         mp_nt = dl[nLev - 1].small_nt;
@@ -505,16 +505,17 @@
         for (int l = 1; l < nLev; l++) {
             const LevelPlan &L = dl[l];
             for (int k = 0; k < L.n_small; k++) tab.push_back(tab[L.small_off - sh + k]);
-            mp_up_lds = std::max(mp_up_lds, L.small_lds); mp_full = std::max(mp_full, L.full_limit);
+            mp_full = std::max(mp_full, L.full_limit); mp_split = std::min(mp_split, L.split_ok);
             for (int k = 0; k < L.n_all; k++) { const int t = tab[L.all_off - sh + k]; mp_dn_lds = std::max(mp_dn_lds, backsolve_lds(3 * (nsb_of(t) + I.cur_nub[t]), 3 * nsb_of(t), true)); mp_dn_maxns = std::max(mp_dn_maxns, 3 * nsb_of(t)); }
         }
+        mp_up_lds = small_launch_lds(std::vector<int>(tab.begin() + (mp_up_off - sh), tab.end()), dims, waves_of(mp_nt), mp_full, mp_split);
         mp_dn_off = sh + (int)tab.size();
         for (int l = nLev - 1; l >= 1; l--) { const LevelPlan &L = dl[l]; for (int k = 0; k < L.n_all; k++) tab.push_back(tab[L.all_off - sh + k]); }
         if (I.tab_used + (long long)tab.size() > (long long)c.d_tab.cap || mp_dn_lds > 160 * 1024) { mp = false; tab.resize(tab_size0); }
     }
     auto solve_lds_of = [&](int t) { return (size_t)(3 * (nsb_of(t) + I.cur_nub[t]) + NB + 8 + NB * (NB + 1)) * 8; };
     for (int t = 0; t < nFr; t++) if (I.need[t] && solve_lds_of(t) > 160 * 1024) return inc_fail(12);
-    int iu_off = 0, iu_n = 0, iu_nt = 0; size_t iu_lds = 0; long long iu_full = 0;
+    int iu_off = 0, iu_n = 0, iu_nt = 0; size_t iu_lds = 0; long long iu_full = 0; int iu_split = 1, iu_nsplit = 0, one_nsplit = 0;
     int id_off = 0, id_n = 0, id_maxns = 0, id_rest = -1; size_t id_lds = 0;
     bool iu = !batch && g_opt.persist && g_opt.inc_multi, id = iu;
     if (iu) {
@@ -524,12 +525,13 @@
             const LevelPlan &L = dl[l];
             if (iu_nt == 0) iu_nt = L.small_nt;
             iu = L.n_big == 0 && L.n_small == L.n_all && L.small_nt == iu_nt;
-            iu_n += L.n_all; iu_lds = std::max(iu_lds, L.small_lds); iu_full = std::max(iu_full, L.full_limit);
+            iu_n += L.n_all; iu_full = std::max(iu_full, L.full_limit); iu_split = std::min(iu_split, L.split_ok);
         }
         iu = iu && (iu_n >= 1 || tail_fast) && iu_n <= g_opt.persist_max_fronts;
         if (iu) {
             iu_off = sh + (int)tab.size();
             for (int l = 0; l < nLev; l++) if (!lev_dirty[l].empty()) for (int k = 0; k < dl[l].n_small; k++) tab.push_back(tab[dl[l].small_off - sh + k]);
+            iu_lds = small_launch_lds(std::vector<int>(tab.begin() + (iu_off - sh), tab.end()), dims, waves_of(iu_nt), iu_full, iu_split, &iu_nsplit);
         }
     }
     if (any_upd) {
@@ -572,12 +574,14 @@
         for (int l = 0; l < nLev; l++) for (int t : lev_dirty[l]) {
             const int R = 3 * (nsb_of(t) + I.cur_nub[t] + 1), C = R - 3;
             if (any_upd && mode[t]) { one_lds = std::max(one_lds, update_front_lds(R, 3 * nsb_of(t), __builtin_popcount(fmask[t]))); continue; }
-            const size_t full = small_front_lds(R, C, one_nt / 64);
-            one_lds = std::max(one_lds, (long long)full <= iu_full ? full : panel_front_lds(R, 3 * nsb_of(t), one_nt / 64));
+            size_t form_lds = 0;
+            one_nsplit += small_front_form(R, C, 3 * nsb_of(t), one_nt / 64, iu_full, iu_split, &form_lds) == FORM_SPLIT;
+            one_lds = std::max(one_lds, form_lds);
         }
         one = one_lds <= 160 * 1024;
     }
     if (!one) { iu = iu && (iu_n >= 2 || any_upd); id = id && id_n >= 2; }
+    if (one || iu) g_inc_split.fetch_add(one ? one_nsplit : iu_nsplit, std::memory_order_relaxed);
     if (tail_fast && !one && tail_refactor_lds() > 64 * 1024) return inc_fail(14);
     if (I.tab_used + (long long)tab.size() > (long long)c.d_tab.cap) return inc_fail(15);
     c.st.reserved0 = (int)fd_dirty.size();
@@ -670,7 +674,7 @@
         c.one_wait = 0;
         const IncFlags fl = (!one && iu) ? IncFlags{ c.d_epoch.p, c.d_marks.p, c.d_tab.p + iu_off, iu_n } : IncFlags{ c.d_epoch.p, nullptr, nullptr, 0 };
         if (tail_fast && !one) {
-            launch_inc_one_nt(1024, tail_refactor_lds(), s, pro, fl, c.inl, c.dp, tstep, (const int *)nullptr, 0, (const int *)nullptr, 0, c.d_pool.p, iu_full, c.d_x.p, UpdArgs{});
+            launch_inc_one_nt(1024, tail_refactor_lds(), s, pro, fl, c.inl, c.dp, tstep, (const int *)nullptr, 0, (const int *)nullptr, 0, c.d_pool.p, iu_full, iu_split, c.d_x.p, UpdArgs{});
         } else if (one) {
             if (g_incprof_stamps) { c.h_kstamp.need(8 + PROF_SLOTS); memset(c.h_kstamp.p, 0, 8 * (8 + PROF_SLOTS)); pro.stamps = c.h_kstamp.p; }
             if (g_opt.inc_one_spin) {
@@ -680,7 +684,7 @@
             }
             gp.h_out.need((size_t)3 * N);
             const UpdArgs upd1{ c.d_perm.p, gp.d_lp.p, nullptr, gp.d_dx.p, gp.h_out.p, gp.h_dx.p, c.h_bad.p };
-            launch_inc_one_nt(one_nt, one_lds, s, pro, fl, c.inl, c.dp, tstep, c.d_tab.p + iu_off, iu_n, c.d_tab.p + id_off, id_n, c.d_pool.p, iu_full, c.d_x.p, upd1, uctx);
+            launch_inc_one_nt(one_nt, one_lds, s, pro, fl, c.inl, c.dp, tstep, c.d_tab.p + iu_off, iu_n, c.d_tab.p + id_off, id_n, c.d_pool.p, iu_full, iu_split, c.d_x.p, upd1, uctx);
         } else
             hipLaunchKernelGGL(k_inc_prologue, dim3(1), dim3(1024), 0, s, pro, fl, c.inl);
     }
@@ -688,12 +692,12 @@
         if (iu) { enqueue_poison(c, s, c.d_tab.p + iu_off, iu_n, 1, any_upd ? c.d_upd.p : nullptr); if (any_upd) HIPCHECK(hipMemsetAsync(c.d_wbuf.p, 0xff, c.d_wbuf.cap * 8, s)); }
         if (id) enqueue_poison(c, s, c.d_tab.p + id_off, id_n, 2);
     }
-    if (iu && !one) launch_front_small_nt(iu_nt, iu_n, iu_lds, s, dpi, c.d_tab.p + iu_off, c.d_pool.p, c.d_H.p, c.d_bad.p, iu_full, c.d_flags.p, 1, uctx);
+    if (iu && !one) launch_front_small_nt(iu_nt, iu_n, iu_lds, s, dpi, c.d_tab.p + iu_off, c.d_pool.p, c.d_H.p, c.d_bad.p, iu_full, iu_split, c.d_flags.p, 1, uctx);
     for (int l = 0; l < nLev; l++) {
         if (lev_dirty[l].empty() || iu || one) continue;
         if (mp && l >= 1) {
             if (l > 1) continue;
-            launch_front_small_nt(mp_nt, mp_n, mp_up_lds, s, dpm, c.d_tab.p + mp_up_off, c.d_pool.p, c.d_H.p, c.d_bad.p, mp_full, c.d_flags.p, 1);
+            launch_front_small_nt(mp_nt, mp_n, mp_up_lds, s, dpm, c.d_tab.p + mp_up_off, c.d_pool.p, c.d_H.p, c.d_bad.p, mp_full, mp_split, c.d_flags.p, 1);
             continue;
         }
         enqueue_factor_level(c, dl[l], s, no_timer);
diff --git a/aprilsam_amd/csrc/solver_launch.inc.h b/aprilsam_amd/csrc/solver_launch.inc.h
--- a/aprilsam_amd/csrc/solver_launch.inc.h
+++ b/aprilsam_amd/csrc/solver_launch.inc.h
@@ -89,13 +89,13 @@
     const int *list = c.d_tab.p + (xp ? c.x_up_off : c.p_up_off), n = xp ? c.x_up_n : c.p_up_n;
     DevPlan dpe = persist_plan(c);
     if (g_opt.skip_flag_waits > 0) dpe.l0 = 1 << 30;
-    launch_front_small_nt(c.p_nt, n, c.p_up_lds, s, dpe, list, c.d_pool.p, c.d_H.p, c.d_bad.p, c.p_up_full, c.d_flags.p, 1);
+    launch_front_small_nt(c.p_nt, n, c.p_up_lds, s, dpe, list, c.d_pool.p, c.d_H.p, c.d_bad.p, c.p_up_full, c.p_up_split, c.d_flags.p, 1);
 }
 
 static void launch_front_small(Context &c, const LevelPlan &L, hipStream_t s, const int *tab = nullptr, int list_off = -1, int list_n = 0) {
     if (!tab) tab = c.d_tab.p;
     const int off = list_off >= 0 ? list_off : L.small_off, n = list_off >= 0 ? list_n : L.n_small;
-    launch_front_small_nt(L.small_nt, n, L.small_lds, s, c.dp, tab + off, c.d_pool.p, c.d_H.p, c.d_bad.p, L.full_limit, (int *)nullptr, 0);
+    launch_front_small_nt(L.small_nt, n, L.small_lds, s, c.dp, tab + off, c.d_pool.p, c.d_H.p, c.d_bad.p, L.full_limit, L.split_ok, (int *)nullptr, 0);
 }
 
 static void enqueue_big_steps(Context &c, const LevelPlan &L, hipStream_t s, KTimer &kt, const int *tab = nullptr) {
diff --git a/aprilsam_amd/host.py b/aprilsam_amd/host.py
--- a/aprilsam_amd/host.py
+++ b/aprilsam_amd/host.py
@@ -103,6 +103,9 @@
             d.aprilsam_amd_plan_query.restype = C.c_longlong
             d.aprilsam_amd_plan_query.argtypes = [C.c_void_p, C.c_char_p, C.POINTER(C.POINTER(C.c_longlong))]
             d.aprilsam_amd_free.argtypes = [C.c_void_p]
+            if hasattr(d, "aprilsam_amd_front_modes"):
+                d.aprilsam_amd_front_modes.argtypes = [C.c_void_p, _ip, C.c_int]
+                d.aprilsam_amd_debug_inc_split_fronts.restype = C.c_longlong
             if hasattr(d, "aprilsam_amd_marginals"):
                 d.aprilsam_amd_marginals.argtypes = [C.POINTER(abi.Graph), C.POINTER(abi.CholeskyParam), C.c_int, _ip, _dp]
                 d.aprilsam_amd_marginals_joint.argtypes = [C.POINTER(abi.Graph), C.POINTER(abi.CholeskyParam), C.c_int, _ip, _ip, _dp]
diff --git a/include/aprilsam_amd.h b/include/aprilsam_amd.h
--- a/include/aprilsam_amd.h
+++ b/include/aprilsam_amd.h
@@ -262,6 +262,8 @@
 void aprilsam_amd_plan_destroy(aprilsam_amd_plan_t *plan);
 long long aprilsam_amd_plan_query(const aprilsam_amd_plan_t *plan, const char *what, long long **out);
 long long aprilsam_amd_shard_plan(const aprilsam_amd_plan_t *plan, int world, int what, long long *out, long long cap);
+int aprilsam_amd_front_modes(const aprilsam_amd_plan_t *plan, int *out, int cap);
+long long aprilsam_amd_debug_inc_split_fronts(void);
 int aprilsam_amd_xcd_place(int nF, const int *parent, const int *level, const int *nsb, int l0, int cap, int cap_leaf, int which, int *out, int out_cap);
 void aprilsam_amd_free(void *p);
 
```

Result: no change. 4920 GN iterations/s (-0.7%).
